# Westlake-AI/SemiReward

Hardware: AMD Instinct MI355X
Metric: unlabeled images/sec/node (FlexMatch+SR, ViT-S CIFAR-100) (higher is better)
Workload: dtype bf16

## Files before the change

include/srhip.h:

```cpp
#ifndef SRHIP_H
#define SRHIP_H

#ifdef __cplusplus
extern "C" {
#endif

enum {
  SRHIP_EPI_BF16 = 0,
  SRHIP_EPI_GELU_BF16 = 1,
  SRHIP_EPI_RESID_F32 = 2,
  SRHIP_EPI_DGELU_BF16 = 3,
  SRHIP_EPI_F32 = 4
};
int srhip_gemm_nt(int epilogue, const void* A, int lda, const void* B, int ldb, void* C, int ldc, int M, int N, int K,
                  const float* bias, const float* row_scale, int rows_per_sample, const void* aux_in, void* aux_out,
                  int ldaux, float alpha, float beta, void* stream);
#define SRHIP_GEMM_PLAN_TILE128 0
#define SRHIP_GEMM_PLAN_SMALL64 1
#define SRHIP_GEMM_PLAN_BIG256 2
#define SRHIP_GEMM_PLAN_BIG128 3
#define SRHIP_GEMM_PLAN_BIG2WG 4
#define SRHIP_GEMM_PLAN_PP256 5
int srhip_gemm_nt_plan(int epilogue, int M, int N, int K, float beta);
int srhip_gemm_nt_planned(int epilogue, const void* A, int lda, const void* B, int ldb, void* C, int ldc, int M, int N, int K,
                          const float* bias, const float* row_scale, int rows_per_sample, const void* aux_in, void* aux_out,
                          int ldaux, float alpha, float beta, int plan_M, void* stream);
int srhip_gemm_small_max_grid(int n);


int srhip_gemm_nt_resid_dropout(const void* A, int lda, const void* B, int ldb, float* C, int ldc, int M, int N, int K,
                                const float* bias, const float* resid, int ldresid, unsigned drop_key, unsigned drop_thresh,
                                float drop_scale, void* stream);
int srhip_gemm_nt_resid_ln_dropout(const void* A, int lda, const void* B, int ldb, float* C, int ldc, int M, int N, int K,
                                   const float* bias, const float* ln_mean, const float* ln_rstd, const float* ln_gamma,
                                   const float* ln_beta, unsigned drop_key, unsigned drop_thresh, float drop_scale, void* stream);

typedef struct srhip_group_desc {
  const void* A; const void* B; float* C;
  int M, N, K, lda, ldb, ldc, tile_start, pad0, pad1, pad2;
} srhip_group_desc;
int srhip_gemm_nt_grouped_f32(const srhip_group_desc* desc_dev, int n_problems, int total_tiles, float alpha, float beta,
                              void* stream);
int srhip_gemm_nt_grouped_n64_f32(const srhip_group_desc* desc_dev, int n_problems, int total_tiles, float alpha, float beta,
                                  void* stream);

#define SRHIP_TN_ATOMIC 1
#define SRHIP_TN_OVERWRITE 2
typedef struct srhip_group_tn_desc {
  const void* A; const void* B; float* C; float* dbias;
  int M, N, K, lda, ldb, ldc, tile_start, flags;
} srhip_group_tn_desc;
int srhip_gemm_tn_grouped_f32(const srhip_group_tn_desc* desc_dev, int n_problems, int total_tiles, float alpha, float beta,
                              void* stream);
typedef struct srhip_slab_desc {
  float* dst; const float* src; long long stride;
  int count, n_slabs, block_start, pad0;
} srhip_slab_desc;
int srhip_slab_reduce_f32(const srhip_slab_desc* desc_dev, int n, int total_blocks, void* stream);
int srhip_gemm_tn_grouped_pp_f32(const srhip_group_tn_desc* desc_dev, int n_problems, int total_tiles, float alpha, float beta,
                                 void* stream);

int srhip_attn_fwd(const void* qkv, void* out, float* lse, int B, int N, int H, float scale, void* stream);
int srhip_attn_bwd(const void* qkv, const void* out, const void* d_out, const float* lse, void* dqkv, float* delta_ws,
                   int B, int N, int H, float scale, void* stream);

int srhip_attn_plan(int B, int N, int H, int* nkt, int* fwd_pair, int* bwd_l2, int* bwd_split);

int srhip_attn_masked_fwd(const void* qkv, void* out, float* lse, const int* key_len, int B, int N, int H, float scale,
                          unsigned drop_key, unsigned drop_thresh, float drop_scale, void* stream);
int srhip_attn_masked_bwd(const void* qkv, const void* out, const void* d_out, const float* lse, void* dqkv, float* delta_ws,
                          const int* key_len, int B, int N, int H, float scale, unsigned drop_key, unsigned drop_thresh,
                          float drop_scale, void* stream);

int srhip_layernorm_fwd(const float* x, const float* gamma, const float* beta, float eps, void* out, float* mean,
                        float* rstd, int M, int D, void* stream);
int srhip_layernorm_bwd(const void* dy, const float* x, const float* mean, const float* rstd, const float* gamma,
                        float* dx, float* dgamma, float* dbeta, int M, int D, void* stream);
int srhip_layernorm_bwd_cast(const void* dy, const float* x, const float* mean, const float* rstd, const float* gamma, float* dx, float* dgamma,
                             float* dbeta, void* out_bf16, const float* row_scale, int rows_per_sample, int M, int D, void* stream);
int srhip_layernorm_bwd_part(const void* dy, const float* x, const float* mean, const float* rstd, const float* gamma, float* dx, float* part,
                             int n_rep, void* out_bf16, const float* row_scale, int rows_per_sample, int M, int D, void* stream);
typedef struct srhip_ln_reduce_desc { float* dgamma; float* dbeta; } srhip_ln_reduce_desc;
int srhip_ln_grad_reduce(const srhip_ln_reduce_desc* desc_dev, float* part, int n_ln, int n_rep, int D, void* stream);
typedef struct srhip_dw_tail {
  const srhip_ln_reduce_desc* ln_desc; float* ln_part;
  const float* dlogits; const float* feat; float* dWh; float* dbh;
  const float* dx; const float* img; const int* img_index; float* dpos; float* dcls; float* pe_ws;
  int n_ln, n_rep, C, B, D, in_chans, HW, ps;
} srhip_dw_tail;
int srhip_gemm_tn_grouped_tail_f32(const srhip_group_tn_desc* desc_dev, int n_problems, int total_tiles, float alpha, float beta,
                                   const srhip_dw_tail* tail, void* stream);
int srhip_patch_embed_bwd_fold(const float* ws, float* dWp, float* dbp, int B, int C, int HW, int ps, int D, void* stream);

int srhip_mlp_fused(const float* x, float* x_out, const float* ln_gamma, const float* ln_beta, float eps, const void* W1,
                    const float* b1, const void* W2, const float* b2, const float* row_scale, int rows_per_sample, int save_rows,
                    void* save_ln2, void* save_pre, void* save_h, float* save_mean, float* save_rstd, int M, int D, int Hd,
                    void* stream);
int srhip_gelu_eval(const float* x, float* y_erf, float* y_poly, int n, void* stream);
int srhip_mlp_fused_proj(const float* x, float* x_out, const void* ao, const void* Wp, const float* bp, const float* row_scale1,
                         int ao_scaled, const float* ln_gamma, const float* ln_beta, float eps, const void* W1, const float* b1, const void* W2,
                         const float* b2, const float* row_scale2, int rows_per_sample, void* ln_next, const float* next_gamma,
                         const float* next_beta, int M, int D, int Hd, void* stream);
int srhip_mlp_fused_proj_strided(const float* x, float* x_out, const void* ao, const void* Wp, const float* bp, const float* row_scale1,
                                 int ao_scaled, const float* ln_gamma, const float* ln_beta, float eps, const void* W1, const float* b1,
                                 const void* W2, const float* b2, const float* row_scale2, int rows_per_sample, void* ln_next,
                                 const float* next_gamma, const float* next_beta, int M, int D, int Hd, int row_pitch, void* stream);

int srhip_attn_block_supported(int N, int D, int H);
int srhip_attn_block_fused(const void* xn_bf16, const void* Wqkv, const float* bqkv, const void* qkv_extra, void* out, const float* out_scale,
                           int B, int N, int D, int H, float scale, void* stream);

int srhip_patch_embed_fwd(const float* img, const int* img_index, const float* Wp, const float* bp, const float* cls,
                          const float* pos, float* x, int B, int C, int HW, int ps, int D, void* stream);
int srhip_patch_embed_bwd(const float* dx, const float* img, const int* img_index, float* dWp, float* dbp, float* dcls,
                          float* dpos, int B, int C, int HW, int ps, int D, void* stream);
long srhip_patch_embed_bwd_ws_floats(int B, int C, int HW, int ps, int D);
int srhip_patch_embed_bwd_ws(const float* dx, const float* img, const int* img_index, float* dWp, float* dbp, float* dcls,
                             float* dpos, float* ws, int B, int C, int HW, int ps, int D, void* stream);

int srhip_patch_im2col(const float* img, const int* img_index, void* out, int B, int C, int HW, int ps, void* stream);
int srhip_patch_assemble(const float* tok, const float* bp, const float* cls, const float* pos, float* x, int B, int Np, int D,
                         void* stream);
int srhip_patch_grad_operands(const float* dx, void* dx_tok_bf16, float* dpos, float* dcls, int B, int Np, int D, void* stream);

enum {
  SRHIP_X3_EPI_F32 = 0,
  SRHIP_X3_EPI_GELU_F32 = 1,
  SRHIP_X3_EPI_RESID_F32 = 2
};
int srhip_gemm_nt_x3(int epilogue, const float* A, int lda, const float* W, int ldw, float* C, int ldc, int M, int N, int K,
                     const float* bias, const float* row_scale, int rows_per_sample, void* stream);
int srhip_attn_fwd_x3(const float* qkv, float* out, int B, int N, int H, float scale, void* stream);
int srhip_layernorm_fwd_f32(const float* x, const float* gamma, const float* beta, float eps, float* out, float* mean, float* rstd, int M,
                            int D, void* stream);
int srhip_patch_im2col_f32(const float* img, const int* img_index, float* out, int B, int C, int HW, int ps, void* stream);

enum { SRHIP_X3B_NT = 0, SRHIP_X3B_NN = 1 };
enum {
  SRHIP_X3B_EPI_F32 = 0,
  SRHIP_X3B_EPI_ACC = 1,
  SRHIP_X3B_EPI_DGELU = 2,
  SRHIP_X3B_EPI_GELU_PRE = 3
};
int srhip_attn_fwd_x3_lse(const float* qkv, float* out, float* lse, int B, int N, int H, float scale, void* stream);
int srhip_gemm_x3(int layout, int epilogue, const float* A, int lda, const float* B, int ldb, float* C, int ldc, int M, int N, int K,
                  const float* bias, const float* aux, float* aux_out, int ldaux, void* stream);
int srhip_gemm_tn_x3_grouped(const srhip_group_tn_desc* desc_dev, int n_problems, int total_tiles, void* stream);
int srhip_attn_bwd_x3(const float* qkv, const float* out, const float* d_out, const float* lse, float* dqkv, float* delta_ws, int B, int N,
                      int H, float scale, void* stream);
int srhip_layernorm_bwd_part_f32(const float* dy, const float* x, const float* mean, const float* rstd, const float* gamma, float* dx,
                                 float* part, int n_rep, float* out, const float* row_scale, int rows_per_sample, int M, int D, void* stream);
int srhip_patch_grad_operands_f32(const float* dx, float* dx_tok, float* dpos, float* dcls, int B, int Np, int D, void* stream);
int srhip_scale_rows_f32(const float* x, const float* scale, int rows_per_sample, float* out, long M, int D, void* stream);

int srhip_cls_head_fwd(const float* x, const float* gamma, const float* beta, float eps, const float* Wh, const float* bh,
                       float* feat, float* logits, float* xhat, float* rstd, int B, int N, int D, int C, void* stream);
int srhip_cls_head_fwd_scatter(const float* x, const float* gamma, const float* beta, float eps, const float* Wh, const float* bh,
                               float* feat, float* logits, float* xhat, float* rstd, float* feat_all, float* logits_all,
                               const long long* out_rows, int B, int N, int D, int C, void* stream);
int srhip_cls_head_bwd(const float* dlogits, const float* Wh, const float* gamma, const float* feat, const float* xhat,
                       const float* rstd, float* dx, float* dWh, float* dbh, float* dgamma, float* dbeta, int B, int N,
                       int D, int C, void* stream);

int srhip_cast_scale_rows(const float* x, const float* scale, int rows_per_sample, void* out, long M, int D, void* stream);
int srhip_transpose_to_bf16(const void* in, int in_is_f32, int ld_in, void* out, int ld_out, int M, int Mp, int C,
                            int apply_gelu, float* colsum, void* stream);
typedef struct srhip_transpose_desc {
  const void* in; void* out;
  int in_is_f32, ld_in, ld_out, M, Mp, C, apply_gelu, tile_start;
  long pad;
} srhip_transpose_desc;
int srhip_transpose_batched(const srhip_transpose_desc* desc_dev, int n, int total_tiles, void* stream);
int srhip_cast_f32_bf16(const float* x, void* out, long n, void* stream);
int srhip_droppath_fill(float* out, const float* probs, int depth, int B, unsigned long long seed, void* stream);
int srhip_droppath_fill_cols(float* out, const float* probs, const long long* cols, int depth, int B, int n_cols, unsigned long long seed,
                             void* stream);

int srhip_vit_fork(float* x, void* ln, const int* parent, int n_new, int dst0, int rows_per_node, int D, void* stream);
int srhip_vit_fanout(const float* node_logits, const float* node_feat, int n_nodes, const int* col_node, const long long* col_rows,
                     int n_cols, float* logits_all, float* feat_all, long long rows_all, int C, int D, void* stream);

int srhip_row_max(const float* in, int in_is_probs, float* probs_out, float* max_probs, long long* max_idx, int B, int C,
                  void* stream);
int srhip_row_max_strided(const float* in, int in_is_probs, float* probs_out, float* max_probs, long long* max_idx, int B, int C,
                          int rows_per_group, long long group_stride, void* stream);
int srhip_flexmatch_mask(const float* max_probs, const long long* max_idx, const long long* idx_ulb, float p_cutoff,
                         long long* selected_label, int* hist, float* classwise_acc, float* mask, int B, int C,
                         int ulb_dest_len, int thresh_warmup, void* stream);
int srhip_flexmatch_mask_passes(const float* max_probs, const long long* max_idx, const long long* idx_ulb, float p_cutoff,
                                long long* selected_label, int* hist, float* classwise_acc, float* mask, int n_pass, int B, int C,
                                int ulb_dest_len, int thresh_warmup, void* stream);
int srhip_index_error(int* bits_out, int reset, void* stream);
int srhip_flexmatch_rebuild_hist(const long long* selected_label, int* hist, int ulb_dest_len, int C, void* stream);
int srhip_fixed_mask(const float* max_probs, float p_cutoff, float* mask, int B, void* stream);
int srhip_freematch_stats(const float* probs, const long long* max_idx, float* colsum, float* hist, int B, int C, void* stream);
int srhip_freematch_update(const float* maxp_all, int n_all, const float* colsum, const float* hist, const float* max_probs,
                           const long long* max_idx, float* time_p, float* p_model, float* label_hist, float* mask, int B, int C,
                           float momentum, float one_minus_momentum, int use_quantile, int clip_thresh, void* stream);
int srhip_distalign(const float* probs, const float* colsum_ulb, int n_ulb, const float* colsum_lb, int n_lb, float* p_model,
                    float* p_target, int* inited, double momentum, float* aligned, float* max_probs, long long* max_idx, int B, int C,
                    void* stream);
int srhip_softmatch_mask(const float* maxp_all, int n_all, const float* max_probs, float* mu_var, double momentum, int n_sigma, float* mask,
                         int B, void* stream);
int srhip_freematch_entropy(const float* logits, const float* mask, const float* p_model, const float* label_hist, float grad_scale,
                            float* loss_out, float* dlogits, float* ws, int B, int C, int accumulate, void* stream);
int srhip_reward_mask2(const float* reward, float* mask2, float* mean_out, const float* mean_in, int groups, int B,
                       void* stream);
int srhip_masked_ce(const float* logits, const long long* targets, const float* mask, const float* mask2, float grad_scale,
                    float* loss_out, float* dlogits, int B, int C, void* stream);
#define SRHIP_REDUCE_NONE 0
#define SRHIP_REDUCE_MEAN 1
#define SRHIP_REDUCE_SUM 2
int srhip_ce_hard(const float* logits, long long ld, const long long* targets, const float* mask, const float* mask2, float grad_scale,
                  int reduction, float* loss_rows, float* loss, float* dlogits, long long ldd, int B, int C, void* stream);
int srhip_ce_soft(const float* logits, long long ld, const float* targets, long long ldt, const float* mask, const float* mask2,
                  float grad_scale, int reduction, float* loss_rows, float* loss, float* dlogits, long long ldd, int B, int C, void* stream);
int srhip_consistency_mse(const float* logits, long long ld, const float* targets, long long ldt, const float* mask, const float* mask2,
                          float grad_scale, int reduction, float* loss_rows, float* loss, float* dlogits, long long ldd, int B, int C,
                          void* stream);
int srhip_consistency_l1(const float* logits, long long ld, const float* targets, long long ldt, const float* mask, const float* mask2,
                         float grad_scale, int reduction, float* loss_rows, float* loss, float* dlogits, long long ldd, int B, int C,
                         void* stream);

int srhip_eval_accumulate(const float* logits, long long ld, const long long* y, int* confusion, void* state, long long* pred_out,
                          long long row_offset, int B, int C, void* stream);

int srhip_pl_monitor(const long long* pseudo, const float* mask0, const float* mask_kept, const float* mask2, const float* reward,
                     const long long* idx_ulb, const long long* ulb_targets, long long n_ulb, int P, int nu, int C, long long* istate,
                     double* fstate, void* stream);

#define SRHIP_SCORE_FIXED 0
#define SRHIP_SCORE_FLEX 1
#define SRHIP_SCORE_FREE 2
#define SRHIP_SCORE_SOFT 3
int srhip_score_rows(const float* logits, long long ld, int B, int C, int mode, float p_cutoff, const float* classwise_acc,
                     const float* time_p, const float* p_model, const float* mu_var, int n_sigma, const float* da_p_model,
                     const float* da_p_target, const int* da_inited, long long* label, float* conf, float* margin, float* entropy,
                     float* weight, void* stream);
int srhip_score_commit(const long long* label, const float* conf, const float* margin, const float* entropy, const float* weight,
                       const float* reward, const float* reward_keep, const long long* idx, long long row_offset, int B, long long n,
                       long long* t_label, float* t_conf, float* t_margin, float* t_entropy, float* t_weight, float* t_reward,
                       unsigned char* t_reward_keep, unsigned char* t_selected, int* t_count, void* stream);
int srhip_reward_mask2_ragged(const float* reward, float* mask2, float* mean_out, int total, int B, void* stream);

long srhip_rewarder_param_count(int F, int L);
long srhip_rewarder_ws_floats(int G, int B);
long srhip_generator_param_count(int F);
long srhip_rewarder_t_floats(int F);
long srhip_generator_t_floats(int F);
int srhip_rewarder_prepare(const float* params, float* params_t, int F, int L, void* stream);
int srhip_generator_prepare(const float* params, float* params_t, int F, void* stream);
int srhip_rewarder_fwd(const float* params, const float* params_t, const float* feats, const long long* labels, float* reward,
                       float* ws, int G, int B, int F, int L, int save_for_bwd, void* stream);
int srhip_rewarder_fwd_strided(const float* params, const float* params_t, const float* feats, long long feat_group_stride,
                               const long long* labels, float* reward, float* ws, float* max_reward_inout, int G, int B, int F, int L,
                               int save_for_bwd, void* stream);
int srhip_rewarder_bwd(const float* params, const float* feats, const long long* labels, const float* target, float* ws,
                       float* grads, float* losses, int B, int F, int L, void* stream);
int srhip_generator_fwd(const float* params, const float* params_t, const float* x, float* out, long long* label, int B, int F,
// ... 154 lines not shown
```

semireward_amd/_lib.py:

```python
import ctypes
import os
from ctypes import c_double, c_float, c_int, c_long, c_longlong, c_uint, c_ulonglong, c_void_p

import torch

HERE = os.path.dirname(os.path.abspath(__file__))
LIB_PATH = os.path.join(HERE, "libsrhip.so")

EPI_BF16, EPI_GELU_BF16, EPI_RESID_F32, EPI_DGELU_BF16, EPI_F32 = range(5)
X3_EPI_F32, X3_EPI_GELU_F32, X3_EPI_RESID_F32 = range(3)
X3B_NT, X3B_NN = range(2)
X3B_EPI_F32, X3B_EPI_ACC, X3B_EPI_DGELU, X3B_EPI_GELU_PRE = range(4)
REDUCE_NONE, REDUCE_MEAN, REDUCE_SUM = range(3)
SCORE_FIXED, SCORE_FLEX, SCORE_FREE, SCORE_SOFT = range(4)

P, I, F, L, Dbl, U = c_void_p, c_int, c_float, c_long, c_double, c_uint
SIGNATURES = {
    "srhip_gemm_nt": (I, [I, P, I, P, I, P, I, I, I, I, P, P, I, P, P, I, F, F, P]),
    "srhip_gemm_nt_plan": (I, [I, I, I, I, F]),
    "srhip_gemm_nt_planned": (I, [I, P, I, P, I, P, I, I, I, I, P, P, I, P, P, I, F, F, I, P]),
    "srhip_vit_fork": (I, [P, P, P, I, I, I, I, P]),
    "srhip_vit_fanout": (I, [P, P, I, P, P, I, P, P, c_longlong, I, I, P]),
    "srhip_gemm_small_max_grid": (I, [I]),
    "srhip_gemm_nt_grouped_f32": (I, [P, I, I, F, F, P]),
    "srhip_gemm_nt_grouped_n64_f32": (I, [P, I, I, F, F, P]),
    "srhip_gemm_tn_grouped_f32": (I, [P, I, I, F, F, P]),
    "srhip_gemm_tn_grouped_pp_f32": (I, [P, I, I, F, F, P]),
    "srhip_gemm_tn_grouped_tail_f32": (I, [P, I, I, F, F, P, P]),
    "srhip_patch_embed_bwd_fold": (I, [P, P, P, I, I, I, I, I, P]),
    "srhip_slab_reduce_f32": (I, [P, I, I, P]),
    "srhip_attn_fwd": (I, [P, P, P, I, I, I, F, P]),
    "srhip_attn_bwd": (I, [P, P, P, P, P, P, I, I, I, F, P]),
    "srhip_attn_plan": (I, [I, I, I, P, P, P, P]),
    "srhip_layernorm_fwd": (I, [P, P, P, F, P, P, P, I, I, P]),
    "srhip_layernorm_bwd": (I, [P, P, P, P, P, P, P, P, I, I, P]),
    "srhip_layernorm_bwd_cast": (I, [P, P, P, P, P, P, P, P, P, P, I, I, I, P]),
    "srhip_layernorm_bwd_part": (I, [P, P, P, P, P, P, P, I, P, P, I, I, I, P]),
    "srhip_ln_grad_reduce": (I, [P, P, I, I, I, P]),
    "srhip_mlp_fused": (I, [P, P, P, P, F, P, P, P, P, P, I, I, P, P, P, P, P, I, I, I, P]),
    "srhip_attn_block_supported": (I, [I, I, I]),
    "srhip_attn_block_fused": (I, [P, P, P, P, P, P, I, I, I, I, F, P]),
    "srhip_gelu_eval": (I, [P, P, P, I, P]),
    "srhip_mlp_fused_proj": (I, [P, P, P, P, P, P, I, P, P, F, P, P, P, P, P, I, P, P, P, I, I, I, P]),
    "srhip_mlp_fused_proj_strided": (I, [P, P, P, P, P, P, I, P, P, F, P, P, P, P, P, I, P, P, P, I, I, I, I, P]),
    "srhip_adam_bias_corrections": (I, [F, F, I, P]),
    "srhip_adamw_flat_dyn": (I, [P, P, P, P, P, P, P, I, P, P, P, F, F, F, Dbl, F, P, I, P]),
    "srhip_adam_flat_dyn": (I, [P, P, P, P, L, F, F, F, F, P, P]),
    "srhip_droppath_fill_cols_dyn": (I, [P, P, P, I, I, I, P, c_ulonglong, P]),
    "srhip_patch_embed_fwd": (I, [P, P, P, P, P, P, P, I, I, I, I, I, P]),
    "srhip_patch_embed_bwd": (I, [P, P, P, P, P, P, P, I, I, I, I, I, P]),
    "srhip_patch_embed_bwd_ws_floats": (L, [I, I, I, I, I]),
    "srhip_patch_embed_bwd_ws": (I, [P, P, P, P, P, P, P, P, I, I, I, I, I, P]),
    "srhip_patch_im2col": (I, [P, P, P, I, I, I, I, P]),
    "srhip_patch_assemble": (I, [P, P, P, P, P, I, I, I, P]),
    "srhip_patch_grad_operands": (I, [P, P, P, P, I, I, I, P]),
    "srhip_gemm_nt_x3": (I, [I, P, I, P, I, P, I, I, I, I, P, P, I, P]),
    "srhip_attn_fwd_x3": (I, [P, P, I, I, I, F, P]),
    "srhip_layernorm_fwd_f32": (I, [P, P, P, F, P, P, P, I, I, P]),
    "srhip_patch_im2col_f32": (I, [P, P, P, I, I, I, I, P]),
    "srhip_attn_fwd_x3_lse": (I, [P, P, P, I, I, I, F, P]),
    "srhip_gemm_x3": (I, [I, I, P, I, P, I, P, I, I, I, I, P, P, P, I, P]),
    "srhip_gemm_tn_x3_grouped": (I, [P, I, I, P]),
    "srhip_attn_bwd_x3": (I, [P, P, P, P, P, P, I, I, I, F, P]),
    "srhip_layernorm_bwd_part_f32": (I, [P, P, P, P, P, P, P, I, P, P, I, I, I, P]),
    "srhip_patch_grad_operands_f32": (I, [P, P, P, P, I, I, I, P]),
    "srhip_scale_rows_f32": (I, [P, P, I, P, L, I, P]),
    "srhip_cls_head_fwd": (I, [P, P, P, F, P, P, P, P, P, P, I, I, I, I, P]),
    "srhip_cls_head_fwd_scatter": (I, [P, P, P, F, P, P, P, P, P, P, P, P, P, I, I, I, I, P]),
    "srhip_cls_head_bwd": (I, [P, P, P, P, P, P, P, P, P, P, P, I, I, I, I, P]),
    "srhip_cast_scale_rows": (I, [P, P, I, P, L, I, P]),
    "srhip_transpose_to_bf16": (I, [P, I, I, P, I, I, I, I, I, P, P]),
    "srhip_transpose_batched": (I, [P, I, I, P]),
    "srhip_cast_f32_bf16": (I, [P, P, L, P]),
    "srhip_droppath_fill": (I, [P, P, I, I, c_ulonglong, P]),
    "srhip_droppath_fill_cols": (I, [P, P, P, I, I, I, c_ulonglong, P]),
    "srhip_row_max": (I, [P, I, P, P, P, I, I, P]),
    "srhip_row_max_strided": (I, [P, I, P, P, P, I, I, I, c_longlong, P]),
    "srhip_flexmatch_mask": (I, [P, P, P, F, P, P, P, P, I, I, I, I, P]),
    "srhip_flexmatch_mask_passes": (I, [P, P, P, F, P, P, P, P, I, I, I, I, I, P]),
    "srhip_flexmatch_rebuild_hist": (I, [P, P, I, I, P]),
    "srhip_fixed_mask": (I, [P, F, P, I, P]),
    "srhip_freematch_stats": (I, [P, P, P, P, I, I, P]),
    "srhip_freematch_update": (I, [P, I, P, P, P, P, P, P, P, P, I, I, F, F, I, I, P]),
    "srhip_freematch_entropy": (I, [P, P, P, P, F, P, P, P, I, I, I, P]),
    "srhip_distalign": (I, [P, P, I, P, I, P, P, P, Dbl, P, P, P, I, I, P]),
    "srhip_softmatch_mask": (I, [P, I, P, P, Dbl, I, P, I, P]),
    "srhip_reward_mask2": (I, [P, P, P, P, I, I, P]),
    "srhip_masked_ce": (I, [P, P, P, P, F, P, P, I, I, P]),
    "srhip_ce_hard": (I, [P, c_longlong, P, P, P, F, I, P, P, P, c_longlong, I, I, P]),
    "srhip_ce_soft": (I, [P, c_longlong, P, c_longlong, P, P, F, I, P, P, P, c_longlong, I, I, P]),
    "srhip_consistency_mse": (I, [P, c_longlong, P, c_longlong, P, P, F, I, P, P, P, c_longlong, I, I, P]),
    "srhip_consistency_l1": (I, [P, c_longlong, P, c_longlong, P, P, F, I, P, P, P, c_longlong, I, I, P]),
    "srhip_eval_accumulate": (I, [P, c_longlong, P, P, P, P, c_longlong, I, I, P]),
    "srhip_pl_monitor": (I, [P, P, P, P, P, P, P, c_longlong, I, I, I, P, P, P]),
    "srhip_score_rows": (I, [P, c_longlong, I, I, I, F, P, P, P, P, I, P, P, P, P, P, P, P, P, P]),
    "srhip_score_commit": (I, [P, P, P, P, P, P, P, P, c_longlong, I, c_longlong, P, P, P, P, P, P, P, P, P, P]),
    "srhip_reward_mask2_ragged": (I, [P, P, P, I, I, P]),
    "srhip_rewarder_param_count": (L, [I, I]),
    "srhip_rewarder_ws_floats": (L, [I, I]),
    "srhip_generator_param_count": (L, [I]),
    "srhip_rewarder_t_floats": (L, [I]),
    "srhip_generator_t_floats": (L, [I]),
    "srhip_rewarder_prepare": (I, [P, P, I, I, P]),
    "srhip_generator_prepare": (I, [P, P, I, P]),
    "srhip_rewarder_fwd": (I, [P, P, P, P, P, P, I, I, I, I, I, P]),
    "srhip_rewarder_fwd_strided": (I, [P, P, P, c_longlong, P, P, P, P, I, I, I, I, I, P]),
    "srhip_rewarder_bwd": (I, [P, P, P, P, P, P, P, I, I, I, P]),
    "srhip_generator_fwd": (I, [P, P, P, P, P, I, I, P]),
    "srhip_sr_target": (I, [P, P, P, I, I, P]),
    "srhip_label_error": (I, [P, I, P]),
    "srhip_index_error": (I, [P, I, P]),
    "srhip_prof_enable": (I, [I]),
    "srhip_prof_count": (I, []),
    "srhip_prof_elapsed_ms": (I, [I, I, P]),
    "srhip_adam_flat": (I, [P, P, P, P, L, F, F, F, F, I, P]),
    "srhip_adamw_flat": (I, [P, P, P, P, P, P, P, I, P, P, F, F, F, F, I, Dbl, F, P, I, P]),
    "srhip_clip_grad_ws_floats": (I, []),
    "srhip_clip_grad_coef": (I, [P, L, F, F, P, P, P]),
    "srhip_nchw_to_nhwc_bf16": (I, [P, P, I, I, I, I, P]),
    "srhip_im2col": (I, [P, P, I, I, I, I, I, I, I, P]),
    "srhip_im2col_bn": (I, [P, P, P, P, P, F, I, P, I, I, I, I, I, I, I, P]),
    "srhip_col2im": (I, [P, P, I, I, I, I, I, I, I, I, P]),
    "srhip_conv_weight_prep": (I, [P, P, P, I, I, I, I, P]),
    "srhip_add_unpad": (I, [P, P, I, I, I, I, P]),
    "srhip_conv_weight_prep_grouped": (I, [P, I, c_longlong, P]),
    "srhip_add_unpad_grouped": (I, [P, I, c_longlong, P]),
    "srhip_conv_weight_flip_grouped": (I, [P, I, c_longlong, P]),
    "srhip_bn_ws_doubles": (ctypes.c_longlong, []),
    "srhip_wrn_conv_supported": (I, [I, I, I]),
    "srhip_wrn_conv_last_plan": (I, []),
    "srhip_bn_acc_doubles": (ctypes.c_longlong, [I]),
    "srhip_wrn_conv_bn": (I, [P, I, P, P, P, P, P, F, F, P, P, P, P, F, I, P, P, P, I, I, I, I, I, I, I, I, P, I, P]),
    "srhip_wrn_head": (I, [P, I, P, P, P, P, P, F, F, P, P, P, P, F, I, P, P, P, P, I, I, I, I, I, P]),
    "srhip_wrn_conv_bn_passes": (I, [P, I, P, P, P, P, P, F, F, P, P, P, P, F, I, P, P, P, I, I, I, I, I, I, I, I, P, I, I, P]),
    "srhip_wrn_head_passes": (I, [P, I, P, P, P, P, P, F, F, P, P, P, P, F, I, P, P, P, P, I, I, I, I, I, I, P]),
    "srhip_bn_running_chain": (I, [P, I, I, F, P]),
    "srhip_bn_stats": (I, [P, F, F, I, P, P, P, P, P, I, I, P]),
    "srhip_bn_act": (I, [P, P, P, P, P, F, F, I, P, P, I, I, P]),
    "srhip_bn_accumulate": (I, [P, P, I, I, P]),
    "srhip_bn_fold": (I, [P, Dbl, F, F, I, P, P, P, P, P, I, P]),
    "srhip_bn_bwd_reduce": (I, [P, P, P, P, P, P, F, P, I, I, P]),
    "srhip_bn_bwd_apply": (I, [P, P, P, P, P, P, F, P, P, P, P, P, P, Dbl, P, I, I, P]),
    "srhip_bn_fwd": (I, [P, P, P, F, F, F, I, I, P, P, P, P, P, P, P, I, I, P]),
    "srhip_bn_bwd": (I, [P, P, P, P, P, P, F, P, P, P, P, P, I, I, P]),
    "srhip_avgpool_fwd": (I, [P, P, I, I, I, P]),
    "srhip_avgpool_bwd": (I, [P, P, I, I, I, P]),
    "srhip_fc_fwd": (I, [P, P, P, P, I, I, I, P]),
    "srhip_fc_bwd": (I, [P, P, P, P, P, P, I, I, I, P]),
    "srhip_sgd_flat": (I, [P, P, P, P, P, I, L, F, F, F, P, Dbl, I, I, P]),
    "srhip_gemm_nt_resid_dropout": (I, [P, I, P, I, P, I, I, I, I, P, P, I, U, U, F, P]),
    "srhip_gemm_nt_resid_ln_dropout": (I, [P, I, P, I, P, I, I, I, I, P, P, P, P, P, U, U, F, P]),
    "srhip_attn_masked_fwd": (I, [P, P, P, P, I, I, I, F, U, U, F, P]),
    "srhip_attn_masked_bwd": (I, [P, P, P, P, P, P, P, I, I, I, F, U, U, F, P]),
    "srhip_embed_ln_fwd": (I, [P, I, P, P, P, P, P, P, F, P, P, P, P, I, I, I, U, U, F, P]),
    "srhip_embed_ln_bwd": (I, [P, P, I, P, P, P, P, P, P, P, P, P, P, P, P, I, I, I, I, U, U, F, P]),
    "srhip_postln_fwd": (I, [P, P, P, F, P, P, P, P, I, I, P]),
    "srhip_postln_bwd": (I, [P, P, P, P, P, P, P, P, P, I, I, U, U, F, P]),
# ... 55 lines not shown
```

semireward_amd/csrc/attn_block.hip:

```cpp
#include <stdlib.h>

#include <type_traits>
#include <utility>

#include "../../include/srhip.h"
#include "common.h"

namespace {

constexpr int HD = 64;
constexpr int DM = 384;
constexpr int NH = DM / HD;
constexpr int KS = DM / 32;
constexpr int SK = 64;
constexpr int ST_EL = 64 * SK;
constexpr int NS = 8;
constexpr int GS = 2;
constexpr int NG = NS / GS;
constexpr int SPM = DM / SK;
constexpr int SPH = 3 * SPM;
constexpr int NSTG = NH * SPH;
constexpr float LOG2E = 1.4426950408889634f;

typedef __attribute__((address_space(3))) void lds_void;
template <int N_>
__device__ __forceinline__ void wait_vm() { asm volatile("s_waitcnt vmcnt(%0)" ::"n"(N_) : "memory"); }
__device__ __forceinline__ void lds_barrier() {
  asm volatile("s_waitcnt lgkmcnt(0)" ::: "memory");
  __builtin_amdgcn_s_barrier();
  asm volatile("" ::: "memory");
}

__device__ __forceinline__ int fresh_lane() {
  int l;
  asm volatile("v_mbcnt_lo_u32_b32 %0, -1, 0\n\tv_mbcnt_hi_u32_b32 %0, -1, %0" : "=v"(l));
  return l;
}

__device__ __forceinline__ float max3_raw(float a, float b, float c) {
  return __builtin_amdgcn_fmed3f(__builtin_amdgcn_fmed3f(a, b, INFINITY), c, INFINITY);
}
__device__ __forceinline__ float rows_max(float x) {
  const unsigned u = __float_as_uint(x);
  const auto a = __builtin_amdgcn_permlane16_swap(u, u, false, false);
  const unsigned v = __float_as_uint(__builtin_amdgcn_fmed3f(__uint_as_float(a[0]), __uint_as_float(a[1]), INFINITY));
  const auto b = __builtin_amdgcn_permlane32_swap(v, v, false, false);
  return __builtin_amdgcn_fmed3f(__uint_as_float(b[0]), __uint_as_float(b[1]), INFINITY);
}
__device__ __forceinline__ float rows_sum(float x) {
  const unsigned u = __float_as_uint(x);
  const auto a = __builtin_amdgcn_permlane16_swap(u, u, false, false);
  const unsigned v = __float_as_uint(__uint_as_float(a[0]) + __uint_as_float(a[1]));
  const auto b = __builtin_amdgcn_permlane32_swap(v, v, false, false);
  return __uint_as_float(b[0]) + __uint_as_float(b[1]);
}

__device__ __forceinline__ f32x4_t mfma16(u32x4_t a, u32x4_t b, f32x4_t c) {
  return __builtin_amdgcn_mfma_f32_16x16x32_bf16(__builtin_bit_cast(bf16x8_t, a), __builtin_bit_cast(bf16x8_t, b), c, 0, 0, 0);
}
__device__ __forceinline__ u32x4_t ldf(const bf16_t* p) { return *reinterpret_cast<const u32x4_t*>(p); }
__device__ __forceinline__ u32x4_t pack8v(f32x4_t lo, f32x4_t hi) {
  return u32x4_t{pack_bf2(lo[0], lo[1]), pack_bf2(lo[2], lo[3]), pack_bf2(hi[0], hi[1]), pack_bf2(hi[2], hi[3])};
}
constexpr int vt_pitch(int NP) { return ((NP / 2) % 64 == 16 || (NP / 2) % 64 == 48) ? NP : NP + 32; }
__device__ __forceinline__ int swz4(int row) { return (0x78 >> (((row >> 2) & 3) * 2)) & 3; }
constexpr int nkt_of(int N) { return 2 * ((N + 31) / 32); }

template <class F, int... Is>
__device__ __forceinline__ void static_for_impl(F&& f, std::integer_sequence<int, Is...>) { (f(std::integral_constant<int, Is>{}), ...); }
template <int N, class F>
__device__ __forceinline__ void static_for(F&& f) { static_for_impl(f, std::make_integer_sequence<int, N>{}); }

struct AbArgs {
  const bf16_t* xnb;
  const bf16_t* qx;
  const float* bqkv;
  const bf16_t* W;
  bf16_t* out;
  const float* osc;
  float scale;
  int B;
};

template <int N, int DBG>
__global__ __launch_bounds__(512, 2) void attn_block_kernel(AbArgs a) {
  constexpr int NKT = nkt_of(N), NP = NKT * 16, TP = vt_pitch(NP);
  constexpr int NQT = (N + 15) / 16;
  constexpr bool EXTRA = NQT == 17;
  static_assert(NQT <= 16 || (EXTRA && N == 257), "two token tiles per wave (+ one extra token)");
  constexpr int NKT_LO = (N - 1) / 16;
  extern __shared__ __attribute__((aligned(16))) bf16_t sm[];
  bf16_t* ring = sm;
  bf16_t* Ks = ring + NS * ST_EL;
  bf16_t* Vt = Ks + NP * HD;
  bf16_t* sx = Vt + HD * TP;
  float* sbias = reinterpret_cast<float*>(sx + 3 * DM);
  const int tid = threadIdx.x, lane = tid & 63;
  const int wave = __builtin_amdgcn_readfirstlane(tid >> 6);
  const int l15 = lane & 15, g = lane >> 4;
  const int img = blockIdx.x;
  const float osc = a.osc ? a.osc[img] : 1.0f;
  const int hpw = NH / gridDim.y, hbeg = blockIdx.y * hpw, hend = hbeg + hpw;
  const size_t row0 = (size_t)img * N;

  const int rho = 8 * wave + (lane >> 3);
  const int srcc = (lane & 7) ^ ((rho >> 1) & 7);
  const int fperm = (rho & 32) + 8 * ((rho & 15) >> 2) + 4 * ((rho >> 4) & 1) + (rho & 3);
  const int vo_kq = (fperm * DM + srcc * 8) * 2, vo_v = (rho * DM + srcc * 8) * 2;
  const __amdgpu_buffer_rsrc_t rw = __builtin_amdgcn_make_buffer_rsrc(const_cast<bf16_t*>(a.W), 0, 3 * DM * DM * 2, 0x00020000);
  constexpr int OOB = 0x7ffffff0;
  auto issue = [&](auto rc, int h) __attribute__((always_inline)) {
    constexpr int r0 = decltype(rc)::value, r = r0 % SPH, m = r / SPM, kc = r % SPM;
    const int hh = h + r0 / SPH;
    const bool valid = hh < hend;
    constexpr int brow = m == 0 ? DM : m == 1 ? 2 * DM : 0;
    lds_void* dst = (lds_void*)(ring + (r0 % NS >= 0 ? ((hh * SPH + r) & (NS - 1)) : 0) * ST_EL + wave * 8 * SK);
    if constexpr ((DBG & 4) != 0) return;
    __builtin_amdgcn_raw_ptr_buffer_load_lds(rw, dst, 16, valid ? (m == 1 ? vo_v : vo_kq) : OOB,
                                             valid ? ((brow + hh * HD) * DM + kc * SK) * 2 : 0, 0, 0);
  };
  issue(std::integral_constant<int, 0>{}, hbeg); issue(std::integral_constant<int, 1>{}, hbeg);
  issue(std::integral_constant<int, 2>{}, hbeg); issue(std::integral_constant<int, 3>{}, hbeg);
  static_assert((NG - 2) * GS == 4, "prologue issues the first two groups");

  for (int i = tid; i < 3 * DM; i += 512) sbias[i] = a.bqkv[i];
  if (EXTRA && tid < 3 * DM / 8) reinterpret_cast<u32x4_t*>(sx)[tid] = ldf(a.qx + (size_t)img * 3 * DM + 8 * tid);
  for (int i = tid; i < (NP - N) * HD / 8; i += 512) reinterpret_cast<u32x4_t*>(Ks + N * HD)[i] = u32x4_t{0u, 0u, 0u, 0u};
  for (int i = tid; i < HD * TP / 8; i += 512) reinterpret_cast<u32x4_t*>(Vt)[i] = u32x4_t{0u, 0u, 0u, 0u};
  __syncthreads();

  u32x4_t xn[2][KS];
#pragma unroll
  for (int tt = 0; tt < 2; ++tt) {
    const bool have = tt == 0 || NQT - (EXTRA ? 1 : 0) == 16 || wave + 8 < NQT - (EXTRA ? 1 : 0);
    const int tok = min(16 * (wave + 8 * tt) + l15, N - 1);
    const bf16_t* xr = a.xnb + (row0 + tok) * DM + 8 * g;
#pragma unroll
    for (int k = 0; k < KS; ++k) xn[tt][k] = have ? ldf(xr + 32 * k) : u32x4_t{0u, 0u, 0u, 0u};
  }

  const int kc_ = g ^ ((l15 >> 1) & 7);
  const int fo0 = l15 * SK + (kc_ << 3), fo1 = l15 * SK + ((kc_ ^ 4) << 3);
  const int kof0 = l15 * HD + (kc_ << 3), kof1 = l15 * HD + ((kc_ ^ 4) << 3);
  const int vof = l15 * TP + ((g ^ swz4(l15)) << 3);
  const float sc2 = a.scale * LOG2E;

  auto sync_group = [&](auto rc, int h) __attribute__((always_inline)) {
    constexpr int r = decltype(rc)::value;
    if constexpr ((DBG & 4) == 0) wait_vm<GS*(NG - 3)>();
    __builtin_amdgcn_s_barrier();
    if constexpr ((DBG & 32) == 0) {
      issue(std::integral_constant<int, r + (NG - 2) * GS>{}, h);
      issue(std::integral_constant<int, r + (NG - 2) * GS + 1>{}, h);
    }
    static_assert(GS == 2, "two stages per group");
  };
  constexpr bool ALL2 = NQT - (EXTRA ? 1 : 0) == 16;
  const bool tile1 = ALL2 || wave + 8 < NQT - (EXTRA ? 1 : 0);

  u32x4_t qf[2][2];
  auto project = [&](auto mc, int h) __attribute__((always_inline)) {
    constexpr int M = decltype(mc)::value;
    f32x4_t acc[2][4];
    const float* bb = sbias + (M == 0 ? DM : M == 1 ? 2 * DM : 0) + h * HD;
#pragma unroll
    for (int t = 0; t < 4; ++t) {
      f32x4_t b4;
      if constexpr (M == 1) { const float b = bb[16 * t + l15]; b4 = f32x4_t{b, b, b, b}; }
      else b4 = *reinterpret_cast<const f32x4_t*>(bb + 32 * (t >> 1) + 8 * g + 4 * (t & 1));
      acc[0][t] = b4; acc[1][t] = b4;
    }
    u32x4_t fa[2][2];
    auto rd = [&](auto uc) __attribute__((always_inline)) {
      constexpr int u = decltype(uc)::value, j = u >> 1, hf = u & 1, stg = j >> 1, sh = j & 1;
      const bf16_t* tile = ring + ((h * SPH + M * SPM + stg) & (NS - 1)) * ST_EL;
      fa[u & 1][0] = ldf(tile + (2 * hf) * 16 * SK + (sh ? fo1 : fo0));
      fa[u & 1][1] = ldf(tile + (2 * hf + 1) * 16 * SK + (sh ? fo1 : fo0));
    };
    auto mm = [&](auto uc) __attribute__((always_inline)) {
      constexpr int u = decltype(uc)::value, j = u >> 1, hf = u & 1;
      u32x4_t(&fr)[2] = fa[u & 1];
      if constexpr ((DBG & 2) != 0) {
        asm volatile("" ::"v"(fr[0]), "v"(fr[1]));
      } else if constexpr (M != 1) {
#pragma unroll
        for (int t = 0; t < 2; ++t) {
          acc[0][2 * hf + t] = mfma16(fr[t], xn[0][j], acc[0][2 * hf + t]);
// ... 210 lines not shown
```

semireward_amd/csrc/mlp_fused.hip:

```cpp
#include <stdlib.h>

#include <utility>

#include "../../include/srhip.h"
#include "common.h"

namespace {

constexpr int BK = 32;
constexpr int RT = 128;
constexpr int TILE_EL = RT * BK;
constexpr int NS = 16;
constexpr int FBM = 128;
constexpr int CH = 64;

__device__ __forceinline__ int swz(int row) { return (0x78 >> (((row >> 2) & 3) * 2)) & 3; }

typedef __attribute__((address_space(3))) void lds_void;
typedef const __attribute__((address_space(1))) void gbl_void;
template <int N_>
__device__ __forceinline__ void wait_vm() { asm volatile("s_waitcnt vmcnt(%0)" ::"n"(N_) : "memory"); }

template <class F, int... Is>
__device__ __forceinline__ void static_for_impl(F&& f, std::integer_sequence<int, Is...>) { (f(std::integral_constant<int, Is>{}), ...); }
template <int N, class F>
__device__ __forceinline__ void static_for(F&& f) { static_for_impl(f, std::make_integer_sequence<int, N>{}); }

struct MlpArgs {
  const float* x;
  float* xo;
  bf16_t *s_ln2, *s_pre, *s_h;
  float *s_mean, *s_rstd;
  int save_rows;
  const float *gamma, *beta, *b1, *b2, *row_scale;
  const bf16_t *W1, *W2;
  const bf16_t *ao, *Wp;
  const float *bp, *row_scale1;
  int ao_scaled;
  bf16_t* ln_next;
  const float *gamma_n, *beta_n;
  float eps;
  int M, Hd, rows_per_sample;
  int pitch;
};

#ifdef SRHIP_TUNING
__device__ long long srhip_mlp_dbg[8 * 1024];
#define MDBG_T(i) do { if (threadIdx.x == 0 && blockIdx.x < 1024) srhip_mlp_dbg[8 * blockIdx.x + (i)] = wall_clock64(); } while (0)
#else
#define MDBG_T(i) do { } while (0)
#endif
template <int D_, int DBG, int GS, bool PROJ = false, int SPREAD = 0, bool PITCH = false>
__global__ __launch_bounds__(512, 2) void mlp_fused_kernel(MlpArgs a) {
  static_assert(PROJ || !PITCH, "the row pitch belongs to the PROJ variant");
  constexpr int KS1 = D_ / BK;
  constexpr int KQ = 4;
  constexpr int G1S = 2 * (KS1 / KQ);
  constexpr int TH = D_ / RT;
  constexpr int NT2 = D_ / 16;
  constexpr int G2S = (CH / BK) * TH;
  constexpr int SPC = G1S + G2S;
  constexpr int NG = NS / GS;
  constexpr int PD = (NG - 2) * GS;
  static_assert(KS1 % KQ == 0 && D_ % RT == 0 && SPC % GS == 0 && NS % GS == 0 && NG >= 3, "layout");
  extern __shared__ __attribute__((aligned(16))) bf16_t sm[];
  float* sb1 = reinterpret_cast<float*>(sm + NS * TILE_EL);
  float* sb2 = sb1 + a.Hd;
  float* sgam = sb2 + D_;
  float* sbet = sgam + D_;
  float* sbp = sbet + D_;
  float* sgn = sbp + D_;
  float* sbn = sgn + D_;
  const int tid = threadIdx.x, lane = tid & 63;
  const int wave = __builtin_amdgcn_readfirstlane(tid >> 6);
  const int l15 = lane & 15, lg = lane >> 4;
  const int nch = a.Hd / CH;
  for (int i = tid; i < a.Hd; i += 512) sb1[i] = a.b1[i];
  for (int i = tid; i < D_; i += 512) { sb2[i] = a.b2[i]; sgam[i] = a.gamma[i]; sbet[i] = a.beta[i]; }
  if constexpr (PROJ) {
    for (int i = tid; i < D_; i += 512) sbp[i] = a.bp[i];
    if (a.ln_next) for (int i = tid; i < D_; i += 512) { sgn[i] = a.gamma_n[i]; sbn[i] = a.beta_n[i]; }
  }
  __syncthreads();

  const int pr = 16 * wave + (lane >> 2);
  const int psl = ((lane & 3) ^ swz(pr)) * 8;
  const int lo1 = ((pr & 31) * D_ + (pr >> 5) * BK + psl) * 2;
  const int lo2 = (pr * a.Hd + psl) * 2;
  const int pdst = 16 * wave * BK;
  const int wbytes = a.Hd * D_ * 2;
  const __amdgpu_buffer_rsrc_t r1 = __builtin_amdgcn_make_buffer_rsrc(const_cast<bf16_t*>(a.W1), 0, wbytes, 0x00020000);
  const __amdgpu_buffer_rsrc_t r2 = __builtin_amdgcn_make_buffer_rsrc(const_cast<bf16_t*>(a.W2), 0, wbytes, 0x00020000);
  constexpr int OOB = 0x7ffffff0;
  constexpr int VOFF = PROJ ? TH : 0;
  const int nchv = nch + VOFF;
  const __amdgpu_buffer_rsrc_t rp = __builtin_amdgcn_make_buffer_rsrc(const_cast<bf16_t*>(PROJ ? a.Wp : a.W2), 0, D_ * D_ * 2, 0x00020000);
  const int lop = (pr * D_ + psl) * 2;
  auto issue = [&](int cv, int j, int slot) {
    if (DBG & 2) return;
    lds_void* dst = (lds_void*)(sm + slot * TILE_EL + pdst);
    const bool valid = cv < nchv;
    if (PROJ && cv < VOFF) {
      __builtin_amdgcn_raw_ptr_buffer_load_lds(rp, dst, 16, lop, (cv * RT * D_ + j * BK) * 2, 0, 0);
      return;
    }
    const int c = cv - VOFF;
    if (j < G1S) {
      const int u = j / (KS1 / KQ), kt = j % (KS1 / KQ);
      __builtin_amdgcn_raw_ptr_buffer_load_lds(r1, dst, 16, valid ? lo1 : OOB, ((c * CH + 32 * u) * D_ + kt * KQ * BK) * 2, 0, 0);
    } else {
      const int jj = j - G1S, u = jj / TH, th = jj % TH;
      __builtin_amdgcn_raw_ptr_buffer_load_lds(r2, dst, 16, valid ? lo2 : OOB, (th * RT * a.Hd + c * CH + u * BK) * 2, 0, 0);
    }
  };

  const int fo2 = l15 * BK + ((lg ^ swz(l15)) << 3);
  const int h1 = 8 * (l15 >> 2) + (l15 & 3);
  const int fo1p = h1 * BK + ((lg ^ swz(h1)) << 3);
  const int fo1q = (h1 + 4) * BK + ((lg ^ swz(h1 + 4)) << 3);

  const size_t rpitch = PITCH ? (size_t)a.pitch : (size_t)D_;
  const int ntiles = (a.M + FBM - 1) / FBM;
  for (int tile = blockIdx.x; tile < ntiles; tile += gridDim.x) {
    const int m = tile * FBM + wave * 16 + l15;
    const int mc = min(m, a.M - 1);
    MDBG_T(0);
    u32x4_t xn[KS1];
    if constexpr (!PROJ) {
      const float* xr = a.x + (size_t)mc * D_ + 8 * lg;
      f32x4_t v[2 * KS1];
      float s = 0.f;
#pragma unroll
      for (int k = 0; k < KS1; ++k) {
        v[2 * k] = *reinterpret_cast<const f32x4_t*>(xr + 32 * k);
        v[2 * k + 1] = *reinterpret_cast<const f32x4_t*>(xr + 32 * k + 4);
      }
#pragma unroll
      for (int k = 0; k < 2 * KS1; ++k) s += (v[k][0] + v[k][1]) + (v[k][2] + v[k][3]);
      s += __shfl_xor(s, 16, 64);
      s += __shfl_xor(s, 32, 64);
      const float mu = s * (1.0f / D_);
      float q = 0.f;
#pragma unroll
      for (int k = 0; k < 2 * KS1; ++k) {
#pragma unroll
        for (int e = 0; e < 4; ++e) { const float d = v[k][e] - mu; q += d * d; }
      }
      q += __shfl_xor(q, 16, 64);
      q += __shfl_xor(q, 32, 64);
      const float rs = rsqrtf(q * (1.0f / D_) + a.eps);
      if (a.save_rows > 0 && m < a.save_rows && lg == 0) { a.s_mean[m] = mu; a.s_rstd[m] = rs; }
#pragma unroll
      for (int k = 0; k < KS1; ++k) {
        const f32x4_t g0 = *reinterpret_cast<const f32x4_t*>(sgam + 32 * k + 8 * lg);
        const f32x4_t g1 = *reinterpret_cast<const f32x4_t*>(sgam + 32 * k + 8 * lg + 4);
        const f32x4_t b0 = *reinterpret_cast<const f32x4_t*>(sbet + 32 * k + 8 * lg);
        const f32x4_t b1 = *reinterpret_cast<const f32x4_t*>(sbet + 32 * k + 8 * lg + 4);
        const f32x4_t p = v[2 * k], r = v[2 * k + 1];
        xn[k] = u32x4_t{pack_bf2((p[0] - mu) * rs * g0[0] + b0[0], (p[1] - mu) * rs * g0[1] + b0[1]),
                        pack_bf2((p[2] - mu) * rs * g0[2] + b0[2], (p[3] - mu) * rs * g0[3] + b0[3]),
                        pack_bf2((r[0] - mu) * rs * g1[0] + b1[0], (r[1] - mu) * rs * g1[1] + b1[1]),
                        pack_bf2((r[2] - mu) * rs * g1[2] + b1[2], (r[3] - mu) * rs * g1[3] + b1[3])};
        if (k & 1) __builtin_amdgcn_sched_barrier(0);
      }
    }
    const bool save_tile = !PROJ && a.save_rows > 0 && tile * FBM + wave * 16 < a.save_rows;
    if (save_tile && m < a.save_rows) {
      bf16_t* lr = a.s_ln2 + (size_t)m * D_ + 8 * lg;
#pragma unroll
      for (int k = 0; k < KS1; ++k) *reinterpret_cast<u32x4_t*>(lr + 32 * k) = xn[k];
    }
    u32x4_t aof[PROJ ? KS1 : 1];
    if constexpr (PROJ) {
      const bf16_t* ar = a.ao + (size_t)mc * rpitch + 8 * lg;
#pragma unroll
      for (int k = 0; k < KS1; ++k) aof[k] = *reinterpret_cast<const u32x4_t*>(ar + 32 * k);
    }
    float rs1v = 1.0f, rs2v = 1.0f;
    f32x4_t acc2[NT2];
    if constexpr (PROJ) {
      if (a.row_scale1) rs1v = a.row_scale1[mc / a.rows_per_sample];
      if (a.row_scale) rs2v = a.row_scale[mc / a.rows_per_sample];
      const float* xr = a.x + (size_t)mc * rpitch + 4 * lg;
#pragma unroll
      for (int t = 0; t < NT2; ++t) acc2[t] = *reinterpret_cast<const f32x4_t*>(xr + 16 * t);
      if (rs1v != 1.0f && !a.ao_scaled) {
#pragma unroll
        for (int k = 0; k < KS1; ++k)
#pragma unroll
          for (int e = 0; e < 4; ++e)
            aof[k][e] = pack_bf2(rs1v * __builtin_bit_cast(float, aof[k][e] << 16), rs1v * __builtin_bit_cast(float, aof[k][e] & 0xffff0000u));
      }
    }
    __syncthreads();
    MDBG_T(1);
#pragma unroll
    for (int p = 0; p < PD; ++p) issue(p / SPC, p % SPC, p);

    __builtin_amdgcn_sched_barrier(0);
    if constexpr (!PROJ) {
#pragma unroll
      for (int t = 0; t < NT2; ++t) acc2[t] = f32x4_t{0.f, 0.f, 0.f, 0.f};
    } else {
#pragma unroll
      for (int t = 0; t < NT2; ++t) {
        const f32x4_t bb = *reinterpret_cast<const f32x4_t*>(sbp + 16 * t + 4 * lg);
        acc2[t][0] += rs1v * bb[0]; acc2[t][1] += rs1v * bb[1]; acc2[t][2] += rs1v * bb[2]; acc2[t][3] += rs1v * bb[3];
      }
    }
    f32x4_t acc1[4];
    u32x4_t hf[2];
    u32x4_t fa0[4], fa1[4];

    auto sync_group = [&](auto jc, int c) __attribute__((always_inline)) {
      constexpr int j = decltype(jc)::value;
      static_assert(j % GS == 0, "group start");
      if constexpr ((DBG & 2) == 0) wait_vm<GS*(NG - 3)>();
      __builtin_amdgcn_s_barrier();
      if constexpr (!SPREAD) {
#pragma unroll
        for (int i = 0; i < GS; ++i) {
          const int jn = (j + PD + i) % SPC, cn = c + (j + PD + i) / SPC;
          issue(cn, jn, (c * SPC + j + PD + i) & (NS - 1));
        }
      }
    };
    auto issue_ahead = [&](auto jc, int c, bool late) __attribute__((always_inline)) {
      constexpr int j = decltype(jc)::value;
      if constexpr (SPREAD == 1) { if (!late) issue(c + (j + PD) / SPC, (j + PD) % SPC, (c * SPC + j + PD) & (NS - 1)); }
    };
    auto read_half = [&](auto jc, auto hc, int c) __attribute__((always_inline)) {
      constexpr int j = decltype(jc)::value, h = decltype(hc)::value;
      u32x4_t(&fa)[4] = h ? fa1 : fa0;
      const bf16_t* st = sm + ((c * SPC + j) & (NS - 1)) * TILE_EL;
      if constexpr ((DBG & 4) != 0) {
#pragma unroll
        for (int t = 0; t < 4; ++t) fa[t] = u32x4_t{(unsigned)(c + t), 1u, 2u, (unsigned)j};
      } else if constexpr (j < G1S) {
#pragma unroll
        for (int s_ = 0; s_ < 2; ++s_) {
          fa[2 * s_] = *reinterpret_cast<const u32x4_t*>(st + fo1p + (2 * h + s_) * 32 * BK);
          fa[2 * s_ + 1] = *reinterpret_cast<const u32x4_t*>(st + fo1q + (2 * h + s_) * 32 * BK);
        }
      } else {
#pragma unroll
        for (int t = 0; t < 4; ++t) fa[t] = *reinterpret_cast<const u32x4_t*>(st + fo2 + (4 * h + t) * 16 * BK);
      }
    };
    float gcarry = 0.f, pcarry = 0.f;
    auto acc1_start = [&](auto uc, auto xc, int c) __attribute__((always_inline)) {
      constexpr int u = decltype(uc)::value, X = decltype(xc)::value;
      acc1[2 * u + X] = *reinterpret_cast<const f32x4_t*>(sb1 + min(c - VOFF, nch - 1) * CH + 32 * u + 8 * lg + 4 * X);
    };
    auto gelu_elem = [&](auto uc, auto ec, int c) __attribute__((always_inline)) {
      constexpr int u = decltype(uc)::value, e = decltype(ec)::value, X = e >> 2, r = e & 3;
      const float v = acc1[2 * u + X][r];
      if constexpr (PROJ && (DBG & 1) == 0) {
        if constexpr ((e & 1) == 1) {
          const f32x2_t g2 = gelu_poly2(f32x2_t{acc1[2 * u + X][r - 1], v}) * f32x2_t{rs2v, rs2v};
          hf[u][e >> 1] = pack_bf2(g2[0], g2[1]);
        }
      } else {
      float gv;
      if constexpr ((DBG & 1) != 0) gv = v; else gv = gelu_erf(v);
      if constexpr (PROJ) gv *= rs2v;
      if constexpr ((e & 1) == 0) { gcarry = gv; pcarry = v; } else hf[u][e >> 1] = pack_bf2(gcarry, gv);
      }
      if constexpr ((e & 1) == 1) {
        if (save_tile && m < a.save_rows) {
          const size_t o = (size_t)m * a.Hd + (c - VOFF) * CH + 32 * u + 8 * lg + (e - 1);
          *reinterpret_cast<uint32_t*>(a.s_pre + o) = pack_bf2(pcarry, v);
          *reinterpret_cast<uint32_t*>(a.s_h + o) = hf[u][e >> 1];
        }
      }
      if constexpr (r == 3) acc1_start(uc, std::integral_constant<int, X>{}, c + 1);
    };
    auto gelu_slot = [&](auto jc, auto hc, auto pc, int c) __attribute__((always_inline)) {
      constexpr int j = decltype(jc)::value, h = decltype(hc)::value, part = decltype(pc)::value;
      if constexpr (j >= 3 && j <= 8 && (DBG & 8) == 0) {
        constexpr int u = (j - 3) / 3, q = 2 * ((j - 3) % 3) + h;
        constexpr int first[7] = {0, 2, 3, 4, 6, 7, 8};
        constexpr int e0 = first[q], n = first[q + 1] - first[q];
        if constexpr (part < n) gelu_elem(std::integral_constant<int, u>{}, std::integral_constant<int, e0 + part>{}, c);
      }
    };
    auto mfma_one = [&](auto jc, auto hc, auto tc) __attribute__((always_inline)) {
      constexpr int j = decltype(jc)::value, h = decltype(hc)::value, t = decltype(tc)::value;
      u32x4_t(&fa)[4] = h ? fa1 : fa0;
      if constexpr ((DBG & 8) != 0) {
        asm volatile("" ::"v"(fa[t]));
        if constexpr (j == G1S - 1) { hf[0] = fa[0]; hf[1] = fa[1]; }
      } else if constexpr (j < G1S) {
        constexpr int u = j / (KS1 / KQ), kt = j % (KS1 / KQ);
        acc1[2 * u + (t & 1)] = __builtin_amdgcn_mfma_f32_16x16x32_bf16(
            __builtin_bit_cast(bf16x8_t, fa[t]), __builtin_bit_cast(bf16x8_t, xn[kt * KQ + 2 * h + (t >> 1)]), acc1[2 * u + (t & 1)],
            0, 0, 0);
      } else {
        constexpr int u = (j - G1S) / TH, th = (j - G1S) % TH;
        acc2[th * 8 + 4 * h + t] = __builtin_amdgcn_mfma_f32_16x16x32_bf16(
            __builtin_bit_cast(bf16x8_t, fa[t]), __builtin_bit_cast(bf16x8_t, hf[u]), acc2[th * 8 + 4 * h + t], 0, 0, 0);
      }
    };
    auto mfma_half = [&](auto jc, auto hc, int c) __attribute__((always_inline)) {
      using T0 = std::integral_constant<int, 0>;
      using T1 = std::integral_constant<int, 1>;
      using T2 = std::integral_constant<int, 2>;
      using T3 = std::integral_constant<int, 3>;
      mfma_one(jc, hc, T0{});
      mfma_one(jc, hc, T1{});
      __builtin_amdgcn_sched_barrier(0);
      gelu_slot(jc, hc, T0{}, c);
      __builtin_amdgcn_sched_barrier(0);
      mfma_one(jc, hc, T2{});
      mfma_one(jc, hc, T3{});
      __builtin_amdgcn_sched_barrier(0);
      gelu_slot(jc, hc, T1{}, c);
      __builtin_amdgcn_sched_barrier(0);
    };
    using H0 = std::integral_constant<int, 0>;
    using H1 = std::integral_constant<int, 1>;
    if constexpr (PROJ) {
      auto read_half_p = [&](auto jc, auto hc, int cv) __attribute__((always_inline)) {
        constexpr int j = decltype(jc)::value, h = decltype(hc)::value;
        u32x4_t(&fa)[4] = h ? fa1 : fa0;
        const bf16_t* st = sm + ((cv * SPC + j) & (NS - 1)) * TILE_EL;
#pragma unroll
        for (int t = 0; t < 4; ++t) fa[t] = *reinterpret_cast<const u32x4_t*>(st + fo2 + (4 * h + t) * 16 * BK);
      };
      sync_group(H0{}, 0);
      read_half_p(H0{}, H0{}, 0);
      static_for<VOFF>([&](auto vc) __attribute__((always_inline)) {
        constexpr int v = decltype(vc)::value;
        static_for<SPC>([&](auto jc) __attribute__((always_inline)) {
          constexpr int j = decltype(jc)::value;
          constexpr int jn = (j + 1) % SPC, vn = v + (j + 1) / SPC;
          read_half_p(jc, H1{}, v);
#pragma unroll
          for (int t = 0; t < 4; ++t)
            acc2[v * 8 + t] = __builtin_amdgcn_mfma_f32_16x16x32_bf16(__builtin_bit_cast(bf16x8_t, fa0[t]), __builtin_bit_cast(bf16x8_t, aof[j]),
                                                                       acc2[v * 8 + t], 0, 0, 0);
          __builtin_amdgcn_sched_barrier(0);
          issue_ahead(jc, v, false);
          if constexpr (jn % GS == 0) sync_group(std::integral_constant<int, jn>{}, vn);
          if constexpr (vn == VOFF) read_half(std::integral_constant<int, 0>{}, H0{}, vn);
          else read_half_p(std::integral_constant<int, jn>{}, H0{}, vn);
#pragma unroll
          for (int t = 0; t < 4; ++t)
            acc2[v * 8 + 4 + t] = __builtin_amdgcn_mfma_f32_16x16x32_bf16(__builtin_bit_cast(bf16x8_t, fa1[t]), __builtin_bit_cast(bf16x8_t, aof[j]),
                                                                           acc2[v * 8 + 4 + t], 0, 0, 0);
          __builtin_amdgcn_sched_barrier(0);
          issue_ahead(jc, v, true);
        });
      });
      MDBG_T(4);
      {
        float sum = 0.f;
#pragma unroll
        for (int t = 0; t < NT2; ++t) sum += (acc2[t][0] + acc2[t][1]) + (acc2[t][2] + acc2[t][3]);
        const float mu = rows_sum4(sum) * (1.0f / D_);
        float q = 0.f;
#pragma unroll
        for (int t = 0; t < NT2; ++t)
#pragma unroll
          for (int e = 0; e < 4; ++e) { const float d = acc2[t][e] - mu; q += d * d; }
        const float rs = rsqrtf(rows_sum4(q) * (1.0f / D_) + a.eps);
        int ko = 4 * lg;
        asm volatile("" : "+v"(ko) : "v"(rs));
#pragma unroll
        for (int sI = 0; sI < KS1; ++sI) {
          if (sI > 0) asm volatile("" : "+v"(ko) : "v"(xn[sI - 1][3]));
          unsigned pk[2][2];
#pragma unroll
          for (int e = 0; e < 2; ++e) {
            const int t = 2 * sI + e;
            const f32x4_t g4 = *reinterpret_cast<const f32x4_t*>(sgam + 16 * t + ko);
            const f32x4_t b4 = *reinterpret_cast<const f32x4_t*>(sbet + 16 * t + ko);
            pk[e][0] = pack_bf2((acc2[t][0] - mu) * rs * g4[0] + b4[0], (acc2[t][1] - mu) * rs * g4[1] + b4[1]);
            pk[e][1] = pack_bf2((acc2[t][2] - mu) * rs * g4[2] + b4[2], (acc2[t][3] - mu) * rs * g4[3] + b4[3]);
          }
          unsigned out4[4];
#pragma unroll
          for (int d = 0; d < 2; ++d) {
            const auto w32 = __builtin_amdgcn_permlane32_swap(pk[0][d], pk[1][d], false, false);
            const auto w16 = __builtin_amdgcn_permlane16_swap(w32[0], w32[1], false, false);
            out4[d] = w16[0];
            out4[2 + d] = w16[1];
          }
          xn[sI] = u32x4_t{out4[0], out4[1], out4[2], out4[3]};
          if (sI & 1) __builtin_amdgcn_sched_barrier(0);
        }
      }
      MDBG_T(5);
#pragma unroll
      for (int t = 0; t < NT2; ++t) {
        const f32x4_t bb = *reinterpret_cast<const f32x4_t*>(sb2 + 16 * t + 4 * lg);
        acc2[t][0] += rs2v * bb[0]; acc2[t][1] += rs2v * bb[1]; acc2[t][2] += rs2v * bb[2]; acc2[t][3] += rs2v * bb[3];
      }
    }
    {
      using I0 = std::integral_constant<int, 0>;
      using I1 = std::integral_constant<int, 1>;
      acc1_start(I0{}, I0{}, VOFF); acc1_start(I0{}, I1{}, VOFF); acc1_start(I1{}, I0{}, VOFF); acc1_start(I1{}, I1{}, VOFF);
    }
    if constexpr (!PROJ) {
      sync_group(H0{}, 0);
      read_half(H0{}, H0{}, 0);
    }
    for (int c = VOFF; c < nchv; ++c)
      static_for<SPC>([&](auto jc) __attribute__((always_inline)) {
        constexpr int j = decltype(jc)::value;
        constexpr int jn = (j + 1) % SPC;
        const int cn = c + (j + 1) / SPC;
        read_half(jc, H1{}, c);
        mfma_half(jc, H0{}, c);
        issue_ahead(jc, c, false);
        if constexpr (jn % GS == 0) sync_group(std::integral_constant<int, jn>{}, cn);
        read_half(std::integral_constant<int, jn>{}, H0{}, cn);
        mfma_half(jc, H1{}, c);
        issue_ahead(jc, c, true);
      });
    MDBG_T(2);
    if (PROJ && a.ln_next) {
      float* xw = a.xo + (size_t)mc * rpitch + 4 * lg;
      float sum = 0.f;
#pragma unroll
      for (int t = 0; t < NT2; ++t) {
        const f32x4_t xv = acc2[t];
        if (m < a.M) *reinterpret_cast<f32x4_t*>(xw + 16 * t) = xv;
        sum += (xv[0] + xv[1]) + (xv[2] + xv[3]);
      }
      const float mu = rows_sum4(sum) * (1.0f / D_);
      float q = 0.f;
#pragma unroll
      for (int t = 0; t < NT2; ++t)
#pragma unroll
        for (int e = 0; e < 4; ++e) { const float d = acc2[t][e] - mu; q += d * d; }
      const float rs = rsqrtf(rows_sum4(q) * (1.0f / D_) + a.eps);
      bf16_t* lw = a.ln_next + (size_t)mc * D_ + 8 * lg;
      int ko = 4 * lg;
      asm volatile("" : "+v"(ko) : "v"(rs));
      unsigned chain = 0;
#pragma unroll
      for (int sI = 0; sI < KS1; ++sI) {
        if (sI > 0) asm volatile("" : "+v"(ko) : "v"(chain));
        unsigned pk[2][2];
#pragma unroll
        for (int e = 0; e < 2; ++e) {
          const int t = 2 * sI + e;
          const f32x4_t g4 = *reinterpret_cast<const f32x4_t*>(sgn + 16 * t + ko);
          const f32x4_t b4 = *reinterpret_cast<const f32x4_t*>(sbn + 16 * t + ko);
          pk[e][0] = pack_bf2((acc2[t][0] - mu) * rs * g4[0] + b4[0], (acc2[t][1] - mu) * rs * g4[1] + b4[1]);
          pk[e][1] = pack_bf2((acc2[t][2] - mu) * rs * g4[2] + b4[2], (acc2[t][3] - mu) * rs * g4[3] + b4[3]);
        }
        unsigned out4[4];
#pragma unroll
        for (int d = 0; d < 2; ++d) {
          const auto w32 = __builtin_amdgcn_permlane32_swap(pk[0][d], pk[1][d], false, false);
          const auto w16 = __builtin_amdgcn_permlane16_swap(w32[0], w32[1], false, false);
          out4[d] = w16[0];
          out4[2 + d] = w16[1];
        }
        chain = out4[3];
        if (m < a.M) *reinterpret_cast<u32x4_t*>(lw + 32 * sI) = u32x4_t{out4[0], out4[1], out4[2], out4[3]};
      }
    } else if (PROJ) {
      float* xw = a.xo + (size_t)mc * rpitch + 4 * lg;
      if (m < a.M) {
#pragma unroll
        for (int t = 0; t < NT2; ++t) *reinterpret_cast<f32x4_t*>(xw + 16 * t) = acc2[t];
      }
    } else if (m < a.M) {
      const float rsc = a.row_scale ? a.row_scale[m / a.rows_per_sample] : 1.0f;
      const float* xr = a.x + (size_t)m * D_ + 4 * lg;
      float* xw = a.xo + (size_t)m * D_ + 4 * lg;
#pragma unroll
      for (int t = 0; t < NT2; ++t) {
        const f32x4_t bb = *reinterpret_cast<const f32x4_t*>(sb2 + 16 * t + 4 * lg);
        f32x4_t xv = *reinterpret_cast<const f32x4_t*>(xr + 16 * t);
        xv[0] += rsc * (acc2[t][0] + bb[0]); xv[1] += rsc * (acc2[t][1] + bb[1]);
        xv[2] += rsc * (acc2[t][2] + bb[2]); xv[3] += rsc * (acc2[t][3] + bb[3]);
        *reinterpret_cast<f32x4_t*>(xw + 16 * t) = xv;
      }
    }
#ifdef SRHIP_TUNING
    __builtin_amdgcn_s_waitcnt(0);
    __syncthreads();
    MDBG_T(3);
#endif
  }
}


__global__ void gelu_eval_kernel(const float* __restrict__ x, float* __restrict__ y_erf, float* __restrict__ y_poly, int n) {
  const int i = 2 * (blockIdx.x * blockDim.x + threadIdx.x);
  if (i >= n) return;
  const float a = x[i], b = i + 1 < n ? x[i + 1] : 0.f;
  const f32x2_t g = gelu_poly2(f32x2_t{a, b});
  y_erf[i] = gelu_erf(a); y_poly[i] = g[0];
  if (i + 1 < n) { y_erf[i + 1] = gelu_erf(b); y_poly[i + 1] = g[1]; }
}

}

#ifdef SRHIP_TUNING
extern "C" int srhip_mlp_debug(long long* out_host, int n) {
  return hipMemcpyFromSymbol(out_host, HIP_SYMBOL(srhip_mlp_dbg), (size_t)n * sizeof(long long)) == hipSuccess ? SR_OK : SR_EINVAL;
}
#endif
extern "C" int srhip_gelu_eval(const float* x, float* y_erf, float* y_poly, int n, void* stream) {
  if (!x || !y_erf || !y_poly || n <= 0) return SR_EINVAL;
  SR_LAUNCH(gelu_eval_kernel, dim3(cdiv((n + 1) / 2, 256)), dim3(256), 0, (hipStream_t)stream, x, y_erf, y_poly, n);
  SR_CHECK_LAUNCH();
  return SR_OK;
}
extern "C" int srhip_mlp_fused(const float* x, float* x_out, const float* ln_gamma, const float* ln_beta, float eps, const void* W1,
                               const float* b1, const void* W2, const float* b2, const float* row_scale, int rows_per_sample,
                               int save_rows, void* save_ln2, void* save_pre, void* save_h, float* save_mean, float* save_rstd,
                               int M, int D, int Hd, void* stream) {
  if (!x || !x_out || !ln_gamma || !ln_beta || !W1 || !b1 || !W2 || !b2 || M <= 0) return SR_EINVAL;
  if (D != 384 || Hd < 128 || (Hd % RT) || Hd > 4096) return SR_EINVAL;
  if (row_scale && rows_per_sample <= 0) return SR_EINVAL;
  if (save_rows < 0 || save_rows > M || (save_rows > 0 && (!save_ln2 || !save_pre || !save_h || !save_mean || !save_rstd))) return SR_EINVAL;
  if (((uintptr_t)x | (uintptr_t)x_out | (uintptr_t)W1 | (uintptr_t)W2 | (uintptr_t)ln_gamma | (uintptr_t)ln_beta | (uintptr_t)save_ln2 |
       (uintptr_t)save_pre | (uintptr_t)save_h) & 15)
    return SR_EINVAL;
  MlpArgs a;
  a.x = x; a.xo = x_out; a.gamma = ln_gamma; a.beta = ln_beta; a.b1 = b1; a.b2 = b2; a.row_scale = row_scale;
  a.s_ln2 = (bf16_t*)save_ln2; a.s_pre = (bf16_t*)save_pre; a.s_h = (bf16_t*)save_h; a.s_mean = save_mean; a.s_rstd = save_rstd;
  a.save_rows = save_rows;
  a.W1 = (const bf16_t*)W1; a.W2 = (const bf16_t*)W2; a.eps = eps; a.M = M; a.Hd = Hd;
  a.rows_per_sample = rows_per_sample > 0 ? rows_per_sample : 1;
  a.ao = nullptr; a.Wp = nullptr; a.bp = nullptr; a.row_scale1 = nullptr; a.ao_scaled = 0; a.ln_next = nullptr; a.gamma_n = a.beta_n = nullptr;
  a.pitch = D;
  const size_t smem = (size_t)NS * TILE_EL * sizeof(bf16_t) + (size_t)(Hd + 6 * D) * sizeof(float);
  void (*kern)(MlpArgs) = mlp_fused_kernel<384, 0, 4>;
#ifdef SRHIP_TUNING
  switch (SR_TUNE_ENV("SRHIP_MLP_DEBUG") ? atoi(SR_TUNE_ENV("SRHIP_MLP_DEBUG")) : 0) {
    case 1: kern = mlp_fused_kernel<384, 1, 4>; break;
    case 2: kern = mlp_fused_kernel<384, 2, 4>; break;
    case 3: kern = mlp_fused_kernel<384, 3, 4>; break;
    case 7: kern = mlp_fused_kernel<384, 7, 4>; break;
    case 11: kern = mlp_fused_kernel<384, 11, 4>; break;
    case 15: kern = mlp_fused_kernel<384, 15, 4>; break;
    case 100: kern = mlp_fused_kernel<384, 0, 2>; break;
    case 101: kern = mlp_fused_kernel<384, 0, 1>; break;
    default: break;
  }
#endif
  (void)hipFuncSetAttribute((const void*)kern, hipFuncAttributeMaxDynamicSharedMemorySize, (int)smem);
  const int ntiles = cdiv(M, FBM);
  SR_LAUNCH(kern, dim3(min(ntiles, 256)), dim3(512), smem, (hipStream_t)stream, a);
  SR_CHECK_LAUNCH();
  return SR_OK;
}

static int mlp_fused_proj_launch(const float* x, float* x_out, const void* ao, const void* Wp, const float* bp, const float* row_scale1,
                                 int ao_scaled, const float* ln_gamma, const float* ln_beta, float eps, const void* W1, const float* b1, const void* W2,
                                 const float* b2, const float* row_scale2, int rows_per_sample, void* ln_next, const float* next_gamma,
                                 const float* next_beta, int M, int D, int Hd, int row_pitch, void* stream) {
  if (!x || !x_out || !ao || !Wp || !bp || !ln_gamma || !ln_beta || !W1 || !b1 || !W2 || !b2 || M <= 0) return SR_EINVAL;
  if (ln_next && (!next_gamma || !next_beta || ((uintptr_t)ln_next & 15))) return SR_EINVAL;
  if (D != 384 || Hd < 128 || (Hd % RT) || Hd > 4096) return SR_EINVAL;
  if ((row_scale1 || row_scale2) && rows_per_sample <= 0) return SR_EINVAL;
  if (((uintptr_t)x | (uintptr_t)x_out | (uintptr_t)ao | (uintptr_t)Wp | (uintptr_t)W1 | (uintptr_t)W2 | (uintptr_t)ln_gamma | (uintptr_t)ln_beta) & 15)
    return SR_EINVAL;
  MlpArgs a;
  a.x = x; a.xo = x_out; a.gamma = ln_gamma; a.beta = ln_beta; a.b1 = b1; a.b2 = b2; a.row_scale = row_scale2;
  a.s_ln2 = a.s_pre = a.s_h = nullptr; a.s_mean = a.s_rstd = nullptr; a.save_rows = 0;
  a.W1 = (const bf16_t*)W1; a.W2 = (const bf16_t*)W2; a.eps = eps; a.M = M; a.Hd = Hd;
  a.rows_per_sample = rows_per_sample > 0 ? rows_per_sample : 1;
  a.ao = (const bf16_t*)ao; a.Wp = (const bf16_t*)Wp; a.bp = bp; a.row_scale1 = row_scale1; a.ao_scaled = ao_scaled;
  a.ln_next = (bf16_t*)ln_next; a.gamma_n = next_gamma; a.beta_n = next_beta; a.pitch = row_pitch ? row_pitch : D;
  const size_t smem = (size_t)NS * TILE_EL * sizeof(bf16_t) + (size_t)(Hd + 6 * D) * sizeof(float);
  static const int spread = SR_TUNE_ENV("SRHIP_MLP_SPREAD") ? atoi(SR_TUNE_ENV("SRHIP_MLP_SPREAD")) : 1;
  void (*kern)(MlpArgs) = spread ? mlp_fused_kernel<384, 0, 4, true, 1> : mlp_fused_kernel<384, 0, 4, true, 0>;
  if (row_pitch) kern = mlp_fused_kernel<384, 0, 4, true, 1, true>;
  (void)hipFuncSetAttribute((const void*)kern, hipFuncAttributeMaxDynamicSharedMemorySize, (int)smem);
  const int ntiles = cdiv(M, FBM);
  SR_LAUNCH(kern, dim3(min(ntiles, 256)), dim3(512), smem, (hipStream_t)stream, a);
  SR_CHECK_LAUNCH();
  return SR_OK;
}

extern "C" int srhip_mlp_fused_proj(const float* x, float* x_out, const void* ao, const void* Wp, const float* bp, const float* row_scale1,
                                    int ao_scaled, const float* ln_gamma, const float* ln_beta, float eps, const void* W1, const float* b1, const void* W2,
                                    const float* b2, const float* row_scale2, int rows_per_sample, void* ln_next, const float* next_gamma,
                                    const float* next_beta, int M, int D, int Hd, void* stream) {
  return mlp_fused_proj_launch(x, x_out, ao, Wp, bp, row_scale1, ao_scaled, ln_gamma, ln_beta, eps, W1, b1, W2, b2, row_scale2, rows_per_sample, ln_next,
                               next_gamma, next_beta, M, D, Hd, 0, stream);
}

extern "C" int srhip_mlp_fused_proj_strided(const float* x, float* x_out, const void* ao, const void* Wp, const float* bp, const float* row_scale1,
                                            int ao_scaled, const float* ln_gamma, const float* ln_beta, float eps, const void* W1, const float* b1,
                                            const void* W2, const float* b2, const float* row_scale2, int rows_per_sample, void* ln_next,
                                            const float* next_gamma, const float* next_beta, int M, int D, int Hd, int row_pitch, void* stream) {
  if (row_pitch < D || (row_pitch % 8) != 0) return SR_EINVAL;
  if (ln_next && row_pitch != D) return SR_EINVAL;
  return mlp_fused_proj_launch(x, x_out, ao, Wp, bp, row_scale1, ao_scaled, ln_gamma, ln_beta, eps, W1, b1, W2, b2, row_scale2, rows_per_sample, ln_next,
                               next_gamma, next_beta, M, D, Hd, row_pitch, stream);
}
```

semireward_amd/csrc/vit_ops.hip:

```cpp
#include "common.h"
#include "srhip.h"
#include "tail_ops.h"

namespace {

template <int NV, typename TOUT = bf16_t>
__global__ __launch_bounds__(256) void ln_fwd_kernel(const float* __restrict__ x, const float* __restrict__ gamma,
                                                    const float* __restrict__ beta, float eps, TOUT* __restrict__ out,
                                                    float* __restrict__ mean, float* __restrict__ rstd, int M) {
  constexpr int D = NV * 128, RW = 2;
  const int row0 = (blockIdx.x * 4 + (threadIdx.x >> 6)) * RW, lane = threadIdx.x & 63;
  if (row0 >= M) return;
  float2 v[RW][NV], g[NV], b[NV];
#pragma unroll
  for (int r = 0; r < RW; ++r) {
    const float2* xr = reinterpret_cast<const float2*>(x + (size_t)min(row0 + r, M - 1) * D);
#pragma unroll
    for (int i = 0; i < NV; ++i) v[r][i] = xr[i * 64 + lane];
  }
#pragma unroll
  for (int i = 0; i < NV; ++i) {
    g[i] = reinterpret_cast<const float2*>(gamma)[i * 64 + lane];
    b[i] = reinterpret_cast<const float2*>(beta)[i * 64 + lane];
  }
// ... 339 lines not shown
  uint4 o = {pack_bf2(a.x * s, a.y * s), pack_bf2(a.z * s, a.w * s), pack_bf2(b.x * s, b.y * s), pack_bf2(b.z * s, b.w * s)};
  reinterpret_cast<uint4*>(out)[i] = o;
}

template <typename TIN, bool GELU>
__device__ __forceinline__ void transpose_tile(const TIN* __restrict__ in, int ld_in, bf16_t* __restrict__ out, int ld_out,
                                               int M, int Mp, float* __restrict__ colsum, int m0, int c0, float (*tile)[65]) {
  for (int e = threadIdx.x; e < 64 * 64; e += 256) {
    const int r = e >> 6, c = e & 63, m = m0 + r;
    float v = 0.f;
    if (m < M) {
      if constexpr (sizeof(TIN) == 2) v = bf2f(in[(size_t)m * ld_in + c0 + c]);
      else v = (float)in[(size_t)m * ld_in + c0 + c];
      if (GELU) v = gelu_erf(v);
    }
    tile[r][c] = v;
  }
  __syncthreads();
  for (int e = threadIdx.x; e < 64 * 32; e += 256) {
    const int c = e >> 5, rp = (e & 31) * 2, m = m0 + rp;
    if (m < Mp) *reinterpret_cast<uint32_t*>(out + (size_t)(c0 + c) * ld_out + m) = pack_bf2(tile[rp][c], tile[rp + 1][c]);
  }
  if (colsum && threadIdx.x < 64) {
    float s = 0.f;
    for (int r = 0; r < 64; ++r) s += tile[r][threadIdx.x];
    atomicAdd(colsum + c0 + threadIdx.x, s);
  }
}

template <typename TIN, bool GELU>
__global__ __launch_bounds__(256) void transpose_kernel(const TIN* __restrict__ in, int ld_in, bf16_t* __restrict__ out, int ld_out,
                                                       int M, int Mp, float* __restrict__ colsum) {
  __shared__ float tile[64][65];
  transpose_tile<TIN, GELU>(in, ld_in, out, ld_out, M, Mp, colsum, blockIdx.x * 64, blockIdx.y * 64, tile);
}

__global__ __launch_bounds__(256) void transpose_batched_kernel(const srhip_transpose_desc* __restrict__ desc, int n) {
  __shared__ float tile[64][65];
  const int t = blockIdx.x;
  int p = 0;
  {
    int lo = 0, hi = n - 1;
    while (lo < hi) { const int mid = (lo + hi + 1) >> 1; if (t >= desc[mid].tile_start) lo = mid; else hi = mid - 1; }
    p = lo;
  }
  const srhip_transpose_desc d = desc[p];
  const int local = t - d.tile_start, tm = (d.Mp + 63) / 64;
  const int m0 = (local % tm) * 64, c0 = (local / tm) * 64;
  if (d.in_is_f32) transpose_tile<float, false>((const float*)d.in, d.ld_in, (bf16_t*)d.out, d.ld_out, d.M, d.Mp, nullptr, m0, c0, tile);
  else if (d.apply_gelu) transpose_tile<bf16_t, true>((const bf16_t*)d.in, d.ld_in, (bf16_t*)d.out, d.ld_out, d.M, d.Mp, nullptr, m0, c0, tile);
  else transpose_tile<bf16_t, false>((const bf16_t*)d.in, d.ld_in, (bf16_t*)d.out, d.ld_out, d.M, d.Mp, nullptr, m0, c0, tile);
}

__global__ void cast_f32_bf16_kernel(const float* __restrict__ x, bf16_t* __restrict__ out, size_t n) {
  const size_t i = ((size_t)blockIdx.x * blockDim.x + threadIdx.x) * 4;
  if (i + 3 < n) {
    const float4 a = *reinterpret_cast<const float4*>(x + i);
    uint2 o = {pack_bf2(a.x, a.y), pack_bf2(a.z, a.w)};
    *reinterpret_cast<uint2*>(out + i) = o;
  } else {
    for (size_t j = i; j < n; ++j) out[j] = f2bf(x[j]);
  }
}

__global__ void droppath_fill_kernel(float* __restrict__ out, const float* __restrict__ probs, int depth, int B,
                                     unsigned long long seed, const long long* __restrict__ cols, int n,
                                     const unsigned long long* __restrict__ seed_dev) {
  if (seed_dev) seed += seed_dev[0];
  const int o = blockIdx.x * blockDim.x + threadIdx.x;
  if (o >= depth * 2 * n) return;
  long long col = o % n;
  if (cols) { col = cols[col]; if (col < 0 || col >= B) col = 0; }
  const int i = (o / n) * B + (int)col;
  const float p = probs[i / (2 * B)];
  unsigned long long z = seed + 0x9E3779B97F4A7C15ull * (unsigned long long)(i + 1);
  z = (z ^ (z >> 30)) * 0xBF58476D1CE4E5B9ull;
  z = (z ^ (z >> 27)) * 0x94D049BB133111EBull;
  z ^= z >> 31;
  const float u = (float)(z >> 40) * (1.0f / 16777216.0f);
  const float keep = 1.0f - p;
  out[o] = (p <= 0.f) ? 1.0f : (u < keep ? 1.0f / keep : 0.0f);
}

}

template <typename TOUT = bf16_t>
__global__ __launch_bounds__(256) void patch_im2col_kernel(const float* __restrict__ img, const int* __restrict__ img_index,
                                                          TOUT* __restrict__ out, int C, int HW, int ps) {
  const int gw = HW / ps, Np = gw * gw, K = C * ps * ps;
  const int p = blockIdx.x, b = blockIdx.y, py = p / gw, px = p % gw;
  const int bi = img_index ? img_index[b] : b;
  const float* im = img + (size_t)bi * C * HW * HW;
  TOUT* o = out + ((size_t)b * Np + p) * K;
  for (int e = 2 * threadIdx.x; e < K; e += 512) {
    const int c = e / (ps * ps), i = (e / ps) % ps, j = e % ps;
    const float2 v = *reinterpret_cast<const float2*>(im + ((size_t)c * HW + py * ps + i) * HW + px * ps + j);
    if constexpr (sizeof(TOUT) == 4) *reinterpret_cast<float2*>(o + e) = v;
    else *reinterpret_cast<uint32_t*>(o + e) = pack_bf2(v.x, v.y);
  }
}

__global__ void patch_assemble_kernel(const float* __restrict__ tok, const float* __restrict__ bp, const float* __restrict__ cls,
                                      const float* __restrict__ pos, float* __restrict__ x, int Np, int D) {
  const int t = blockIdx.x, b = blockIdx.y, N = Np + 1;
  float* xr = x + ((size_t)b * N + t) * D;
  for (int d = threadIdx.x; d < D; d += blockDim.x) {
    const float v = (t == 0) ? cls[d] : tok[((size_t)b * Np + t - 1) * D + d] + bp[d];
    xr[d] = v + pos[(size_t)t * D + d];
  }
}

template <typename TOUT = bf16_t>
__global__ void patch_gather_grad_kernel(const float* __restrict__ dx, TOUT* __restrict__ out, int Np, int D) {
  const int p = blockIdx.x, b = blockIdx.y;
  const float* src = dx + ((size_t)b * (Np + 1) + 1 + p) * D;
  TOUT* o = out + ((size_t)b * Np + p) * D;
  for (int d = 2 * threadIdx.x; d < D; d += 2 * blockDim.x) {
    if constexpr (sizeof(TOUT) == 4) *reinterpret_cast<float2*>(o + d) = make_float2(src[d], src[d + 1]);
    else *reinterpret_cast<uint32_t*>(o + d) = pack_bf2(src[d], src[d + 1]);
  }
}

extern "C" int srhip_layernorm_fwd(const float* x, const float* gamma, const float* beta, float eps, void* out,
                                   float* mean, float* rstd, int M, int D, void* stream) {
  if (M <= 0 || (D != 128 && D != 384 && D != 512 && D != 768) || ((mean == nullptr) != (rstd == nullptr))) return SR_EINVAL;
  hipStream_t s = (hipStream_t)stream;
  dim3 grid(cdiv(M, 8)), block(256);
  if (D == 128) SR_LAUNCH(ln_fwd_kernel<1>, grid, block, 0, s, x, gamma, beta, eps, (bf16_t*)out, mean, rstd, M);
  else if (D == 512) SR_LAUNCH(ln_fwd_kernel<4>, grid, block, 0, s, x, gamma, beta, eps, (bf16_t*)out, mean, rstd, M);
  else if (D == 384) SR_LAUNCH(ln_fwd_kernel<3>, grid, block, 0, s, x, gamma, beta, eps, (bf16_t*)out, mean, rstd, M);
  else SR_LAUNCH(ln_fwd_kernel<6>, grid, block, 0, s, x, gamma, beta, eps, (bf16_t*)out, mean, rstd, M);
  SR_CHECK_LAUNCH();
  return SR_OK;
}

extern "C" int srhip_layernorm_fwd_f32(const float* x, const float* gamma, const float* beta, float eps, float* out,
                                       float* mean, float* rstd, int M, int D, void* stream) {
  if (!x || !out || M <= 0 || (D != 128 && D != 384 && D != 512 && D != 768) || ((mean == nullptr) != (rstd == nullptr))) return SR_EINVAL;
  hipStream_t s = (hipStream_t)stream;
  dim3 grid(cdiv(M, 8)), block(256);
  if (D == 128) SR_LAUNCH((ln_fwd_kernel<1, float>), grid, block, 0, s, x, gamma, beta, eps, out, mean, rstd, M);
  else if (D == 512) SR_LAUNCH((ln_fwd_kernel<4, float>), grid, block, 0, s, x, gamma, beta, eps, out, mean, rstd, M);
  else if (D == 384) SR_LAUNCH((ln_fwd_kernel<3, float>), grid, block, 0, s, x, gamma, beta, eps, out, mean, rstd, M);
  else SR_LAUNCH((ln_fwd_kernel<6, float>), grid, block, 0, s, x, gamma, beta, eps, out, mean, rstd, M);
  SR_CHECK_LAUNCH();
  return SR_OK;
}

static int layernorm_bwd_impl(const void* dy, const float* x, const float* mean, const float* rstd, const float* gamma, float* dx, float* dgamma,
                              float* dbeta, void* out_bf16, const float* row_scale, int rows_per_sample, int M, int D, void* stream,
                              float* part = nullptr, int n_rep = 0) {
  if (M <= 0 || (D != 128 && D != 384 && D != 512 && D != 768) || (row_scale && rows_per_sample <= 0)) return SR_EINVAL;
  hipStream_t s = (hipStream_t)stream;
  static const int rpw_env = SR_TUNE_ENV("SRHIP_LNB_RPW") ? atoi(SR_TUNE_ENV("SRHIP_LNB_RPW")) : 0;
  const bool small = rpw_env ? rpw_env == 2 : M < 16384;
  dim3 grid(cdiv(M, small ? 8 : 32)), block(256);
  const int rps = rows_per_sample > 0 ? rows_per_sample : 1;
#define LNB(NV)                                                                                                                                   \
  do {                                                                                                                                            \
    if (small) SR_LAUNCH((ln_bwd_kernel<NV, 2>), grid, block, 0, s, (const bf16_t*)dy, x, mean, rstd, gamma, dx, dgamma, dbeta, M,        \
                                  (bf16_t*)out_bf16, row_scale, rps, part, n_rep);                                                                             \
    else SR_LAUNCH((ln_bwd_kernel<NV, 8>), grid, block, 0, s, (const bf16_t*)dy, x, mean, rstd, gamma, dx, dgamma, dbeta, M,              \
                            (bf16_t*)out_bf16, row_scale, rps, part, n_rep);                                                                                   \
  } while (0)
  if (D == 128) LNB(1); else if (D == 512) LNB(4); else if (D == 384) LNB(3); else LNB(6);
#undef LNB
// ... 97 lines not shown
  if ((feat_all || logits_all) && !out_rows) return SR_EINVAL;
  SR_LAUNCH(cls_head_fwd_kernel, dim3(B, C >= 32 ? 4 : 1), dim3(256), (D + 4) * sizeof(float), (hipStream_t)stream, x, gamma, beta, eps,
                     Wh, bh, feat, logits, xhat, rstd, feat_all, logits_all, out_rows, N, D, C);
  SR_CHECK_LAUNCH();
  return SR_OK;
}

extern "C" int srhip_cls_head_bwd(const float* dlogits, const float* Wh, const float* gamma, const float* feat,
                                  const float* xhat, const float* rstd, float* dx, float* dWh, float* dbh, float* dgamma,
                                  float* dbeta, int B, int N, int D, int C, void* stream) {
  if (B <= 0 || D > 1024 || C <= 0 || (!dx && !dWh) || !dlogits) return SR_EINVAL;
  if (dx && (!Wh || !gamma || !xhat || !rstd || !dgamma || !dbeta)) return SR_EINVAL;
  if (dWh && (!dbh || !feat)) return SR_EINVAL;
  hipStream_t s = (hipStream_t)stream;
  if (dx) {
    SR_LAUNCH(cls_head_bwd_x_kernel, dim3(B), dim3(256), (C + 4) * sizeof(float), s, dlogits, Wh, gamma, xhat, rstd, dx,
                       dgamma, dbeta, N, D, C);
    SR_CHECK_LAUNCH();
  }
  if (dWh) {
    SR_LAUNCH(cls_head_bwd_w_kernel, dim3(C), dim3(256), 0, s, dlogits, feat, dWh, dbh, B, D, C);
    SR_CHECK_LAUNCH();
  }
  return SR_OK;
}

extern "C" int srhip_cast_scale_rows(const float* x, const float* scale, int rows_per_sample, void* out, long M, int D,
                                     void* stream) {
  if (M <= 0 || D % 8 || (scale && rows_per_sample <= 0)) return SR_EINVAL;
  const size_t n8 = (size_t)M * D / 8;
  SR_LAUNCH(cast_scale_rows_kernel, dim3(cdiv(n8, 256)), dim3(256), 0, (hipStream_t)stream, x, scale,
                     rows_per_sample > 0 ? rows_per_sample : 1, (bf16_t*)out, n8, D);
  SR_CHECK_LAUNCH();
  return SR_OK;
}

extern "C" int srhip_transpose_to_bf16(const void* in, int in_is_f32, int ld_in, void* out, int ld_out, int M, int Mp, int C,
                                       int apply_gelu, float* colsum, void* stream) {
  if (M <= 0 || Mp < M || (Mp % 2) || (C % 64) || ld_out < Mp || (ld_out % 2)) return SR_EINVAL;
  dim3 grid(cdiv(Mp, 64), C / 64), block(256);
  hipStream_t s = (hipStream_t)stream;
  if (in_is_f32) {
    if (apply_gelu) return SR_EINVAL;
    SR_LAUNCH((transpose_kernel<float, false>), grid, block, 0, s, (const float*)in, ld_in, (bf16_t*)out, ld_out, M, Mp, colsum);
  } else if (apply_gelu) {
    SR_LAUNCH((transpose_kernel<bf16_t, true>), grid, block, 0, s, (const bf16_t*)in, ld_in, (bf16_t*)out, ld_out, M, Mp, colsum);
  } else {
    SR_LAUNCH((transpose_kernel<bf16_t, false>), grid, block, 0, s, (const bf16_t*)in, ld_in, (bf16_t*)out, ld_out, M, Mp, colsum);
  }
  SR_CHECK_LAUNCH();
  return SR_OK;
}

extern "C" int srhip_cast_f32_bf16(const float* x, void* out, long n, void* stream) {
  if (n <= 0) return SR_EINVAL;
  SR_LAUNCH(cast_f32_bf16_kernel, dim3(cdiv(cdiv(n, 4), 256)), dim3(256), 0, (hipStream_t)stream, x, (bf16_t*)out, (size_t)n);
  SR_CHECK_LAUNCH();
  return SR_OK;
}

extern "C" int srhip_droppath_fill(float* out, const float* probs, int depth, int B, unsigned long long seed, void* stream) {
  if (depth <= 0 || B <= 0) return SR_EINVAL;
  SR_LAUNCH(droppath_fill_kernel, dim3(cdiv((long)depth * 2 * B, 256)), dim3(256), 0, (hipStream_t)stream, out, probs, depth, B, seed,
                     (const long long*)nullptr, B, (const unsigned long long*)nullptr);
  SR_CHECK_LAUNCH();
  return SR_OK;
}
extern "C" int srhip_droppath_fill_cols(float* out, const float* probs, const long long* cols, int depth, int B, int n_cols,
                                        unsigned long long seed, void* stream) {
  if (depth <= 0 || B <= 0 || n_cols <= 0 || !cols) return SR_EINVAL;
  SR_LAUNCH(droppath_fill_kernel, dim3(cdiv((long)depth * 2 * n_cols, 256)), dim3(256), 0, (hipStream_t)stream, out, probs, depth, B, seed,
                     cols, n_cols, (const unsigned long long*)nullptr);
  SR_CHECK_LAUNCH();
  return SR_OK;
}
extern "C" int srhip_droppath_fill_cols_dyn(float* out, const float* probs, const long long* cols, int depth, int B, int n_cols,
                                            const unsigned long long* seed_dev, unsigned long long seed_offset, void* stream) {
  if (depth <= 0 || B <= 0 || n_cols <= 0 || !seed_dev) return SR_EINVAL;
  SR_LAUNCH(droppath_fill_kernel, dim3(cdiv((long)depth * 2 * n_cols, 256)), dim3(256), 0, (hipStream_t)stream, out, probs, depth, B, seed_offset,
                     cols, cols ? n_cols : B, seed_dev);
  SR_CHECK_LAUNCH();
  return SR_OK;
}

extern "C" int srhip_transpose_batched(const srhip_transpose_desc* desc_dev, int n, int total_tiles, void* stream) {
  if (!desc_dev || n <= 0 || total_tiles <= 0) return SR_EINVAL;
  SR_LAUNCH(transpose_batched_kernel, dim3(total_tiles), dim3(256), 0, (hipStream_t)stream, desc_dev, n);
  SR_CHECK_LAUNCH();
  return SR_OK;
}

extern "C" int srhip_patch_im2col(const float* img, const int* img_index, void* out, int B, int C, int HW, int ps, void* stream) {
  if (!img || !out || B <= 0 || C <= 0 || ps <= 0 || (ps & 1) || HW % ps) return SR_EINVAL;
  const int gw = HW / ps;
  SR_LAUNCH(patch_im2col_kernel<bf16_t>, dim3(gw * gw, B), dim3(256), 0, (hipStream_t)stream, img, img_index, (bf16_t*)out, C, HW, ps);
  SR_CHECK_LAUNCH();
  return SR_OK;
}

extern "C" int srhip_patch_im2col_f32(const float* img, const int* img_index, float* out, int B, int C, int HW, int ps, void* stream) {
  if (!img || !out || B <= 0 || C <= 0 || ps <= 0 || (ps & 1) || HW % ps) return SR_EINVAL;
  const int gw = HW / ps;
  SR_LAUNCH(patch_im2col_kernel<float>, dim3(gw * gw, B), dim3(256), 0, (hipStream_t)stream, img, img_index, out, C, HW, ps);
  SR_CHECK_LAUNCH();
  return SR_OK;
}

extern "C" int srhip_patch_assemble(const float* tok, const float* bp, const float* cls, const float* pos, float* x, int B, int Np,
                                    int D, void* stream) {
  if (!tok || !bp || !cls || !pos || !x || B <= 0 || Np <= 0 || D <= 0) return SR_EINVAL;
  SR_LAUNCH(patch_assemble_kernel, dim3(Np + 1, B), dim3(D < 256 ? 64 : 256), 0, (hipStream_t)stream, tok, bp, cls, pos, x, Np, D);
  SR_CHECK_LAUNCH();
  return SR_OK;
}

extern "C" int srhip_patch_grad_operands(const float* dx, void* dx_tok_bf16, float* dpos, float* dcls, int B, int Np, int D,
                                         void* stream) {
  if (!dx || !dx_tok_bf16 || !dpos || !dcls || B <= 0 || Np <= 0 || D <= 0 || (D & 1) || D > 1024) return SR_EINVAL;
  hipStream_t s = (hipStream_t)stream;
  SR_LAUNCH(patch_embed_bwd_pos_kernel, dim3(Np + 1), dim3(D), 0, s, dx, dpos, dcls, B, Np + 1, D);
  SR_CHECK_LAUNCH();
  SR_LAUNCH(patch_gather_grad_kernel<bf16_t>, dim3(Np, B), dim3(D < 512 ? 64 : 256), 0, s, dx, (bf16_t*)dx_tok_bf16, Np, D);
  SR_CHECK_LAUNCH();
  return SR_OK;
}

extern "C" int srhip_patch_grad_operands_f32(const float* dx, float* dx_tok, float* dpos, float* dcls, int B, int Np, int D, void* stream) {
  if (!dx || !dx_tok || !dpos || !dcls || B <= 0 || Np <= 0 || D <= 0 || (D & 1) || D > 1024) return SR_EINVAL;
  hipStream_t s = (hipStream_t)stream;
  SR_LAUNCH(patch_embed_bwd_pos_kernel, dim3(Np + 1), dim3(D), 0, s, dx, dpos, dcls, B, Np + 1, D);
  SR_CHECK_LAUNCH();
  SR_LAUNCH(patch_gather_grad_kernel<float>, dim3(Np, B), dim3(D < 512 ? 64 : 256), 0, s, dx, dx_tok, Np, D);
  SR_CHECK_LAUNCH();
  return SR_OK;
}

extern "C" int srhip_layernorm_bwd_part_f32(const float* dy, const float* x, const float* mean, const float* rstd, const float* gamma, float* dx,
                                            float* part, int n_rep, float* out, const float* row_scale, int rows_per_sample, int M, int D,
                                            void* stream) {
  if (!dy || !part || n_rep <= 0 || M <= 0 || (D != 128 && D != 384 && D != 512 && D != 768) || (row_scale && rows_per_sample <= 0))
    return SR_EINVAL;
  hipStream_t s = (hipStream_t)stream;
  const bool small = M < 16384;
  dim3 grid(cdiv(M, small ? 8 : 32)), block(256);
  const int rps = rows_per_sample > 0 ? rows_per_sample : 1;
#define LNB(NV)                                                                                                                          \
  do {                                                                                                                                   \
    if (small) SR_LAUNCH((ln_bwd_kernel<NV, 2, float>), grid, block, 0, s, dy, x, mean, rstd, gamma, dx, (float*)nullptr, (float*)nullptr, M, \
                         out, row_scale, rps, part, n_rep);                                                                              \
    else SR_LAUNCH((ln_bwd_kernel<NV, 8, float>), grid, block, 0, s, dy, x, mean, rstd, gamma, dx, (float*)nullptr, (float*)nullptr, M,     \
                   out, row_scale, rps, part, n_rep);                                                                                    \
  } while (0)
  if (D == 128) LNB(1); else if (D == 512) LNB(4); else if (D == 384) LNB(3); else LNB(6);
#undef LNB
  SR_CHECK_LAUNCH();
  return SR_OK;
}
```

semireward_amd/nets/vit.py:

```python
import math
import types

import numpy as np
import torch

from .. import ops
from .pretrained import load_checkpoint
from .surface import ModuleSurface


class VitConfig:
    def __init__(self, img_size=224, patch_size=16, in_chans=3, num_classes=1000, embed_dim=768, depth=12,
                 num_heads=12, mlp_ratio=4.0, drop_path_rate=0.0, eps=1e-6):
        self.img_size, self.patch_size, self.in_chans, self.num_classes = img_size, patch_size, in_chans, num_classes
        self.embed_dim, self.depth, self.num_heads, self.mlp_ratio = embed_dim, depth, num_heads, mlp_ratio
        self.drop_path_rate, self.eps = drop_path_rate, eps
        assert embed_dim % num_heads == 0 and embed_dim // num_heads == 64, "libsrhip attention is built for head_dim 64"
        assert embed_dim in (128, 384, 768)

    @property
    def num_tokens(self):
        return (self.img_size // self.patch_size) ** 2 + 1

    @property
    def hidden(self):
        return int(self.embed_dim * self.mlp_ratio)


def param_names_shapes(cfg):
    D, Hd, p, C = cfg.embed_dim, cfg.hidden, cfg.patch_size, cfg.num_classes
    out = [("cls_token", (1, 1, D)), ("pos_embed", (1, cfg.num_tokens, D)),
           ("patch_embed.proj.weight", (D, cfg.in_chans, p, p)), ("patch_embed.proj.bias", (D,))]
    for i in range(cfg.depth):
        b = "blocks.%d." % i
        out += [(b + "norm1.weight", (D,)), (b + "norm1.bias", (D,)),
                (b + "attn.qkv.weight", (3 * D, D)), (b + "attn.qkv.bias", (3 * D,)),
                (b + "attn.proj.weight", (D, D)), (b + "attn.proj.bias", (D,)),
                (b + "norm2.weight", (D,)), (b + "norm2.bias", (D,)),
                (b + "mlp.fc1.weight", (Hd, D)), (b + "mlp.fc1.bias", (Hd,)),
                (b + "mlp.fc2.weight", (D, Hd)), (b + "mlp.fc2.bias", (D,))]
    out += [("norm.weight", (D,)), ("norm.bias", (D,)), ("head.weight", (C, D)), ("head.bias", (C,))]
    return out


DW_GROUPS = 3
LN_REP = 16
_FUSED_MLP = True
_FUSED_ATTN = True
_FUSED_PROJ = True
_FUSED_NEXT_LN = True
_LAST_BLOCK_CLASS_ROWS = True
_FUSED_MLP_MIN_ROWS = 16384


def _fused_mlp(cfg, rows):
    Hd = cfg.hidden
    return cfg.embed_dim == 384 and Hd % 128 == 0 and Hd <= 4096 and rows >= _FUSED_MLP_MIN_ROWS and _FUSED_MLP


def launch_kernels(cfg, n_images, kernels_as_images=None, precision="bf16"):
    if precision == "bf16x3":
        return ("bf16x3",)
    D, N, H, Hd = cfg.embed_dim, cfg.num_tokens, cfg.num_heads, cfg.hidden
    M = n_images * N
    fused = _fused_mlp(cfg, max(M, (kernels_as_images or 0) * N))
    fused_attn = _FUSED_ATTN and ops.attn_block_supported(N, D, H)
    gemms = []
    if cfg.in_chans * cfg.patch_size ** 2 > 64:
        gemms.append((ops.EPI_F32, n_images * (N - 1), D, cfg.in_chans * cfg.patch_size ** 2))
    if not fused_attn:
        gemms.append((ops.EPI_BF16, M, 3 * D, D))
    if not (fused and _FUSED_PROJ):
        gemms.append((ops.EPI_RESID_F32, M, D, D))
    if not fused:
        gemms += [(ops.EPI_GELU_BF16, M, Hd, D), (ops.EPI_RESID_F32, M, D, Hd)]
    return (fused, fused_attn) + tuple(ops.gemm_nt_plan(e, m, n, k) for e, m, n, k in gemms)


def droppath_keep_host(probs, depth, B, seed, cols=None):
    p = np.asarray(probs, dtype=np.float32)[:depth]
    col = np.arange(B, dtype=np.int64) if cols is None else np.asarray(cols, dtype=np.int64)
    col = np.where((col < 0) | (col >= B), 0, col)
    i = (np.arange(2 * depth, dtype=np.int64)[:, None] * B + col[None, :]).astype(np.uint64)
    with np.errstate(over="ignore"):
        z = np.uint64(int(seed) & 0xFFFFFFFFFFFFFFFF) + np.uint64(0x9E3779B97F4A7C15) * (i + np.uint64(1))
        z = (z ^ (z >> np.uint64(30))) * np.uint64(0xBF58476D1CE4E5B9)
        z = (z ^ (z >> np.uint64(27))) * np.uint64(0x94D049BB133111EB)
        z ^= z >> np.uint64(31)
    u = (z >> np.uint64(40)).astype(np.float32) * np.float32(1.0 / 16777216.0)
    pp = np.repeat(p, 2)[:, None]
    keep = (pp <= np.float32(0)) | (u < (np.float32(1.0) - pp))
    return keep.reshape(depth, 2, col.shape[0])


class FwdContext:
    __slots__ = ("B", "img", "img_index", "dp", "xs", "xmid", "ln1", "ln2", "qkv", "ao", "lse", "pre", "h", "st1", "st2",
                 "feat", "xhat", "rstd", "precision")


class VisionTransformer(ModuleSurface):
    GEMM_WEIGHTS = ("attn.qkv.weight", "attn.proj.weight", "mlp.fc1.weight", "mlp.fc2.weight")
    rows_independent = True
    scatter_outputs = True
    droppath_by_cols = True
    precise_rows = True
    precise_grad_rows = True
    pass_prefix_sharing = True
    lazy_transposed = True

    def __init__(self, cfg=None, device="cuda", **kw):
        self.cfg = cfg if cfg is not None else VitConfig(**kw)
        cfg = self.cfg
        self.device = torch.device(device)
        self._init_block(param_names_shapes(cfg), align=1, bf16=True)
        self.grad_ready_cb = None
        self.grad_rows_precision = "bf16"
        self.wT = {}
        for i in range(cfg.depth):
            for w in self.GEMM_WEIGHTS:
                n = "blocks.%d.%s" % (i, w)
                r, c = self.offsets[n][1]
                self.wT[n] = torch.zeros(c, r, dtype=torch.bfloat16, device=self.device)
        self.dp_probs_host = torch.linspace(0, cfg.drop_path_rate, cfg.depth)
        self.dp_probs = self.dp_probs_host.to(self.device)
        self.last_droppath_seed = None
        self._rng_calls = 0
        self.seed = 0

    def init_weights(self, seed=0):
        g = torch.Generator(device="cpu").manual_seed(seed)
        sd, fan = {}, {}
        for n, s_ in self.names_shapes:
            if n in ("cls_token", "pos_embed"):
                sd[n] = torch.zeros(s_)
# ... 11 lines not shown
        for n, t in self.wT.items():
            r, c = self.offsets[n][1]
            items.append((self.p(n), True, c, t, r, r, r, c, False))
        return items

    def no_weight_decay(self):
        return {"pos_embed", "cls_token"}

    def make_droppath(self, B, cols=None):
        dp = torch.empty(self.cfg.depth, 2, B if cols is None else cols.numel(), dtype=torch.float32, device=self.device)
        self._rng_calls += 1
        self.last_droppath_seed = ((self.seed << 32) + self._rng_calls) & 0xFFFFFFFFFFFFFFFF
        sc = getattr(self, "step_scalars", None)
        if sc is not None:
            self._step_draws = getattr(self, "_step_draws", 0) + 1
            ops.droppath_fill(dp, self.dp_probs, self.cfg.depth, B, self._step_draws, cols=cols, seed_dev=sc.seed_ptr)
        else:
            ops.droppath_fill(dp, self.dp_probs, self.cfg.depth, B, (self.seed << 32) + self._rng_calls, cols=cols)
        return dp

    def _ctx_buffers(self, B, precision="bf16"):
        key = ("ctx" if precision == "bf16" else "ctx3", B)
        if key in self._buf_cache:
            return self._buf_cache[key]
        cfg = self.cfg
        D, N, H, Hd = cfg.embed_dim, cfg.num_tokens, cfg.num_heads, cfg.hidden
        M = B * N
        f32 = torch.float32
        act = torch.bfloat16 if precision == "bf16" else f32
        mk = lambda shape, dt: [torch.empty(shape, dtype=dt, device=self.device) for _ in range(cfg.depth)]
        ctx = FwdContext()
        ctx.precision = precision
        ctx.xs = mk((M, D), f32) + [torch.empty(M, D, dtype=f32, device=self.device)]
        ctx.xmid, ctx.ln1, ctx.ln2 = mk((M, D), f32), mk((M, D), act), mk((M, D), act)
        ctx.qkv, ctx.ao, ctx.pre = mk((M, 3 * D), act), mk((M, D), act), mk((M, Hd), act)
        ctx.h = mk((M, Hd), act)
        ctx.lse = mk((B, H, N), f32)
        ctx.st1 = [(t[0], t[1]) for t in mk((2, M), f32)]
        ctx.st2 = [(t[0], t[1]) for t in mk((2, M), f32)]
        ctx.xhat = torch.empty(B, D, dtype=f32, device=self.device)
        ctx.rstd = torch.empty(B, dtype=f32, device=self.device)
        self._buf_cache[key] = ctx
        return ctx

    def forward_features(self, img, img_index=None, droppath=None, save=False, B=None, buftag="", out=None, precision="bf16",
                         kernels_as_images=None, tree=None):
        if tree is not None:
            assert not save and out is not None, "a pass-prefix tree is for rows without a backward that write the step's tables"
        if precision == "bf16x3":
            if save:
                assert self.grad_rows_precision == "bf16x3", "a bf16x3 forward with saved activations needs model.grad_rows_precision = 'bf16x3'"
            return self._forward_x3(img, img_index, droppath, B, buftag, out, tree, save)
        if precision != "bf16":
            raise ValueError("precision must be 'bf16' or 'bf16x3', got %r" % (precision,))
        cfg = self.cfg
        D, N, H, Hd = cfg.embed_dim, cfg.num_tokens, cfg.num_heads, cfg.hidden
        B = tree.n if tree is not None else (int(img_index.numel()) if img_index is not None else (B or img.shape[0]))
        M = B * N
        Mk = max(M, (kernels_as_images or 0) * N)
        gp = dict(plan_M=M) if tree is not None else {}
        f32, bf16 = torch.float32, torch.bfloat16
        tag = ("s" if save else "i") + buftag
        ctx = None
        if save:
            ctx = self._ctx_buffers(B)
            ctx.B, ctx.img, ctx.img_index, ctx.dp = B, img, img_index, droppath
            x = ctx.xs[0]
        else:
            x = self._buf(tag + "x", (M, D), f32)
            ln = self._buf(tag + "ln", (M, D), bf16)
            qkv = self._buf(tag + "qkv", (M, 3 * D), bf16)
            ao = self._buf(tag + "ao", (M, D), bf16)
        fused_mlp = (not save) and _fused_mlp(cfg, Mk)
        hbuf = None if (fused_mlp or save) else self._buf(tag + "h", (M, Hd), bf16)
        fused_attn = (not save) and _FUSED_ATTN and ops.attn_block_supported(N, D, H)
        qkvx = self._buf(tag + "qkvx", (B, 3 * D), bf16) if (fused_attn and N == 257) else None
        wb = self.flat_bf16
        P = self.p
        Be, idx_e = (tree.U, tree.uimg_dev) if tree is not None else (B, img_index)
        self._patch_embed(img, idx_e, x, Be, B, tag, "bf16", B * (N - 1) if tree is not None else None)
        scale = 64 ** -0.5
        dst0, dst1 = (droppath.stride(0), droppath.stride(1)) if droppath is not None else (0, 0)
        ln_ready = False
        for i in range(cfg.depth):
            b = "blocks.%d." % i
            if tree is not None:
                fk = tree.forks[i]
                if fk is not None:
                    ops.vit_fork(x, ln if ln_ready else None, fk[0], fk[1], fk[2], N, D)
                B = tree.level_n[i]
                M = B * N
                tree.launched.append(B)
            s1 = ops.RawRows(droppath, i * dst0) if droppath is not None else None
            s2 = ops.RawRows(droppath, i * dst0 + dst1) if droppath is not None else None
            if save:
                ln, qkv, ao = ctx.ln1[i], ctx.qkv[i], ctx.ao[i]
                ops.layernorm_fwd(x, P(b + "norm1.weight"), P(b + "norm1.bias"), cfg.eps, ln, ctx.st1[i][0], ctx.st1[i][1], M, D)
            elif not ln_ready:
                ops.layernorm_fwd(x, P(b + "norm1.weight"), P(b + "norm1.bias"), cfg.eps, ln, None, None, M, D)
            ao_scaled = False
            if fused_attn:
                ao_scaled = fused_mlp and _FUSED_PROJ and s1 is not None
                ops.attn_block_fused(ln, P(b + "attn.qkv.weight", wb), P(b + "attn.qkv.bias"), ao, B, N, D, H, scale, qkv_extra=qkvx,
                                     out_scale=s1 if ao_scaled else None)
            else:
                ops.gemm_nt(ops.EPI_BF16, ln, P(b + "attn.qkv.weight", wb), qkv, M, 3 * D, D, bias=P(b + "attn.qkv.bias"), **gp)
                ops.attn_fwd(qkv, ao, ctx.lse[i] if save else None, B, N, H, scale)
            if save:
                xm = ctx.xmid[i]
                ops.gemm_nt(ops.EPI_RESID_F32, ao, P(b + "attn.proj.weight", wb), xm, M, D, D, bias=P(b + "attn.proj.bias"),
                            row_scale=s1, rows_per_sample=N, aux_in=x, ldaux=D)
                ln2 = ctx.ln2[i]
                ops.layernorm_fwd(xm, P(b + "norm2.weight"), P(b + "norm2.bias"), cfg.eps, ln2, ctx.st2[i][0], ctx.st2[i][1], M, D)
                ops.gemm_nt(ops.EPI_GELU_BF16, ln2, P(b + "mlp.fc1.weight", wb), ctx.h[i], M, Hd, D, bias=P(b + "mlp.fc1.bias"),
                            aux_out=ctx.pre[i], ldaux=Hd)
                xn = ctx.xs[i + 1]
                ops.gemm_nt(ops.EPI_RESID_F32, ctx.h[i], P(b + "mlp.fc2.weight", wb), xn, M, D, Hd, bias=P(b + "mlp.fc2.bias"),
                            row_scale=s2, rows_per_sample=N, aux_in=xm, ldaux=D)
                x = xn
            elif fused_mlp and _FUSED_PROJ:
                nb = "blocks.%d." % (i + 1)
                ln_ready = _FUSED_NEXT_LN and i + 1 < cfg.depth
                class_rows = _LAST_BLOCK_CLASS_ROWS and i == cfg.depth - 1
                rps, rows, pitch = (1, B, N * D) if class_rows else (N, M, None)
                ops.mlp_fused_proj(x, ao, P(b + "attn.proj.weight", wb), P(b + "attn.proj.bias"), s1, P(b + "norm2.weight"),
                                   P(b + "norm2.bias"), cfg.eps, P(b + "mlp.fc1.weight", wb), P(b + "mlp.fc1.bias"),
                                   P(b + "mlp.fc2.weight", wb), P(b + "mlp.fc2.bias"), s2, rps, rows, D, Hd,
                                   ln_next=ln if ln_ready else None, next_gamma=P(nb + "norm1.weight") if ln_ready else None,
                                   next_beta=P(nb + "norm1.bias") if ln_ready else None, ao_scaled=ao_scaled, row_pitch=pitch)
            else:
                ops.gemm_nt(ops.EPI_RESID_F32, ao, P(b + "attn.proj.weight", wb), x, M, D, D, bias=P(b + "attn.proj.bias"),
                            row_scale=s1, rows_per_sample=N, **gp)
                if fused_mlp:
                    ops.mlp_fused(x, P(b + "norm2.weight"), P(b + "norm2.bias"), cfg.eps, P(b + "mlp.fc1.weight", wb),
                                  P(b + "mlp.fc1.bias"), P(b + "mlp.fc2.weight", wb), P(b + "mlp.fc2.bias"), s2, N, M, D, Hd)
                else:
                    ops.layernorm_fwd(x, P(b + "norm2.weight"), P(b + "norm2.bias"), cfg.eps, ln, None, None, M, D)
                    ops.gemm_nt(ops.EPI_GELU_BF16, ln, P(b + "mlp.fc1.weight", wb), hbuf, M, Hd, D, bias=P(b + "mlp.fc1.bias"), **gp)
                    ops.gemm_nt(ops.EPI_RESID_F32, hbuf, P(b + "mlp.fc2.weight", wb), x, M, D, Hd, bias=P(b + "mlp.fc2.bias"),
                                row_scale=s2, rows_per_sample=N, **gp)
        return self._head(x, B, out, ctx, tree, tag)

    def _patch_embed(self, img, idx, x, Be, B, tag, precision, plan_M=None):
        cfg = self.cfg
        D, Np, Kp = cfg.embed_dim, cfg.num_tokens - 1, cfg.in_chans * cfg.patch_size ** 2
        P = self.p
        if Kp <= 64:
            ops.patch_embed_fwd(img, idx, P("patch_embed.proj.weight"), P("patch_embed.proj.bias"), P("cls_token"),
                                P("pos_embed"), x, Be, cfg.in_chans, cfg.img_size, cfg.patch_size, D)
            return
        x3 = precision == "bf16x3"
        col = self._buf(tag + "col", (B * Np, Kp), torch.float32 if x3 else torch.bfloat16)
        tok = self._buf(tag + "tok", (B * Np, D), torch.float32)
        if x3:
            ops.patch_im2col_f32(img, idx, col, Be, cfg.in_chans, cfg.img_size, cfg.patch_size)
            ops.gemm_nt_x3(ops.X3_EPI_F32, col, P("patch_embed.proj.weight"), tok, Be * Np, D, Kp)
        else:
            ops.patch_im2col(img, idx, col, Be, cfg.in_chans, cfg.img_size, cfg.patch_size)
            ops.gemm_nt(ops.EPI_F32, col, P("patch_embed.proj.weight", self.flat_bf16), tok, Be * Np, D, Kp, plan_M=plan_M)
        ops.patch_assemble(tok, P("patch_embed.proj.bias"), P("cls_token"), P("pos_embed"), x, Be, Np, D)

    def _head(self, x, B, out, ctx, tree, tag):
        cfg = self.cfg
        D, N, C = cfg.embed_dim, cfg.num_tokens, cfg.num_classes
        P = self.p
        f32 = torch.float32
        feat = logits = xhat = rstd = None
        if tree is not None:
            feat, logits = self._buf(tag + "tfeat", (tree.n, D), f32), self._buf(tag + "tlogits", (tree.n, C), f32)
        elif ctx is not None or out is None:
            feat, logits = torch.empty(B, D, dtype=f32, device=self.device), torch.empty(B, C, dtype=f32, device=self.device)
        if ctx is not None:
            ctx.feat, xhat, rstd = feat, ctx.xhat, ctx.rstd
        if out is not None and tree is None:
            logits_all, feats_all, rows = out
            ops.cls_head_fwd_scatter(x, P("norm.weight"), P("norm.bias"), cfg.eps, P("head.weight"), P("head.bias"), feat, logits, xhat, rstd,
                                     feats_all, logits_all, rows, B, N, D, C)
        else:
            ops.cls_head_fwd(x, P("norm.weight"), P("norm.bias"), cfg.eps, P("head.weight"), P("head.bias"), feat, logits, xhat, rstd, B, N, D, C)
        if tree is not None:
            logits_all, feats_all, rows = out
            ops.vit_fanout(logits, feat, B, tree.col_node_dev, rows, tree.n, logits_all, feats_all, C, D)
            return None, None, None
        return logits, feat, ctx

    def _forward_x3(self, img, img_index, droppath, B, buftag, out, tree=None, save=False):
        cfg = self.cfg
        D, N, H, Hd = cfg.embed_dim, cfg.num_tokens, cfg.num_heads, cfg.hidden
        B = tree.n if tree is not None else (int(img_index.numel()) if img_index is not None else (B or img.shape[0]))
        M = B * N
        f32 = torch.float32
        ctx = None
        if save:
            tag = "q"
            ctx = self._ctx_buffers(B, "bf16x3")
            ctx.B, ctx.img, ctx.img_index, ctx.dp = B, img, img_index, droppath
            x = ctx.xs[0]
        else:
            tag = "p" + buftag
            x = self._buf(tag + "x", (M, D), f32)
            ln = ln2 = self._buf(tag + "ln", (M, D), f32)
            ao = self._buf(tag + "ao", (M, D), f32)
            wide = self._buf(tag + "wide", (M * max(3 * D, Hd),), f32)
            qkv, hbuf = wide[:M * 3 * D].view(M, 3 * D), wide[:M * Hd].view(M, Hd)
            st1 = st2 = (None, None)
        P = self.p
        Be, idx_e = (tree.U, tree.uimg_dev) if tree is not None else (B, img_index)
        self._patch_embed(img, idx_e, x, Be, B, tag, "bf16x3")
        scale = 64 ** -0.5
        dst0, dst1 = (droppath.stride(0), droppath.stride(1)) if droppath is not None else (0, 0)
        for i in range(cfg.depth):
            b = "blocks.%d." % i
# ... 266 lines not shown
```

semireward_amd/ops.py:

```python
import collections
import ctypes
import os

import torch

from . import _lib
from ._lib import EPI_BF16, EPI_DGELU_BF16, EPI_F32, EPI_GELU_BF16, EPI_RESID_F32
from ._lib import X3_EPI_F32, X3_EPI_GELU_F32, X3_EPI_RESID_F32
from ._lib import X3B_NT, X3B_NN, X3B_EPI_F32, X3B_EPI_ACC, X3B_EPI_DGELU, X3B_EPI_GELU_PRE
from ._lib import REDUCE_NONE, REDUCE_MEAN, REDUCE_SUM


_CHECK_ARGS = os.environ.get("SRHIP_CHECK_ARGS", "0") != "0"


def _p_checked(t):
    if t is None:
        return None
    assert t.is_cuda and t.is_contiguous(), "libsrhip needs contiguous device tensors"
    return t.data_ptr()


def _p_fast(t):
    return None if t is None else t.data_ptr()
# ... 396 lines not shown
    return bool(lib().srhip_attn_block_supported(N, D, H))


def attn_block_fused(xn, Wqkv, bqkv, out, B, N, D, H, scale, qkv_extra=None, out_scale=None):
    if N == 257:
        gemm_nt(EPI_BF16, xn[256:], Wqkv, qkv_extra, B, 3 * D, D, lda=N * D, bias=bqkv)
    if _PROFILE is not None:
        M = B * N
        _PROFILE.timed("srhip_attn_block_fused", (_p(xn), _p(Wqkv), _p(bqkv), _p(qkv_extra), _p(out), _p(out_scale), B, N, D, H, scale, _s(),), 2.0 * M * 3 * D * D + 4.0 * B * H * N * N * 64, "attn_block_kernel<%d>" % N,
                              2.0 * M * D + 2.0 * M * D + 2.0 * 3 * D * D)
        return
    _call("srhip_attn_block_fused", _p(xn), _p(Wqkv), _p(bqkv), _p(qkv_extra), _p(out), _p(out_scale), B, N, D, H, scale, _s())


AttnPlan = collections.namedtuple("AttnPlan", "nkt fwd_pair bwd_l2 bwd_split")


def attn_plan(B, N, H):
    v = [ctypes.c_int(0) for _ in range(4)]
    rc = int(_lib.lib().srhip_attn_plan(B, N, H, *[ctypes.addressof(x) for x in v]))
    if rc != 0:
        _lib.check(rc, "srhip_attn_plan")
    return AttnPlan(v[0].value, bool(v[1].value), bool(v[2].value), v[3].value)


def attn_fwd(qkv, out, lse, B, N, H, scale):
    if _PROFILE is not None:
        _PROFILE.timed("srhip_attn_fwd", (_p(qkv), _p(out), _p(lse), B, N, H, scale, _s()), 4.0 * B * H * N * N * 64, "attn_fwd_kernel",
                       2.0 * B * N * 4 * H * 64)
        return
    _call("srhip_attn_fwd", _p(qkv), _p(out), _p(lse), B, N, H, scale, _s())


def attn_bwd(qkv, out, d_out, lse, dqkv, delta_ws, B, N, H, scale):
    if _PROFILE is not None:
        _PROFILE.timed("srhip_attn_bwd", (_p(qkv), _p(out), _p(d_out), _p(lse), _p(dqkv), _p(delta_ws), B, N, H, scale, _s()),
                       10.0 * B * H * N * N * 64, "attn_bwd (dq + dkv kernels)", 2.0 * B * N * 8 * H * 64)
        return
    _call("srhip_attn_bwd", _p(qkv), _p(out), _p(d_out), _p(lse), _p(dqkv), _p(delta_ws), B, N, H, scale, _s())


def layernorm_fwd(x, gamma, beta, eps, out, mean, rstd, M, D):
    _call("srhip_layernorm_fwd", _p(x), _p(gamma), _p(beta), eps, _p(out), _p(mean), _p(rstd), M, D, _s())


def layernorm_bwd_cast(dy, x, mean, rstd, gamma, dx, dgamma, dbeta, out_bf16, row_scale, rows_per_sample, M, D):
    _call("srhip_layernorm_bwd_cast", _p(dy), _p(x), _p(mean), _p(rstd), _p(gamma), _p(dx), _p(dgamma), _p(dbeta), _p(out_bf16), _p(row_scale),
          rows_per_sample, M, D, _s())


def layernorm_bwd_part(dy, x, mean, rstd, gamma, dx, part, n_rep, out_bf16, row_scale, rows_per_sample, M, D):
    if _PROFILE is not None:
        _PROFILE.timed("srhip_layernorm_bwd_part", (_p(dy), _p(x), _p(mean), _p(rstd), _p(gamma), _p(dx), _p(part), n_rep, _p(out_bf16),
                                                    _p(row_scale), rows_per_sample, M, D, _s()), 0.0, "ln_bwd_kernel", 16.0 * M * D)
        return
    _call("srhip_layernorm_bwd_part", _p(dy), _p(x), _p(mean), _p(rstd), _p(gamma), _p(dx), _p(part), n_rep, _p(out_bf16), _p(row_scale),
          rows_per_sample, M, D, _s())


def make_ln_reduce_desc(pairs, device):
    import numpy as np
    arr = np.array([[_p(g), _p(b)] for g, b in pairs], dtype=np.uint64)
    desc = torch.from_numpy(arr.view(np.uint8).copy()).to(device)
    desc.out_ranges = [(_p(t), t.numel() * t.element_size()) for pair in pairs for t in pair]
    return desc


def ln_grad_reduce(desc, part, n_ln, n_rep, D):
    _call("srhip_ln_grad_reduce", _p(desc), _p(part), n_ln, n_rep, D, _s())


def mlp_fused(x, gamma, beta, eps, W1, b1, W2, b2, row_scale, rows_per_sample, M, D, Hd, x_out=None, save=None):
    rows, ln2, pre, h, mean, rstd = save if save is not None else (0, None, None, None, None, None)
    args = (_p(x), _p(x_out if x_out is not None else x), _p(gamma), _p(beta), eps, _p(W1), _p(b1), _p(W2), _p(b2), _p(row_scale),
            rows_per_sample, rows, _p(ln2), _p(pre), _p(h), _p(mean), _p(rstd), M, D, Hd)
    if _PROFILE is not None:
        _PROFILE.timed("srhip_mlp_fused", (*args, _s(),), 4.0 * M * D * Hd, "mlp_fused_kernel<384, 0, 4>",
                              8.0 * M * D + 4.0 * D * Hd + rows * (2.0 * D + 4.0 * Hd))
        return
    _call("srhip_mlp_fused", *args, _s())


def mlp_fused_proj(x, ao, Wp, bp, row_scale1, gamma, beta, eps, W1, b1, W2, b2, row_scale2, rows_per_sample, M, D, Hd, x_out=None,
                   ln_next=None, next_gamma=None, next_beta=None, ao_scaled=False, row_pitch=None):
    args = (_p(x), _p(x_out if x_out is not None else x), _p(ao), _p(Wp), _p(bp), _p(row_scale1), int(bool(ao_scaled)), _p(gamma), _p(beta), eps,
            _p(W1), _p(b1),
            _p(W2), _p(b2), _p(row_scale2), rows_per_sample, _p(ln_next), _p(next_gamma), _p(next_beta), M, D, Hd)
    if _PROFILE is not None:
        nbytes = 8.0 * M * D + 2.0 * M * D + (2.0 * M * D if ln_next is not None else 0.0) + 4.0 * D * Hd + 2.0 * D * D
        if row_pitch is not None:
            _PROFILE.timed("srhip_mlp_fused_proj_strided", (*args, int(row_pitch), _s(),), 4.0 * M * D * Hd + 2.0 * M * D * D,
                           "mlp_fused_kernel<384, 0, 4, true, 1> class rows", nbytes)
            return
        _PROFILE.timed("srhip_mlp_fused_proj", (*args, _s(),), 4.0 * M * D * Hd + 2.0 * M * D * D, "mlp_fused_kernel<384, 0, 4, true, 1>", nbytes)
        return
    if row_pitch is not None:
        _call("srhip_mlp_fused_proj_strided", *args, int(row_pitch), _s())
        return
    _call("srhip_mlp_fused_proj", *args, _s())


def gelu_eval(x, y_erf, y_poly):
    _call("srhip_gelu_eval", _p(x), _p(y_erf), _p(y_poly), x.numel(), _s())


def layernorm_bwd(dy, x, mean, rstd, gamma, dx, dgamma, dbeta, M, D):
    _call("srhip_layernorm_bwd", _p(dy), _p(x), _p(mean), _p(rstd), _p(gamma), _p(dx), _p(dgamma), _p(dbeta), M, D, _s())


def patch_embed_fwd(img, img_index, Wp, bp, cls, pos, x, B, C, HW, ps, D):
    _call("srhip_patch_embed_fwd", _p(img), _p(img_index), _p(Wp), _p(bp), _p(cls), _p(pos), _p(x), B, C, HW, ps, D, _s())


def patch_embed_bwd(dx, img, img_index, dWp, dbp, dcls, dpos, B, C, HW, ps, D):
    _call("srhip_patch_embed_bwd", _p(dx), _p(img), _p(img_index), _p(dWp), _p(dbp), _p(dcls), _p(dpos), B, C, HW, ps, D, _s())


def patch_embed_bwd_ws_floats(B, C, HW, ps, D):
    n = int(_lib.lib().srhip_patch_embed_bwd_ws_floats(B, C, HW, ps, D))
    if n < 0:
        raise ValueError("srhip_patch_embed_bwd_ws refuses B=%d C=%d HW=%d ps=%d D=%d" % (B, C, HW, ps, D))
    return n


def patch_embed_bwd_ws(dx, img, img_index, dWp, dbp, dcls, dpos, ws, B, C, HW, ps, D, part_done=False):
    if part_done:
        _call("srhip_patch_embed_bwd_fold", _p(ws), _p(dWp), _p(dbp), B, C, HW, ps, D, _s())
        return
    _call("srhip_patch_embed_bwd_ws", _p(dx), _p(img), _p(img_index), _p(dWp), _p(dbp), _p(dcls), _p(dpos), _p(ws), B, C, HW, ps, D, _s())


def patch_im2col(img, img_index, out, B, C, HW, ps):
    _call("srhip_patch_im2col", _p(img), _p(img_index), _p(out), B, C, HW, ps, _s())


def patch_assemble(tok, bp, cls, pos, x, B, Np, D):
    _call("srhip_patch_assemble", _p(tok), _p(bp), _p(cls), _p(pos), _p(x), B, Np, D, _s())


def patch_grad_operands(dx, dx_tok, dpos, dcls, B, Np, D):
    _call("srhip_patch_grad_operands", _p(dx), _p(dx_tok), _p(dpos), _p(dcls), B, Np, D, _s())


def gemm_nt_x3(epi, A, W, C, M, N, K, *, lda=None, ldw=None, ldc=None, bias=None, row_scale=None, rows_per_sample=0):
    args = (epi, _p(A), lda or K, _p(W), ldw or K, _p(C), ldc or N, M, N, K, _p(bias), _p(row_scale), rows_per_sample, _s())
    if _PROFILE is not None:
        _PROFILE.timed("srhip_gemm_nt_x3", args, 2.0 * M * N * K, "gemm_nt_x3_kernel<%d>" % epi,
                       4.0 * (M * K + N * K) + 4.0 * M * N * (2 if epi == X3_EPI_RESID_F32 else 1))
        return
    _call("srhip_gemm_nt_x3", *args)


def attn_fwd_x3(qkv, out, B, N, H, scale):
    if _PROFILE is not None:
        _PROFILE.timed("srhip_attn_fwd_x3", (_p(qkv), _p(out), B, N, H, scale, _s()), 4.0 * B * H * N * N * 64, "attn_fwd_x3_kernel",
                       4.0 * B * N * 4 * H * 64)
        return
    _call("srhip_attn_fwd_x3", _p(qkv), _p(out), B, N, H, scale, _s())


def layernorm_fwd_f32(x, gamma, beta, eps, out, mean, rstd, M, D):
    _call("srhip_layernorm_fwd_f32", _p(x), _p(gamma), _p(beta), eps, _p(out), _p(mean), _p(rstd), M, D, _s())


def patch_im2col_f32(img, img_index, out, B, C, HW, ps):
    _call("srhip_patch_im2col_f32", _p(img), _p(img_index), _p(out), B, C, HW, ps, _s())


def attn_fwd_x3_lse(qkv, out, lse, B, N, H, scale):
    args = (_p(qkv), _p(out), _p(lse), B, N, H, scale, _s())
    if _PROFILE is not None:
        _PROFILE.timed("srhip_attn_fwd_x3_lse", args, 4.0 * B * H * N * N * 64, "attn_fwd_x3_lse_kernel", 4.0 * B * N * 4 * H * 64)
        return
    _call("srhip_attn_fwd_x3_lse", *args)


def gemm_x3(layout, epi, A, B, C, M, N, K, *, lda=None, ldb=None, ldc=None, bias=None, aux=None, aux_out=None, ldaux=0):
# ... 7 lines not shown
    _call("srhip_gemm_x3", *args)


def gemm_tn_x3_grouped(desc, n_problems, total_tiles, flops=0.0, nbytes=0.0):
    args = (_p(desc), n_problems, total_tiles, _s())
    if _PROFILE is not None:
        _PROFILE.timed("srhip_gemm_tn_x3_grouped", args, flops, "gemm_tn_x3_grouped_kernel", nbytes)
        return
    _call("srhip_gemm_tn_x3_grouped", *args)


def make_group_tn_x3_desc(problems, device):
    desc, n, tiles, flops, _ = make_group_tn_desc(problems, device)
    nbytes = float(sum(4.0 * (M * K + N * K) + 8.0 * M * N for *_, M, N, K in problems))
    return desc, n, tiles, flops, nbytes


def attn_bwd_x3(qkv, out, d_out, lse, dqkv, delta_ws, B, N, H, scale):
    args = (_p(qkv), _p(out), _p(d_out), _p(lse), _p(dqkv), _p(delta_ws), B, N, H, scale, _s())
    if _PROFILE is not None:
        _PROFILE.timed("srhip_attn_bwd_x3", args, 14.0 * B * H * N * N * 64, "attn_bwd_x3_kernels", 4.0 * B * N * H * 64 * 8)
        return
    _call("srhip_attn_bwd_x3", *args)


def layernorm_bwd_part_f32(dy, x, mean, rstd, gamma, dx, part, n_rep, out, row_scale, rows_per_sample, M, D):
    _call("srhip_layernorm_bwd_part_f32", _p(dy), _p(x), _p(mean), _p(rstd), _p(gamma), _p(dx), _p(part), n_rep, _p(out), _p(row_scale),
          rows_per_sample, M, D, _s())


def patch_grad_operands_f32(dx, dx_tok, dpos, dcls, B, Np, D):
    _call("srhip_patch_grad_operands_f32", _p(dx), _p(dx_tok), _p(dpos), _p(dcls), B, Np, D, _s())


def scale_rows_f32(x, scale, rows_per_sample, out, M, D):
    _call("srhip_scale_rows_f32", _p(x), _p(scale), rows_per_sample, _p(out), M, D, _s())


def cls_head_fwd_scatter(x, gamma, beta, eps, Wh, bh, feat, logits, xhat, rstd, feat_all, logits_all, out_rows, B, N, D, C):
    _call("srhip_cls_head_fwd_scatter", _p(x), _p(gamma), _p(beta), eps, _p(Wh), _p(bh), _p(feat), _p(logits), _p(xhat), _p(rstd), _p(feat_all),
          _p(logits_all), _p(out_rows), B, N, D, C, _s())


def cls_head_fwd(x, gamma, beta, eps, Wh, bh, feat, logits, xhat, rstd, B, N, D, C):
    _call("srhip_cls_head_fwd", _p(x), _p(gamma), _p(beta), eps, _p(Wh), _p(bh), _p(feat), _p(logits), _p(xhat), _p(rstd),
          B, N, D, C, _s())


def cls_head_bwd(dlogits, Wh, gamma, feat, xhat, rstd, dx, dWh, dbh, dgamma, dbeta, B, N, D, C):
    _call("srhip_cls_head_bwd", _p(dlogits), _p(Wh), _p(gamma), _p(feat), _p(xhat), _p(rstd), _p(dx), _p(dWh), _p(dbh),
          _p(dgamma), _p(dbeta), B, N, D, C, _s())


def cast_scale_rows(x, scale, rows_per_sample, out, M, D):
    _call("srhip_cast_scale_rows", _p(x), _p(scale), rows_per_sample, _p(out), M, D, _s())


def transpose_to_bf16(inp, in_is_f32, ld_in, out, ld_out, M, Mp, C, apply_gelu=False, colsum=None):
    _call("srhip_transpose_to_bf16", _p(inp), int(in_is_f32), ld_in, _p(out), ld_out, M, Mp, C, int(apply_gelu), _p(colsum), _s())


TRANSPOSE_DESC_DTYPE = [("in", "<u8"), ("out", "<u8"), ("in_is_f32", "<i4"), ("ld_in", "<i4"), ("ld_out", "<i4"), ("M", "<i4"),
                        ("Mp", "<i4"), ("C", "<i4"), ("apply_gelu", "<i4"), ("tile_start", "<i4"), ("pad", "<i8")]


def make_transpose_desc(items, device):
    import numpy as np
    arr = np.zeros(len(items), dtype=TRANSPOSE_DESC_DTYPE)
    t = 0
    for i, (inp, f32, ld_in, out, ld_out, M, Mp, C, gelu) in enumerate(items):
        assert C % 64 == 0 and Mp % 2 == 0 and Mp >= M
        arr[i] = (_p(inp), _p(out), int(f32), ld_in, ld_out, M, Mp, C, int(gelu), t, 0)
        t += ((Mp + 63) // 64) * (C // 64)
    assert arr.itemsize == 56
    return torch.from_numpy(arr.view(np.uint8).copy()).to(device), len(items), t


def transpose_batched(desc, n, total_tiles):
    _call("srhip_transpose_batched", _p(desc), n, total_tiles, _s())


def cast_f32_bf16(x, out, n):
    _call("srhip_cast_f32_bf16", _p(x), _p(out), n, _s())


def droppath_fill(out, probs, depth, B, seed, cols=None, seed_dev=None):
    if seed_dev is not None:
        _call("srhip_droppath_fill_cols_dyn", _p(out), _p(probs), _p(cols), depth, B, cols.numel() if cols is not None else B, seed_dev, seed, _s())
    elif cols is None:
        _call("srhip_droppath_fill", _p(out), _p(probs), depth, B, seed, _s())
    else:
        _call("srhip_droppath_fill_cols", _p(out), _p(probs), _p(cols), depth, B, cols.numel(), seed, _s())


def vit_fork(x, ln, parent, n_new, dst0, rows_per_node, D):
    _call("srhip_vit_fork", _p(x), _p(ln), _p(parent), n_new, dst0, rows_per_node, D, _s())


def vit_fanout(node_logits, node_feat, n_nodes, col_node, col_rows, n_cols, logits_all, feat_all, C, D):
    _call("srhip_vit_fanout", _p(node_logits), _p(node_feat), n_nodes, _p(col_node), _p(col_rows), n_cols, _p(logits_all), _p(feat_all),
          min(logits_all.shape[0], feat_all.shape[0]), C, D, _s())


def row_max(inp, in_is_probs, probs_out, max_probs, max_idx, B, C):
    _call("srhip_row_max", _p(inp), int(in_is_probs), _p(probs_out), _p(max_probs), _p(max_idx), B, C, _s())


def row_max_strided(base, first_row, in_is_probs, probs_out, max_probs, max_idx, B, C, rows_per_group, group_rows):
    _call("srhip_row_max_strided", _pa(base, first_row * C), int(in_is_probs), _p(probs_out), _p(max_probs), _p(max_idx), B, C, rows_per_group,
          group_rows * C, _s())


def flexmatch_mask(max_probs, max_idx, idx_ulb, p_cutoff, selected_label, hist, classwise_acc, mask, B, C, ulb_dest_len,
                   thresh_warmup):
    _call("srhip_flexmatch_mask", _p(max_probs), _p(max_idx), _p(idx_ulb), p_cutoff, _p(selected_label), _p(hist),
          _p(classwise_acc), _p(mask), B, C, ulb_dest_len, int(thresh_warmup), _s())


def flexmatch_mask_passes(max_probs, max_idx, idx_ulb, p_cutoff, selected_label, hist, classwise_acc, mask, n_pass, B, C, ulb_dest_len,
                          thresh_warmup):
    _call("srhip_flexmatch_mask_passes", _p(max_probs), _p(max_idx), _p(idx_ulb), p_cutoff, _p(selected_label), _p(hist),
          _p(classwise_acc), _p(mask), n_pass, B, C, ulb_dest_len, int(thresh_warmup), _s())


def flexmatch_rebuild_hist(selected_label, hist, ulb_dest_len, C):
    _call("srhip_flexmatch_rebuild_hist", _p(selected_label), _p(hist), ulb_dest_len, C, _s())


def fixed_mask(max_probs, p_cutoff, mask, B):
    _call("srhip_fixed_mask", _p(max_probs), p_cutoff, _p(mask), B, _s())


def freematch_stats(probs, max_idx, colsum, hist, B, C):
    _call("srhip_freematch_stats", _p(probs), _p(max_idx), _p(colsum), _p(hist), B, C, _s())


def freematch_update(maxp_all, n_all, colsum, hist, max_probs, max_idx, time_p, p_model, label_hist, mask, B, C, m, use_quantile, clip_thresh):
    import numpy as np
    _call("srhip_freematch_update", _p(maxp_all), n_all, _p(colsum), _p(hist), _p(max_probs), _p(max_idx), _p(time_p), _p(p_model),
          _p(label_hist), _p(mask), B, C, float(np.float32(m)), float(np.float32(1 - m)), int(use_quantile), int(clip_thresh), _s())


def distalign(probs, colsum_ulb, n_ulb, colsum_lb, n_lb, p_model, p_target, inited, momentum, aligned, max_probs, max_idx, B, C):
    _call("srhip_distalign", _p(probs), _p(colsum_ulb), n_ulb, _p(colsum_lb), n_lb, _p(p_model), _p(p_target), _p(inited), float(momentum),
          _p(aligned), _p(max_probs), _p(max_idx), B, C, _s())


def softmatch_mask(maxp_all, n_all, max_probs, mu_var, momentum, n_sigma, mask, B):
    _call("srhip_softmatch_mask", _p(maxp_all), n_all, _p(max_probs), _p(mu_var), float(momentum), int(n_sigma), _p(mask), B, _s())


def freematch_entropy(logits, mask, p_model, label_hist, grad_scale, loss_out, dlogits, ws, B, C, accumulate=False):
    _call("srhip_freematch_entropy", _p(logits), _p(mask), _p(p_model), _p(label_hist), grad_scale, _p(loss_out), _p(dlogits), _p(ws),
          B, C, int(accumulate), _s())


def reward_mask2(reward, mask2, mean_out, groups, B, mean_in=None, total=None):
    if total is not None and total != groups * B:
        assert mean_in is None and groups == -(-total // B)
        _call("srhip_reward_mask2_ragged", _p(reward), _p(mask2), _p(mean_out), total, B, _s())
        return
    _call("srhip_reward_mask2", _p(reward), _p(mask2), _p(mean_out), _p(mean_in), groups, B, _s())


def masked_ce(logits, targets, mask, mask2, grad_scale, loss_out, dlogits, B, C):
    _call("srhip_masked_ce", _p(logits), _p(targets), _p(mask), _p(mask2), grad_scale, _p(loss_out), _p(dlogits), B, C, _s())
# ... 667 lines not shown
```

Measured before the change: 1690.

## Skip compute for drop-path-dropped samples in fused attention and MLP kernels

Adds a device kernel that builds a per-block plan listing the samples whose drop-path MLP branch is kept. A new planned variant of the fused proj+MLP kernel uses that plan so it can skip the MLP work for dropped samples. The attention block kernel now writes zeros and exits early for images whose output scale is zero. This removes GEMM work for stochastically dropped residual branches, at the cost of an extra plan launch per forward, more complex kernel indexing, and possible load imbalance.

```diff
diff --git a/include/srhip.h b/include/srhip.h
--- a/include/srhip.h
+++ b/include/srhip.h
@@ -105,6 +105,10 @@
                                  int ao_scaled, const float* ln_gamma, const float* ln_beta, float eps, const void* W1, const float* b1,
                                  const void* W2, const float* b2, const float* row_scale2, int rows_per_sample, void* ln_next,
                                  const float* next_gamma, const float* next_beta, int M, int D, int Hd, int row_pitch, void* stream);
+int srhip_mlp_fused_proj_planned(const float* x, float* x_out, const void* ao, const void* Wp, const float* bp, const float* row_scale1,
+                                 int ao_scaled, const float* ln_gamma, const float* ln_beta, float eps, const void* W1, const float* b1,
+                                 const void* W2, const float* b2, const float* row_scale2, int rows_per_sample, void* ln_next,
+                                 const float* next_gamma, const float* next_beta, int M, int D, int Hd, const int* plan_row, int B, void* stream);
 
 int srhip_attn_block_supported(int N, int D, int H);
 int srhip_attn_block_fused(const void* xn_bf16, const void* Wqkv, const float* bqkv, const void* qkv_extra, void* out, const float* out_scale,
@@ -175,6 +179,7 @@
 int srhip_droppath_fill(float* out, const float* probs, int depth, int B, unsigned long long seed, void* stream);
 int srhip_droppath_fill_cols(float* out, const float* probs, const long long* cols, int depth, int B, int n_cols, unsigned long long seed,
                              void* stream);
+int srhip_vit_droppath_plan(const float* dp, long long stride_block, long long stride_branch, int depth, int B, int* plan, void* stream);
 
 int srhip_vit_fork(float* x, void* ln, const int* parent, int n_new, int dst0, int rows_per_node, int D, void* stream);
 int srhip_vit_fanout(const float* node_logits, const float* node_feat, int n_nodes, const int* col_node, const long long* col_rows,
diff --git a/semireward_amd/_lib.py b/semireward_amd/_lib.py
--- a/semireward_amd/_lib.py
+++ b/semireward_amd/_lib.py
@@ -43,6 +43,7 @@
     "srhip_gelu_eval": (I, [P, P, P, I, P]),
     "srhip_mlp_fused_proj": (I, [P, P, P, P, P, P, I, P, P, F, P, P, P, P, P, I, P, P, P, I, I, I, P]),
     "srhip_mlp_fused_proj_strided": (I, [P, P, P, P, P, P, I, P, P, F, P, P, P, P, P, I, P, P, P, I, I, I, I, P]),
+    "srhip_mlp_fused_proj_planned": (I, [P, P, P, P, P, P, I, P, P, F, P, P, P, P, P, I, P, P, P, I, I, I, P, I, P]),
     "srhip_adam_bias_corrections": (I, [F, F, I, P]),
     "srhip_adamw_flat_dyn": (I, [P, P, P, P, P, P, P, I, P, P, P, F, F, F, Dbl, F, P, I, P]),
     "srhip_adam_flat_dyn": (I, [P, P, P, P, L, F, F, F, F, P, P]),
@@ -73,6 +74,7 @@
     "srhip_transpose_batched": (I, [P, I, I, P]),
     "srhip_cast_f32_bf16": (I, [P, P, L, P]),
     "srhip_droppath_fill": (I, [P, P, I, I, c_ulonglong, P]),
+    "srhip_vit_droppath_plan": (I, [P, c_longlong, c_longlong, I, I, P, P]),
     "srhip_droppath_fill_cols": (I, [P, P, P, I, I, I, c_ulonglong, P]),
     "srhip_row_max": (I, [P, I, P, P, P, I, I, P]),
     "srhip_row_max_strided": (I, [P, I, P, P, P, I, I, I, c_longlong, P]),
diff --git a/semireward_amd/csrc/attn_block.hip b/semireward_amd/csrc/attn_block.hip
--- a/semireward_amd/csrc/attn_block.hip
+++ b/semireward_amd/csrc/attn_block.hip
@@ -89,6 +89,15 @@
   constexpr bool EXTRA = NQT == 17;
   static_assert(NQT <= 16 || (EXTRA && N == 257), "two token tiles per wave (+ one extra token)");
   constexpr int NKT_LO = (N - 1) / 16;
+  if (a.osc && a.osc[blockIdx.x] == 0.0f) {
+    const int hpw0 = NH / gridDim.y, cw = hpw0 * (HD / 8);
+    bf16_t* o = a.out + (size_t)blockIdx.x * N * DM + blockIdx.y * hpw0 * HD;
+    for (int i = threadIdx.x; i < N * cw; i += 512) {
+      const int r = i / cw, c = i - r * cw;
+      *reinterpret_cast<u32x4_t*>(o + (size_t)r * DM + 8 * c) = u32x4_t{0u, 0u, 0u, 0u};
+    }
+    return;
+  }
   extern __shared__ __attribute__((aligned(16))) bf16_t sm[];
   bf16_t* ring = sm;
   bf16_t* Ks = ring + NS * ST_EL;
@@ -102,7 +111,6 @@
   const float osc = a.osc ? a.osc[img] : 1.0f;
   const int hpw = NH / gridDim.y, hbeg = blockIdx.y * hpw, hend = hbeg + hpw;
   const size_t row0 = (size_t)img * N;
-
   const int rho = 8 * wave + (lane >> 3);
   const int srcc = (lane & 7) ^ ((rho >> 1) & 7);
   const int fperm = (rho & 32) + 8 * ((rho & 15) >> 2) + 4 * ((rho >> 4) & 1) + (rho & 3);
diff --git a/semireward_amd/csrc/mlp_fused.hip b/semireward_amd/csrc/mlp_fused.hip
--- a/semireward_amd/csrc/mlp_fused.hip
+++ b/semireward_amd/csrc/mlp_fused.hip
@@ -42,6 +42,8 @@
   float eps;
   int M, Hd, rows_per_sample;
   int pitch;
+  const int* plan;
+  int nsamp;
 };
 
 #ifdef SRHIP_TUNING
@@ -52,442 +54,14 @@
 #endif
 template <int D_, int DBG, int GS, bool PROJ = false, int SPREAD = 0, bool PITCH = false>
 __global__ __launch_bounds__(512, 2) void mlp_fused_kernel(MlpArgs a) {
-  static_assert(PROJ || !PITCH, "the row pitch belongs to the PROJ variant");
-  constexpr int KS1 = D_ / BK;
-  constexpr int KQ = 4;
-  constexpr int G1S = 2 * (KS1 / KQ);
-  constexpr int TH = D_ / RT;
-  constexpr int NT2 = D_ / 16;
-  constexpr int G2S = (CH / BK) * TH;
-  constexpr int SPC = G1S + G2S;
-  constexpr int NG = NS / GS;
-  constexpr int PD = (NG - 2) * GS;
-  static_assert(KS1 % KQ == 0 && D_ % RT == 0 && SPC % GS == 0 && NS % GS == 0 && NG >= 3, "layout");
-  extern __shared__ __attribute__((aligned(16))) bf16_t sm[];
-  float* sb1 = reinterpret_cast<float*>(sm + NS * TILE_EL);
-  float* sb2 = sb1 + a.Hd;
-  float* sgam = sb2 + D_;
-  float* sbet = sgam + D_;
-  float* sbp = sbet + D_;
-  float* sgn = sbp + D_;
-  float* sbn = sgn + D_;
-  const int tid = threadIdx.x, lane = tid & 63;
-  const int wave = __builtin_amdgcn_readfirstlane(tid >> 6);
-  const int l15 = lane & 15, lg = lane >> 4;
-  const int nch = a.Hd / CH;
-  for (int i = tid; i < a.Hd; i += 512) sb1[i] = a.b1[i];
-  for (int i = tid; i < D_; i += 512) { sb2[i] = a.b2[i]; sgam[i] = a.gamma[i]; sbet[i] = a.beta[i]; }
-  if constexpr (PROJ) {
-    for (int i = tid; i < D_; i += 512) sbp[i] = a.bp[i];
-    if (a.ln_next) for (int i = tid; i < D_; i += 512) { sgn[i] = a.gamma_n[i]; sbn[i] = a.beta_n[i]; }
-  }
-  __syncthreads();
-
-  const int pr = 16 * wave + (lane >> 2);
-  const int psl = ((lane & 3) ^ swz(pr)) * 8;
-  const int lo1 = ((pr & 31) * D_ + (pr >> 5) * BK + psl) * 2;
-  const int lo2 = (pr * a.Hd + psl) * 2;
-  const int pdst = 16 * wave * BK;
-  const int wbytes = a.Hd * D_ * 2;
-  const __amdgpu_buffer_rsrc_t r1 = __builtin_amdgcn_make_buffer_rsrc(const_cast<bf16_t*>(a.W1), 0, wbytes, 0x00020000);
-  const __amdgpu_buffer_rsrc_t r2 = __builtin_amdgcn_make_buffer_rsrc(const_cast<bf16_t*>(a.W2), 0, wbytes, 0x00020000);
-  constexpr int OOB = 0x7ffffff0;
-  constexpr int VOFF = PROJ ? TH : 0;
-  const int nchv = nch + VOFF;
-  const __amdgpu_buffer_rsrc_t rp = __builtin_amdgcn_make_buffer_rsrc(const_cast<bf16_t*>(PROJ ? a.Wp : a.W2), 0, D_ * D_ * 2, 0x00020000);
-  const int lop = (pr * D_ + psl) * 2;
-  auto issue = [&](int cv, int j, int slot) {
-    if (DBG & 2) return;
-    lds_void* dst = (lds_void*)(sm + slot * TILE_EL + pdst);
-    const bool valid = cv < nchv;
-    if (PROJ && cv < VOFF) {
-      __builtin_amdgcn_raw_ptr_buffer_load_lds(rp, dst, 16, lop, (cv * RT * D_ + j * BK) * 2, 0, 0);
-      return;
-    }
-    const int c = cv - VOFF;
-    if (j < G1S) {
-      const int u = j / (KS1 / KQ), kt = j % (KS1 / KQ);
-      __builtin_amdgcn_raw_ptr_buffer_load_lds(r1, dst, 16, valid ? lo1 : OOB, ((c * CH + 32 * u) * D_ + kt * KQ * BK) * 2, 0, 0);
-    } else {
-      const int jj = j - G1S, u = jj / TH, th = jj % TH;
-      __builtin_amdgcn_raw_ptr_buffer_load_lds(r2, dst, 16, valid ? lo2 : OOB, (th * RT * a.Hd + c * CH + u * BK) * 2, 0, 0);
-    }
-  };
-
-  const int fo2 = l15 * BK + ((lg ^ swz(l15)) << 3);
-  const int h1 = 8 * (l15 >> 2) + (l15 & 3);
-  const int fo1p = h1 * BK + ((lg ^ swz(h1)) << 3);
-  const int fo1q = (h1 + 4) * BK + ((lg ^ swz(h1 + 4)) << 3);
-
-  const size_t rpitch = PITCH ? (size_t)a.pitch : (size_t)D_;
-  const int ntiles = (a.M + FBM - 1) / FBM;
-  for (int tile = blockIdx.x; tile < ntiles; tile += gridDim.x) {
-    const int m = tile * FBM + wave * 16 + l15;
-    const int mc = min(m, a.M - 1);
-    MDBG_T(0);
-    u32x4_t xn[KS1];
-    if constexpr (!PROJ) {
-      const float* xr = a.x + (size_t)mc * D_ + 8 * lg;
-      f32x4_t v[2 * KS1];
-      float s = 0.f;
-#pragma unroll
-      for (int k = 0; k < KS1; ++k) {
-        v[2 * k] = *reinterpret_cast<const f32x4_t*>(xr + 32 * k);
-        v[2 * k + 1] = *reinterpret_cast<const f32x4_t*>(xr + 32 * k + 4);
-      }
-#pragma unroll
-      for (int k = 0; k < 2 * KS1; ++k) s += (v[k][0] + v[k][1]) + (v[k][2] + v[k][3]);
-      s += __shfl_xor(s, 16, 64);
-      s += __shfl_xor(s, 32, 64);
-      const float mu = s * (1.0f / D_);
-      float q = 0.f;
-#pragma unroll
-      for (int k = 0; k < 2 * KS1; ++k) {
-#pragma unroll
-        for (int e = 0; e < 4; ++e) { const float d = v[k][e] - mu; q += d * d; }
-      }
-      q += __shfl_xor(q, 16, 64);
-      q += __shfl_xor(q, 32, 64);
-      const float rs = rsqrtf(q * (1.0f / D_) + a.eps);
-      if (a.save_rows > 0 && m < a.save_rows && lg == 0) { a.s_mean[m] = mu; a.s_rstd[m] = rs; }
-#pragma unroll
-      for (int k = 0; k < KS1; ++k) {
-        const f32x4_t g0 = *reinterpret_cast<const f32x4_t*>(sgam + 32 * k + 8 * lg);
-        const f32x4_t g1 = *reinterpret_cast<const f32x4_t*>(sgam + 32 * k + 8 * lg + 4);
-        const f32x4_t b0 = *reinterpret_cast<const f32x4_t*>(sbet + 32 * k + 8 * lg);
-        const f32x4_t b1 = *reinterpret_cast<const f32x4_t*>(sbet + 32 * k + 8 * lg + 4);
-        const f32x4_t p = v[2 * k], r = v[2 * k + 1];
-        xn[k] = u32x4_t{pack_bf2((p[0] - mu) * rs * g0[0] + b0[0], (p[1] - mu) * rs * g0[1] + b0[1]),
-                        pack_bf2((p[2] - mu) * rs * g0[2] + b0[2], (p[3] - mu) * rs * g0[3] + b0[3]),
-                        pack_bf2((r[0] - mu) * rs * g1[0] + b1[0], (r[1] - mu) * rs * g1[1] + b1[1]),
-                        pack_bf2((r[2] - mu) * rs * g1[2] + b1[2], (r[3] - mu) * rs * g1[3] + b1[3])};
-        if (k & 1) __builtin_amdgcn_sched_barrier(0);
-      }
-    }
-    const bool save_tile = !PROJ && a.save_rows > 0 && tile * FBM + wave * 16 < a.save_rows;
-    if (save_tile && m < a.save_rows) {
-      bf16_t* lr = a.s_ln2 + (size_t)m * D_ + 8 * lg;
-#pragma unroll
-      for (int k = 0; k < KS1; ++k) *reinterpret_cast<u32x4_t*>(lr + 32 * k) = xn[k];
-    }
-    u32x4_t aof[PROJ ? KS1 : 1];
-    if constexpr (PROJ) {
-      const bf16_t* ar = a.ao + (size_t)mc * rpitch + 8 * lg;
-#pragma unroll
-      for (int k = 0; k < KS1; ++k) aof[k] = *reinterpret_cast<const u32x4_t*>(ar + 32 * k);
-    }
-    float rs1v = 1.0f, rs2v = 1.0f;
-    f32x4_t acc2[NT2];
-    if constexpr (PROJ) {
-      if (a.row_scale1) rs1v = a.row_scale1[mc / a.rows_per_sample];
-      if (a.row_scale) rs2v = a.row_scale[mc / a.rows_per_sample];
-      const float* xr = a.x + (size_t)mc * rpitch + 4 * lg;
-#pragma unroll
-      for (int t = 0; t < NT2; ++t) acc2[t] = *reinterpret_cast<const f32x4_t*>(xr + 16 * t);
-      if (rs1v != 1.0f && !a.ao_scaled) {
-#pragma unroll
-        for (int k = 0; k < KS1; ++k)
-#pragma unroll
-          for (int e = 0; e < 4; ++e)
-            aof[k][e] = pack_bf2(rs1v * __builtin_bit_cast(float, aof[k][e] << 16), rs1v * __builtin_bit_cast(float, aof[k][e] & 0xffff0000u));
-      }
-    }
-    __syncthreads();
-    MDBG_T(1);
-#pragma unroll
-    for (int p = 0; p < PD; ++p) issue(p / SPC, p % SPC, p);
-
-    __builtin_amdgcn_sched_barrier(0);
-    if constexpr (!PROJ) {
-#pragma unroll
-      for (int t = 0; t < NT2; ++t) acc2[t] = f32x4_t{0.f, 0.f, 0.f, 0.f};
-    } else {
-#pragma unroll
-      for (int t = 0; t < NT2; ++t) {
-        const f32x4_t bb = *reinterpret_cast<const f32x4_t*>(sbp + 16 * t + 4 * lg);
-        acc2[t][0] += rs1v * bb[0]; acc2[t][1] += rs1v * bb[1]; acc2[t][2] += rs1v * bb[2]; acc2[t][3] += rs1v * bb[3];
-      }
-    }
-    f32x4_t acc1[4];
-    u32x4_t hf[2];
-    u32x4_t fa0[4], fa1[4];
-
-    auto sync_group = [&](auto jc, int c) __attribute__((always_inline)) {
-      constexpr int j = decltype(jc)::value;
-      static_assert(j % GS == 0, "group start");
-      if constexpr ((DBG & 2) == 0) wait_vm<GS*(NG - 3)>();
-      __builtin_amdgcn_s_barrier();
-      if constexpr (!SPREAD) {
-#pragma unroll
-        for (int i = 0; i < GS; ++i) {
-          const int jn = (j + PD + i) % SPC, cn = c + (j + PD + i) / SPC;
-          issue(cn, jn, (c * SPC + j + PD + i) & (NS - 1));
-        }
-      }
-    };
-    auto issue_ahead = [&](auto jc, int c, bool late) __attribute__((always_inline)) {
-      constexpr int j = decltype(jc)::value;
-      if constexpr (SPREAD == 1) { if (!late) issue(c + (j + PD) / SPC, (j + PD) % SPC, (c * SPC + j + PD) & (NS - 1)); }
-    };
-    auto read_half = [&](auto jc, auto hc, int c) __attribute__((always_inline)) {
-      constexpr int j = decltype(jc)::value, h = decltype(hc)::value;
-      u32x4_t(&fa)[4] = h ? fa1 : fa0;
-      const bf16_t* st = sm + ((c * SPC + j) & (NS - 1)) * TILE_EL;
-      if constexpr ((DBG & 4) != 0) {
-#pragma unroll
-        for (int t = 0; t < 4; ++t) fa[t] = u32x4_t{(unsigned)(c + t), 1u, 2u, (unsigned)j};
-      } else if constexpr (j < G1S) {
-#pragma unroll
-        for (int s_ = 0; s_ < 2; ++s_) {
-          fa[2 * s_] = *reinterpret_cast<const u32x4_t*>(st + fo1p + (2 * h + s_) * 32 * BK);
-          fa[2 * s_ + 1] = *reinterpret_cast<const u32x4_t*>(st + fo1q + (2 * h + s_) * 32 * BK);
-        }
-      } else {
-#pragma unroll
-        for (int t = 0; t < 4; ++t) fa[t] = *reinterpret_cast<const u32x4_t*>(st + fo2 + (4 * h + t) * 16 * BK);
-      }
-    };
-    float gcarry = 0.f, pcarry = 0.f;
-    auto acc1_start = [&](auto uc, auto xc, int c) __attribute__((always_inline)) {
-      constexpr int u = decltype(uc)::value, X = decltype(xc)::value;
-      acc1[2 * u + X] = *reinterpret_cast<const f32x4_t*>(sb1 + min(c - VOFF, nch - 1) * CH + 32 * u + 8 * lg + 4 * X);
-    };
-    auto gelu_elem = [&](auto uc, auto ec, int c) __attribute__((always_inline)) {
-      constexpr int u = decltype(uc)::value, e = decltype(ec)::value, X = e >> 2, r = e & 3;
-      const float v = acc1[2 * u + X][r];
-      if constexpr (PROJ && (DBG & 1) == 0) {
-        if constexpr ((e & 1) == 1) {
-          const f32x2_t g2 = gelu_poly2(f32x2_t{acc1[2 * u + X][r - 1], v}) * f32x2_t{rs2v, rs2v};
-          hf[u][e >> 1] = pack_bf2(g2[0], g2[1]);
-        }
-      } else {
-      float gv;
-      if constexpr ((DBG & 1) != 0) gv = v; else gv = gelu_erf(v);
-      if constexpr (PROJ) gv *= rs2v;
-      if constexpr ((e & 1) == 0) { gcarry = gv; pcarry = v; } else hf[u][e >> 1] = pack_bf2(gcarry, gv);
-      }
-      if constexpr ((e & 1) == 1) {
-        if (save_tile && m < a.save_rows) {
-          const size_t o = (size_t)m * a.Hd + (c - VOFF) * CH + 32 * u + 8 * lg + (e - 1);
-          *reinterpret_cast<uint32_t*>(a.s_pre + o) = pack_bf2(pcarry, v);
-          *reinterpret_cast<uint32_t*>(a.s_h + o) = hf[u][e >> 1];
-        }
-      }
-      if constexpr (r == 3) acc1_start(uc, std::integral_constant<int, X>{}, c + 1);
-    };
-    auto gelu_slot = [&](auto jc, auto hc, auto pc, int c) __attribute__((always_inline)) {
-      constexpr int j = decltype(jc)::value, h = decltype(hc)::value, part = decltype(pc)::value;
-      if constexpr (j >= 3 && j <= 8 && (DBG & 8) == 0) {
-        constexpr int u = (j - 3) / 3, q = 2 * ((j - 3) % 3) + h;
-        constexpr int first[7] = {0, 2, 3, 4, 6, 7, 8};
-        constexpr int e0 = first[q], n = first[q + 1] - first[q];
-        if constexpr (part < n) gelu_elem(std::integral_constant<int, u>{}, std::integral_constant<int, e0 + part>{}, c);
-      }
-    };
-    auto mfma_one = [&](auto jc, auto hc, auto tc) __attribute__((always_inline)) {
-      constexpr int j = decltype(jc)::value, h = decltype(hc)::value, t = decltype(tc)::value;
-      u32x4_t(&fa)[4] = h ? fa1 : fa0;
-      if constexpr ((DBG & 8) != 0) {
-        asm volatile("" ::"v"(fa[t]));
-        if constexpr (j == G1S - 1) { hf[0] = fa[0]; hf[1] = fa[1]; }
-      } else if constexpr (j < G1S) {
-        constexpr int u = j / (KS1 / KQ), kt = j % (KS1 / KQ);
-        acc1[2 * u + (t & 1)] = __builtin_amdgcn_mfma_f32_16x16x32_bf16(
-            __builtin_bit_cast(bf16x8_t, fa[t]), __builtin_bit_cast(bf16x8_t, xn[kt * KQ + 2 * h + (t >> 1)]), acc1[2 * u + (t & 1)],
-            0, 0, 0);
-      } else {
-        constexpr int u = (j - G1S) / TH, th = (j - G1S) % TH;
-        acc2[th * 8 + 4 * h + t] = __builtin_amdgcn_mfma_f32_16x16x32_bf16(
-            __builtin_bit_cast(bf16x8_t, fa[t]), __builtin_bit_cast(bf16x8_t, hf[u]), acc2[th * 8 + 4 * h + t], 0, 0, 0);
-      }
-    };
-    auto mfma_half = [&](auto jc, auto hc, int c) __attribute__((always_inline)) {
-      using T0 = std::integral_constant<int, 0>;
-      using T1 = std::integral_constant<int, 1>;
-      using T2 = std::integral_constant<int, 2>;
-      using T3 = std::integral_constant<int, 3>;
-      mfma_one(jc, hc, T0{});
-      mfma_one(jc, hc, T1{});
-      __builtin_amdgcn_sched_barrier(0);
-      gelu_slot(jc, hc, T0{}, c);
-      __builtin_amdgcn_sched_barrier(0);
-      mfma_one(jc, hc, T2{});
-      mfma_one(jc, hc, T3{});
-      __builtin_amdgcn_sched_barrier(0);
-      gelu_slot(jc, hc, T1{}, c);
-      __builtin_amdgcn_sched_barrier(0);
-    };
-    using H0 = std::integral_constant<int, 0>;
-    using H1 = std::integral_constant<int, 1>;
-    if constexpr (PROJ) {
-      auto read_half_p = [&](auto jc, auto hc, int cv) __attribute__((always_inline)) {
-        constexpr int j = decltype(jc)::value, h = decltype(hc)::value;
-        u32x4_t(&fa)[4] = h ? fa1 : fa0;
-        const bf16_t* st = sm + ((cv * SPC + j) & (NS - 1)) * TILE_EL;
-#pragma unroll
-        for (int t = 0; t < 4; ++t) fa[t] = *reinterpret_cast<const u32x4_t*>(st + fo2 + (4 * h + t) * 16 * BK);
-      };
-      sync_group(H0{}, 0);
-      read_half_p(H0{}, H0{}, 0);
-      static_for<VOFF>([&](auto vc) __attribute__((always_inline)) {
-        constexpr int v = decltype(vc)::value;
-        static_for<SPC>([&](auto jc) __attribute__((always_inline)) {
-          constexpr int j = decltype(jc)::value;
-          constexpr int jn = (j + 1) % SPC, vn = v + (j + 1) / SPC;
-          read_half_p(jc, H1{}, v);
-#pragma unroll
-          for (int t = 0; t < 4; ++t)
-            acc2[v * 8 + t] = __builtin_amdgcn_mfma_f32_16x16x32_bf16(__builtin_bit_cast(bf16x8_t, fa0[t]), __builtin_bit_cast(bf16x8_t, aof[j]),
-                                                                       acc2[v * 8 + t], 0, 0, 0);
-          __builtin_amdgcn_sched_barrier(0);
-          issue_ahead(jc, v, false);
-          if constexpr (jn % GS == 0) sync_group(std::integral_constant<int, jn>{}, vn);
-          if constexpr (vn == VOFF) read_half(std::integral_constant<int, 0>{}, H0{}, vn);
-          else read_half_p(std::integral_constant<int, jn>{}, H0{}, vn);
-#pragma unroll
-          for (int t = 0; t < 4; ++t)
-            acc2[v * 8 + 4 + t] = __builtin_amdgcn_mfma_f32_16x16x32_bf16(__builtin_bit_cast(bf16x8_t, fa1[t]), __builtin_bit_cast(bf16x8_t, aof[j]),
-                                                                           acc2[v * 8 + 4 + t], 0, 0, 0);
-          __builtin_amdgcn_sched_barrier(0);
-          issue_ahead(jc, v, true);
-        });
-      });
-      MDBG_T(4);
-      {
-        float sum = 0.f;
-#pragma unroll
-        for (int t = 0; t < NT2; ++t) sum += (acc2[t][0] + acc2[t][1]) + (acc2[t][2] + acc2[t][3]);
-        const float mu = rows_sum4(sum) * (1.0f / D_);
-        float q = 0.f;
-#pragma unroll
-        for (int t = 0; t < NT2; ++t)
-#pragma unroll
-          for (int e = 0; e < 4; ++e) { const float d = acc2[t][e] - mu; q += d * d; }
-        const float rs = rsqrtf(rows_sum4(q) * (1.0f / D_) + a.eps);
-        int ko = 4 * lg;
-        asm volatile("" : "+v"(ko) : "v"(rs));
-#pragma unroll
-        for (int sI = 0; sI < KS1; ++sI) {
-          if (sI > 0) asm volatile("" : "+v"(ko) : "v"(xn[sI - 1][3]));
-          unsigned pk[2][2];
-#pragma unroll
-          for (int e = 0; e < 2; ++e) {
-            const int t = 2 * sI + e;
-            const f32x4_t g4 = *reinterpret_cast<const f32x4_t*>(sgam + 16 * t + ko);
-            const f32x4_t b4 = *reinterpret_cast<const f32x4_t*>(sbet + 16 * t + ko);
-            pk[e][0] = pack_bf2((acc2[t][0] - mu) * rs * g4[0] + b4[0], (acc2[t][1] - mu) * rs * g4[1] + b4[1]);
-            pk[e][1] = pack_bf2((acc2[t][2] - mu) * rs * g4[2] + b4[2], (acc2[t][3] - mu) * rs * g4[3] + b4[3]);
-          }
-          unsigned out4[4];
-#pragma unroll
-          for (int d = 0; d < 2; ++d) {
-            const auto w32 = __builtin_amdgcn_permlane32_swap(pk[0][d], pk[1][d], false, false);
-            const auto w16 = __builtin_amdgcn_permlane16_swap(w32[0], w32[1], false, false);
-            out4[d] = w16[0];
-            out4[2 + d] = w16[1];
-          }
-          xn[sI] = u32x4_t{out4[0], out4[1], out4[2], out4[3]};
-          if (sI & 1) __builtin_amdgcn_sched_barrier(0);
-        }
-      }
-      MDBG_T(5);
-#pragma unroll
-      for (int t = 0; t < NT2; ++t) {
-        const f32x4_t bb = *reinterpret_cast<const f32x4_t*>(sb2 + 16 * t + 4 * lg);
-        acc2[t][0] += rs2v * bb[0]; acc2[t][1] += rs2v * bb[1]; acc2[t][2] += rs2v * bb[2]; acc2[t][3] += rs2v * bb[3];
-      }
-    }
-    {
-      using I0 = std::integral_constant<int, 0>;
-      using I1 = std::integral_constant<int, 1>;
-      acc1_start(I0{}, I0{}, VOFF); acc1_start(I0{}, I1{}, VOFF); acc1_start(I1{}, I0{}, VOFF); acc1_start(I1{}, I1{}, VOFF);
-    }
-    if constexpr (!PROJ) {
-      sync_group(H0{}, 0);
-      read_half(H0{}, H0{}, 0);
-    }
-    for (int c = VOFF; c < nchv; ++c)
-      static_for<SPC>([&](auto jc) __attribute__((always_inline)) {
-        constexpr int j = decltype(jc)::value;
-        constexpr int jn = (j + 1) % SPC;
-        const int cn = c + (j + 1) / SPC;
-        read_half(jc, H1{}, c);
-        mfma_half(jc, H0{}, c);
-        issue_ahead(jc, c, false);
-        if constexpr (jn % GS == 0) sync_group(std::integral_constant<int, jn>{}, cn);
-        read_half(std::integral_constant<int, jn>{}, H0{}, cn);
-        mfma_half(jc, H1{}, c);
-        issue_ahead(jc, c, true);
-      });
-    MDBG_T(2);
-    if (PROJ && a.ln_next) {
-      float* xw = a.xo + (size_t)mc * rpitch + 4 * lg;
-      float sum = 0.f;
-#pragma unroll
-      for (int t = 0; t < NT2; ++t) {
-        const f32x4_t xv = acc2[t];
-        if (m < a.M) *reinterpret_cast<f32x4_t*>(xw + 16 * t) = xv;
-        sum += (xv[0] + xv[1]) + (xv[2] + xv[3]);
-      }
-      const float mu = rows_sum4(sum) * (1.0f / D_);
-      float q = 0.f;
-#pragma unroll
-      for (int t = 0; t < NT2; ++t)
-#pragma unroll
-        for (int e = 0; e < 4; ++e) { const float d = acc2[t][e] - mu; q += d * d; }
-      const float rs = rsqrtf(rows_sum4(q) * (1.0f / D_) + a.eps);
-      bf16_t* lw = a.ln_next + (size_t)mc * D_ + 8 * lg;
-      int ko = 4 * lg;
-      asm volatile("" : "+v"(ko) : "v"(rs));
-      unsigned chain = 0;
-#pragma unroll
-      for (int sI = 0; sI < KS1; ++sI) {
-        if (sI > 0) asm volatile("" : "+v"(ko) : "v"(chain));
-        unsigned pk[2][2];
-#pragma unroll
-        for (int e = 0; e < 2; ++e) {
-          const int t = 2 * sI + e;
-          const f32x4_t g4 = *reinterpret_cast<const f32x4_t*>(sgn + 16 * t + ko);
-          const f32x4_t b4 = *reinterpret_cast<const f32x4_t*>(sbn + 16 * t + ko);
-          pk[e][0] = pack_bf2((acc2[t][0] - mu) * rs * g4[0] + b4[0], (acc2[t][1] - mu) * rs * g4[1] + b4[1]);
-          pk[e][1] = pack_bf2((acc2[t][2] - mu) * rs * g4[2] + b4[2], (acc2[t][3] - mu) * rs * g4[3] + b4[3]);
-        }
-        unsigned out4[4];
-#pragma unroll
-        for (int d = 0; d < 2; ++d) {
-          const auto w32 = __builtin_amdgcn_permlane32_swap(pk[0][d], pk[1][d], false, false);
-          const auto w16 = __builtin_amdgcn_permlane16_swap(w32[0], w32[1], false, false);
-          out4[d] = w16[0];
-          out4[2 + d] = w16[1];
-        }
-        chain = out4[3];
-        if (m < a.M) *reinterpret_cast<u32x4_t*>(lw + 32 * sI) = u32x4_t{out4[0], out4[1], out4[2], out4[3]};
-      }
-    } else if (PROJ) {
-      float* xw = a.xo + (size_t)mc * rpitch + 4 * lg;
-      if (m < a.M) {
-#pragma unroll
-        for (int t = 0; t < NT2; ++t) *reinterpret_cast<f32x4_t*>(xw + 16 * t) = acc2[t];
-      }
-    } else if (m < a.M) {
-      const float rsc = a.row_scale ? a.row_scale[m / a.rows_per_sample] : 1.0f;
-      const float* xr = a.x + (size_t)m * D_ + 4 * lg;
-      float* xw = a.xo + (size_t)m * D_ + 4 * lg;
-#pragma unroll
-      for (int t = 0; t < NT2; ++t) {
-        const f32x4_t bb = *reinterpret_cast<const f32x4_t*>(sb2 + 16 * t + 4 * lg);
-        f32x4_t xv = *reinterpret_cast<const f32x4_t*>(xr + 16 * t);
-        xv[0] += rsc * (acc2[t][0] + bb[0]); xv[1] += rsc * (acc2[t][1] + bb[1]);
-        xv[2] += rsc * (acc2[t][2] + bb[2]); xv[3] += rsc * (acc2[t][3] + bb[3]);
-        *reinterpret_cast<f32x4_t*>(xw + 16 * t) = xv;
-      }
-    }
-#ifdef SRHIP_TUNING
-    __builtin_amdgcn_s_waitcnt(0);
-    __syncthreads();
-    MDBG_T(3);
-#endif
-  }
+  constexpr bool PLAN = false;
+#include "mlp_fused_body.h"
+}
+template <int D_, int GS>
+__global__ __launch_bounds__(512, 2) void mlp_planned_kernel(MlpArgs a) {
+  constexpr int DBG = 0, SPREAD = 1;
+  constexpr bool PROJ = true, PITCH = false, PLAN = true;
+#include "mlp_fused_body.h"
 }
 
 
@@ -531,7 +105,7 @@
   a.W1 = (const bf16_t*)W1; a.W2 = (const bf16_t*)W2; a.eps = eps; a.M = M; a.Hd = Hd;
   a.rows_per_sample = rows_per_sample > 0 ? rows_per_sample : 1;
   a.ao = nullptr; a.Wp = nullptr; a.bp = nullptr; a.row_scale1 = nullptr; a.ao_scaled = 0; a.ln_next = nullptr; a.gamma_n = a.beta_n = nullptr;
-  a.pitch = D;
+  a.pitch = D; a.plan = nullptr; a.nsamp = 0;
   const size_t smem = (size_t)NS * TILE_EL * sizeof(bf16_t) + (size_t)(Hd + 6 * D) * sizeof(float);
   void (*kern)(MlpArgs) = mlp_fused_kernel<384, 0, 4>;
 #ifdef SRHIP_TUNING
@@ -557,7 +131,7 @@
 static int mlp_fused_proj_launch(const float* x, float* x_out, const void* ao, const void* Wp, const float* bp, const float* row_scale1,
                                  int ao_scaled, const float* ln_gamma, const float* ln_beta, float eps, const void* W1, const float* b1, const void* W2,
                                  const float* b2, const float* row_scale2, int rows_per_sample, void* ln_next, const float* next_gamma,
-                                 const float* next_beta, int M, int D, int Hd, int row_pitch, void* stream) {
+                                 const float* next_beta, int M, int D, int Hd, int row_pitch, const int* plan, int nsamp, void* stream) {
   if (!x || !x_out || !ao || !Wp || !bp || !ln_gamma || !ln_beta || !W1 || !b1 || !W2 || !b2 || M <= 0) return SR_EINVAL;
   if (ln_next && (!next_gamma || !next_beta || ((uintptr_t)ln_next & 15))) return SR_EINVAL;
   if (D != 384 || Hd < 128 || (Hd % RT) || Hd > 4096) return SR_EINVAL;
@@ -571,10 +145,12 @@
   a.rows_per_sample = rows_per_sample > 0 ? rows_per_sample : 1;
   a.ao = (const bf16_t*)ao; a.Wp = (const bf16_t*)Wp; a.bp = bp; a.row_scale1 = row_scale1; a.ao_scaled = ao_scaled;
   a.ln_next = (bf16_t*)ln_next; a.gamma_n = next_gamma; a.beta_n = next_beta; a.pitch = row_pitch ? row_pitch : D;
+  a.plan = plan; a.nsamp = nsamp;
   const size_t smem = (size_t)NS * TILE_EL * sizeof(bf16_t) + (size_t)(Hd + 6 * D) * sizeof(float);
   static const int spread = SR_TUNE_ENV("SRHIP_MLP_SPREAD") ? atoi(SR_TUNE_ENV("SRHIP_MLP_SPREAD")) : 1;
   void (*kern)(MlpArgs) = spread ? mlp_fused_kernel<384, 0, 4, true, 1> : mlp_fused_kernel<384, 0, 4, true, 0>;
   if (row_pitch) kern = mlp_fused_kernel<384, 0, 4, true, 1, true>;
+  if (plan) kern = mlp_planned_kernel<384, 4>;
   (void)hipFuncSetAttribute((const void*)kern, hipFuncAttributeMaxDynamicSharedMemorySize, (int)smem);
   const int ntiles = cdiv(M, FBM);
   SR_LAUNCH(kern, dim3(min(ntiles, 256)), dim3(512), smem, (hipStream_t)stream, a);
@@ -587,7 +163,7 @@
                                     const float* b2, const float* row_scale2, int rows_per_sample, void* ln_next, const float* next_gamma,
                                     const float* next_beta, int M, int D, int Hd, void* stream) {
   return mlp_fused_proj_launch(x, x_out, ao, Wp, bp, row_scale1, ao_scaled, ln_gamma, ln_beta, eps, W1, b1, W2, b2, row_scale2, rows_per_sample, ln_next,
-                               next_gamma, next_beta, M, D, Hd, 0, stream);
+                               next_gamma, next_beta, M, D, Hd, 0, nullptr, 0, stream);
 }
 
 extern "C" int srhip_mlp_fused_proj_strided(const float* x, float* x_out, const void* ao, const void* Wp, const float* bp, const float* row_scale1,
@@ -597,5 +173,16 @@
   if (row_pitch < D || (row_pitch % 8) != 0) return SR_EINVAL;
   if (ln_next && row_pitch != D) return SR_EINVAL;
   return mlp_fused_proj_launch(x, x_out, ao, Wp, bp, row_scale1, ao_scaled, ln_gamma, ln_beta, eps, W1, b1, W2, b2, row_scale2, rows_per_sample, ln_next,
-                               next_gamma, next_beta, M, D, Hd, row_pitch, stream);
+                               next_gamma, next_beta, M, D, Hd, row_pitch, nullptr, 0, stream);
 }
+
+extern "C" int srhip_mlp_fused_proj_planned(const float* x, float* x_out, const void* ao, const void* Wp, const float* bp, const float* row_scale1,
+                                            int ao_scaled, const float* ln_gamma, const float* ln_beta, float eps, const void* W1, const float* b1,
+                                            const void* W2, const float* b2, const float* row_scale2, int rows_per_sample, void* ln_next,
+                                            const float* next_gamma, const float* next_beta, int M, int D, int Hd, const int* plan_row, int B,
+                                            void* stream) {
+  if (!plan_row || ((uintptr_t)plan_row & 3) || B <= 0 || rows_per_sample <= 0 || !row_scale2) return SR_EINVAL;
+  if ((long long)B * rows_per_sample != (long long)M) return SR_EINVAL;
+  return mlp_fused_proj_launch(x, x_out, ao, Wp, bp, row_scale1, ao_scaled, ln_gamma, ln_beta, eps, W1, b1, W2, b2, row_scale2, rows_per_sample, ln_next,
+                               next_gamma, next_beta, M, D, Hd, 0, plan_row, B, stream);
+}
diff --git a/semireward_amd/csrc/mlp_fused_body.h b/semireward_amd/csrc/mlp_fused_body.h
--- /dev/null
+++ b/semireward_amd/csrc/mlp_fused_body.h
@@ -0,0 +1,456 @@
+  static_assert(PROJ || !PITCH, "the row pitch belongs to the PROJ variant");
+  static_assert((PROJ && !PITCH) || !PLAN, "the row map belongs to the dense PROJ variant");
+  constexpr int KS1 = D_ / BK;
+  constexpr int KQ = 4;
+  constexpr int G1S = 2 * (KS1 / KQ);
+  constexpr int TH = D_ / RT;
+  constexpr int NT2 = D_ / 16;
+  constexpr int G2S = (CH / BK) * TH;
+  constexpr int SPC = G1S + G2S;
+  constexpr int NG = NS / GS;
+  constexpr int PD = (NG - 2) * GS;
+  static_assert(KS1 % KQ == 0 && D_ % RT == 0 && SPC % GS == 0 && NS % GS == 0 && NG >= 3, "layout");
+  extern __shared__ __attribute__((aligned(16))) bf16_t sm[];
+  float* sb1 = reinterpret_cast<float*>(sm + NS * TILE_EL);
+  float* sb2 = sb1 + a.Hd;
+  float* sgam = sb2 + D_;
+  float* sbet = sgam + D_;
+  float* sbp = sbet + D_;
+  float* sgn = sbp + D_;
+  float* sbn = sgn + D_;
+  const int tid = threadIdx.x, lane = tid & 63;
+  const int wave = __builtin_amdgcn_readfirstlane(tid >> 6);
+  const int l15 = lane & 15, lg = lane >> 4;
+  const int nch = a.Hd / CH;
+  for (int i = tid; i < a.Hd; i += 512) sb1[i] = a.b1[i];
+  for (int i = tid; i < D_; i += 512) { sb2[i] = a.b2[i]; sgam[i] = a.gamma[i]; sbet[i] = a.beta[i]; }
+  if constexpr (PROJ) {
+    for (int i = tid; i < D_; i += 512) sbp[i] = a.bp[i];
+    if (a.ln_next) for (int i = tid; i < D_; i += 512) { sgn[i] = a.gamma_n[i]; sbn[i] = a.beta_n[i]; }
+  }
+  __syncthreads();
+
+  const int pr = 16 * wave + (lane >> 2);
+  const int psl = ((lane & 3) ^ swz(pr)) * 8;
+  const int lo1 = ((pr & 31) * D_ + (pr >> 5) * BK + psl) * 2;
+  const int lo2 = (pr * a.Hd + psl) * 2;
+  const int pdst = 16 * wave * BK;
+  const int wbytes = a.Hd * D_ * 2;
+  const __amdgpu_buffer_rsrc_t r1 = __builtin_amdgcn_make_buffer_rsrc(const_cast<bf16_t*>(a.W1), 0, wbytes, 0x00020000);
+  const __amdgpu_buffer_rsrc_t r2 = __builtin_amdgcn_make_buffer_rsrc(const_cast<bf16_t*>(a.W2), 0, wbytes, 0x00020000);
+  constexpr int OOB = 0x7ffffff0;
+  constexpr int VOFF = PROJ ? TH : 0;
+  int nchv = nch + VOFF;
+  const __amdgpu_buffer_rsrc_t rp = __builtin_amdgcn_make_buffer_rsrc(const_cast<bf16_t*>(PROJ ? a.Wp : a.W2), 0, D_ * D_ * 2, 0x00020000);
+  const int lop = (pr * D_ + psl) * 2;
+  auto issue = [&](int cv, int j, int slot) {
+    if (DBG & 2) return;
+    lds_void* dst = (lds_void*)(sm + slot * TILE_EL + pdst);
+    const bool valid = cv < nchv;
+    if (PROJ && cv < VOFF) {
+      __builtin_amdgcn_raw_ptr_buffer_load_lds(rp, dst, 16, lop, (cv * RT * D_ + j * BK) * 2, 0, 0);
+      return;
+    }
+    const int c = cv - VOFF;
+    if (j < G1S) {
+      const int u = j / (KS1 / KQ), kt = j % (KS1 / KQ);
+      __builtin_amdgcn_raw_ptr_buffer_load_lds(r1, dst, 16, valid ? lo1 : OOB, ((c * CH + 32 * u) * D_ + kt * KQ * BK) * 2, 0, 0);
+    } else {
+      const int jj = j - G1S, u = jj / TH, th = jj % TH;
+      __builtin_amdgcn_raw_ptr_buffer_load_lds(r2, dst, 16, valid ? lo2 : OOB, (th * RT * a.Hd + c * CH + u * BK) * 2, 0, 0);
+    }
+  };
+
+  const int fo2 = l15 * BK + ((lg ^ swz(l15)) << 3);
+  const int h1 = 8 * (l15 >> 2) + (l15 & 3);
+  const int fo1p = h1 * BK + ((lg ^ swz(h1)) << 3);
+  const int fo1q = (h1 + 4) * BK + ((lg ^ swz(h1 + 4)) << 3);
+
+  const size_t rpitch = PITCH ? (size_t)a.pitch : (size_t)D_;
+  const int ntiles = (a.M + FBM - 1) / FBM;
+  for (int tile = blockIdx.x; tile < ntiles; tile += gridDim.x) {
+    const int m = tile * FBM + wave * 16 + l15;
+    const int mc = min(m, a.M - 1);
+    int pm = mc, si = 0;
+    bool heavy = true;
+    if constexpr (PLAN) {
+      const int q = mc / a.rows_per_sample;
+      si = (int)min((unsigned)a.plan[1 + q], (unsigned)(a.nsamp - 1));
+      pm = si * a.rows_per_sample + (mc - q * a.rows_per_sample);
+      heavy = (long long)tile * FBM < (long long)a.plan[0] * a.rows_per_sample;
+      nchv = heavy ? nch + VOFF : VOFF;
+    }
+    MDBG_T(0);
+    u32x4_t xn[KS1];
+    if constexpr (!PROJ) {
+      const float* xr = a.x + (size_t)mc * D_ + 8 * lg;
+      f32x4_t v[2 * KS1];
+      float s = 0.f;
+#pragma unroll
+      for (int k = 0; k < KS1; ++k) {
+        v[2 * k] = *reinterpret_cast<const f32x4_t*>(xr + 32 * k);
+        v[2 * k + 1] = *reinterpret_cast<const f32x4_t*>(xr + 32 * k + 4);
+      }
+#pragma unroll
+      for (int k = 0; k < 2 * KS1; ++k) s += (v[k][0] + v[k][1]) + (v[k][2] + v[k][3]);
+      s += __shfl_xor(s, 16, 64);
+      s += __shfl_xor(s, 32, 64);
+      const float mu = s * (1.0f / D_);
+      float q = 0.f;
+#pragma unroll
+      for (int k = 0; k < 2 * KS1; ++k) {
+#pragma unroll
+        for (int e = 0; e < 4; ++e) { const float d = v[k][e] - mu; q += d * d; }
+      }
+      q += __shfl_xor(q, 16, 64);
+      q += __shfl_xor(q, 32, 64);
+      const float rs = rsqrtf(q * (1.0f / D_) + a.eps);
+      if (a.save_rows > 0 && m < a.save_rows && lg == 0) { a.s_mean[m] = mu; a.s_rstd[m] = rs; }
+#pragma unroll
+      for (int k = 0; k < KS1; ++k) {
+        const f32x4_t g0 = *reinterpret_cast<const f32x4_t*>(sgam + 32 * k + 8 * lg);
+        const f32x4_t g1 = *reinterpret_cast<const f32x4_t*>(sgam + 32 * k + 8 * lg + 4);
+        const f32x4_t b0 = *reinterpret_cast<const f32x4_t*>(sbet + 32 * k + 8 * lg);
+        const f32x4_t b1 = *reinterpret_cast<const f32x4_t*>(sbet + 32 * k + 8 * lg + 4);
+        const f32x4_t p = v[2 * k], r = v[2 * k + 1];
+        xn[k] = u32x4_t{pack_bf2((p[0] - mu) * rs * g0[0] + b0[0], (p[1] - mu) * rs * g0[1] + b0[1]),
+                        pack_bf2((p[2] - mu) * rs * g0[2] + b0[2], (p[3] - mu) * rs * g0[3] + b0[3]),
+                        pack_bf2((r[0] - mu) * rs * g1[0] + b1[0], (r[1] - mu) * rs * g1[1] + b1[1]),
+                        pack_bf2((r[2] - mu) * rs * g1[2] + b1[2], (r[3] - mu) * rs * g1[3] + b1[3])};
+        if (k & 1) __builtin_amdgcn_sched_barrier(0);
+      }
+    }
+    const bool save_tile = !PROJ && a.save_rows > 0 && tile * FBM + wave * 16 < a.save_rows;
+    if (save_tile && m < a.save_rows) {
+      bf16_t* lr = a.s_ln2 + (size_t)m * D_ + 8 * lg;
+#pragma unroll
+      for (int k = 0; k < KS1; ++k) *reinterpret_cast<u32x4_t*>(lr + 32 * k) = xn[k];
+    }
+    u32x4_t aof[PROJ ? KS1 : 1];
+    if constexpr (PROJ) {
+      const bf16_t* ar = a.ao + (size_t)pm * rpitch + 8 * lg;
+#pragma unroll
+      for (int k = 0; k < KS1; ++k) aof[k] = *reinterpret_cast<const u32x4_t*>(ar + 32 * k);
+    }
+    float rs1v = 1.0f, rs2v = 1.0f;
+    f32x4_t acc2[NT2];
+    if constexpr (PROJ) {
+      if (a.row_scale1) rs1v = a.row_scale1[PLAN ? si : mc / a.rows_per_sample];
+      if (a.row_scale) rs2v = a.row_scale[PLAN ? si : mc / a.rows_per_sample];
+      const float* xr = a.x + (size_t)pm * rpitch + 4 * lg;
+#pragma unroll
+      for (int t = 0; t < NT2; ++t) acc2[t] = *reinterpret_cast<const f32x4_t*>(xr + 16 * t);
+      if (rs1v != 1.0f && !a.ao_scaled) {
+#pragma unroll
+        for (int k = 0; k < KS1; ++k)
+#pragma unroll
+          for (int e = 0; e < 4; ++e)
+            aof[k][e] = pack_bf2(rs1v * __builtin_bit_cast(float, aof[k][e] << 16), rs1v * __builtin_bit_cast(float, aof[k][e] & 0xffff0000u));
+      }
+    }
+    __syncthreads();
+    MDBG_T(1);
+#pragma unroll
+    for (int p = 0; p < PD; ++p) issue(p / SPC, p % SPC, p);
+
+    __builtin_amdgcn_sched_barrier(0);
+    if constexpr (!PROJ) {
+#pragma unroll
+      for (int t = 0; t < NT2; ++t) acc2[t] = f32x4_t{0.f, 0.f, 0.f, 0.f};
+    } else {
+#pragma unroll
+      for (int t = 0; t < NT2; ++t) {
+        const f32x4_t bb = *reinterpret_cast<const f32x4_t*>(sbp + 16 * t + 4 * lg);
+        acc2[t][0] += rs1v * bb[0]; acc2[t][1] += rs1v * bb[1]; acc2[t][2] += rs1v * bb[2]; acc2[t][3] += rs1v * bb[3];
+      }
+    }
+    f32x4_t acc1[4];
+    u32x4_t hf[2];
+    u32x4_t fa0[4], fa1[4];
+
+    auto sync_group = [&](auto jc, int c) __attribute__((always_inline)) {
+      constexpr int j = decltype(jc)::value;
+      static_assert(j % GS == 0, "group start");
+      if constexpr ((DBG & 2) == 0) wait_vm<GS*(NG - 3)>();
+      __builtin_amdgcn_s_barrier();
+      if constexpr (!SPREAD) {
+#pragma unroll
+        for (int i = 0; i < GS; ++i) {
+          const int jn = (j + PD + i) % SPC, cn = c + (j + PD + i) / SPC;
+          issue(cn, jn, (c * SPC + j + PD + i) & (NS - 1));
+        }
+      }
+    };
+    auto issue_ahead = [&](auto jc, int c, bool late) __attribute__((always_inline)) {
+      constexpr int j = decltype(jc)::value;
+      if constexpr (SPREAD == 1) { if (!late) issue(c + (j + PD) / SPC, (j + PD) % SPC, (c * SPC + j + PD) & (NS - 1)); }
+    };
+    auto read_half = [&](auto jc, auto hc, int c) __attribute__((always_inline)) {
+      constexpr int j = decltype(jc)::value, h = decltype(hc)::value;
+      u32x4_t(&fa)[4] = h ? fa1 : fa0;
+      const bf16_t* st = sm + ((c * SPC + j) & (NS - 1)) * TILE_EL;
+      if constexpr ((DBG & 4) != 0) {
+#pragma unroll
+        for (int t = 0; t < 4; ++t) fa[t] = u32x4_t{(unsigned)(c + t), 1u, 2u, (unsigned)j};
+      } else if constexpr (j < G1S) {
+#pragma unroll
+        for (int s_ = 0; s_ < 2; ++s_) {
+          fa[2 * s_] = *reinterpret_cast<const u32x4_t*>(st + fo1p + (2 * h + s_) * 32 * BK);
+          fa[2 * s_ + 1] = *reinterpret_cast<const u32x4_t*>(st + fo1q + (2 * h + s_) * 32 * BK);
+        }
+      } else {
+#pragma unroll
+        for (int t = 0; t < 4; ++t) fa[t] = *reinterpret_cast<const u32x4_t*>(st + fo2 + (4 * h + t) * 16 * BK);
+      }
+    };
+    float gcarry = 0.f, pcarry = 0.f;
+    auto acc1_start = [&](auto uc, auto xc, int c) __attribute__((always_inline)) {
+      constexpr int u = decltype(uc)::value, X = decltype(xc)::value;
+      acc1[2 * u + X] = *reinterpret_cast<const f32x4_t*>(sb1 + min(c - VOFF, nch - 1) * CH + 32 * u + 8 * lg + 4 * X);
+    };
+    auto gelu_elem = [&](auto uc, auto ec, int c) __attribute__((always_inline)) {
+      constexpr int u = decltype(uc)::value, e = decltype(ec)::value, X = e >> 2, r = e & 3;
+      const float v = acc1[2 * u + X][r];
+      if constexpr (PROJ && (DBG & 1) == 0) {
+        if constexpr ((e & 1) == 1) {
+          const f32x2_t g2 = gelu_poly2(f32x2_t{acc1[2 * u + X][r - 1], v}) * f32x2_t{rs2v, rs2v};
+          hf[u][e >> 1] = pack_bf2(g2[0], g2[1]);
+        }
+      } else {
+      float gv;
+      if constexpr ((DBG & 1) != 0) gv = v; else gv = gelu_erf(v);
+      if constexpr (PROJ) gv *= rs2v;
+      if constexpr ((e & 1) == 0) { gcarry = gv; pcarry = v; } else hf[u][e >> 1] = pack_bf2(gcarry, gv);
+      }
+      if constexpr ((e & 1) == 1) {
+        if (save_tile && m < a.save_rows) {
+          const size_t o = (size_t)m * a.Hd + (c - VOFF) * CH + 32 * u + 8 * lg + (e - 1);
+          *reinterpret_cast<uint32_t*>(a.s_pre + o) = pack_bf2(pcarry, v);
+          *reinterpret_cast<uint32_t*>(a.s_h + o) = hf[u][e >> 1];
+        }
+      }
+      if constexpr (r == 3) acc1_start(uc, std::integral_constant<int, X>{}, c + 1);
+    };
+    auto gelu_slot = [&](auto jc, auto hc, auto pc, int c) __attribute__((always_inline)) {
+      constexpr int j = decltype(jc)::value, h = decltype(hc)::value, part = decltype(pc)::value;
+      if constexpr (j >= 3 && j <= 8 && (DBG & 8) == 0) {
+        constexpr int u = (j - 3) / 3, q = 2 * ((j - 3) % 3) + h;
+        constexpr int first[7] = {0, 2, 3, 4, 6, 7, 8};
+        constexpr int e0 = first[q], n = first[q + 1] - first[q];
+        if constexpr (part < n) gelu_elem(std::integral_constant<int, u>{}, std::integral_constant<int, e0 + part>{}, c);
+      }
+    };
+    auto mfma_one = [&](auto jc, auto hc, auto tc) __attribute__((always_inline)) {
+      constexpr int j = decltype(jc)::value, h = decltype(hc)::value, t = decltype(tc)::value;
+      u32x4_t(&fa)[4] = h ? fa1 : fa0;
+      if constexpr ((DBG & 8) != 0) {
+        asm volatile("" ::"v"(fa[t]));
+        if constexpr (j == G1S - 1) { hf[0] = fa[0]; hf[1] = fa[1]; }
+      } else if constexpr (j < G1S) {
+        constexpr int u = j / (KS1 / KQ), kt = j % (KS1 / KQ);
+        acc1[2 * u + (t & 1)] = __builtin_amdgcn_mfma_f32_16x16x32_bf16(
+            __builtin_bit_cast(bf16x8_t, fa[t]), __builtin_bit_cast(bf16x8_t, xn[kt * KQ + 2 * h + (t >> 1)]), acc1[2 * u + (t & 1)],
+            0, 0, 0);
+      } else {
+        constexpr int u = (j - G1S) / TH, th = (j - G1S) % TH;
+        acc2[th * 8 + 4 * h + t] = __builtin_amdgcn_mfma_f32_16x16x32_bf16(
+            __builtin_bit_cast(bf16x8_t, fa[t]), __builtin_bit_cast(bf16x8_t, hf[u]), acc2[th * 8 + 4 * h + t], 0, 0, 0);
+      }
+    };
+    auto mfma_half = [&](auto jc, auto hc, int c) __attribute__((always_inline)) {
+      using T0 = std::integral_constant<int, 0>;
+      using T1 = std::integral_constant<int, 1>;
+      using T2 = std::integral_constant<int, 2>;
+      using T3 = std::integral_constant<int, 3>;
+      mfma_one(jc, hc, T0{});
+      mfma_one(jc, hc, T1{});
+      __builtin_amdgcn_sched_barrier(0);
+      gelu_slot(jc, hc, T0{}, c);
+      __builtin_amdgcn_sched_barrier(0);
+      mfma_one(jc, hc, T2{});
+      mfma_one(jc, hc, T3{});
+      __builtin_amdgcn_sched_barrier(0);
+      gelu_slot(jc, hc, T1{}, c);
+      __builtin_amdgcn_sched_barrier(0);
+    };
+    using H0 = std::integral_constant<int, 0>;
+    using H1 = std::integral_constant<int, 1>;
+    if constexpr (PROJ) {
+      auto read_half_p = [&](auto jc, auto hc, int cv) __attribute__((always_inline)) {
+        constexpr int j = decltype(jc)::value, h = decltype(hc)::value;
+        u32x4_t(&fa)[4] = h ? fa1 : fa0;
+        const bf16_t* st = sm + ((cv * SPC + j) & (NS - 1)) * TILE_EL;
+#pragma unroll
+        for (int t = 0; t < 4; ++t) fa[t] = *reinterpret_cast<const u32x4_t*>(st + fo2 + (4 * h + t) * 16 * BK);
+      };
+      sync_group(H0{}, 0);
+      read_half_p(H0{}, H0{}, 0);
+      static_for<VOFF>([&](auto vc) __attribute__((always_inline)) {
+        constexpr int v = decltype(vc)::value;
+        static_for<SPC>([&](auto jc) __attribute__((always_inline)) {
+          constexpr int j = decltype(jc)::value;
+          constexpr int jn = (j + 1) % SPC, vn = v + (j + 1) / SPC;
+          read_half_p(jc, H1{}, v);
+#pragma unroll
+          for (int t = 0; t < 4; ++t)
+            acc2[v * 8 + t] = __builtin_amdgcn_mfma_f32_16x16x32_bf16(__builtin_bit_cast(bf16x8_t, fa0[t]), __builtin_bit_cast(bf16x8_t, aof[j]),
+                                                                       acc2[v * 8 + t], 0, 0, 0);
+          __builtin_amdgcn_sched_barrier(0);
+          issue_ahead(jc, v, false);
+          if constexpr (jn % GS == 0) sync_group(std::integral_constant<int, jn>{}, vn);
+          if constexpr (vn == VOFF) read_half(std::integral_constant<int, 0>{}, H0{}, vn);
+          else read_half_p(std::integral_constant<int, jn>{}, H0{}, vn);
+#pragma unroll
+          for (int t = 0; t < 4; ++t)
+            acc2[v * 8 + 4 + t] = __builtin_amdgcn_mfma_f32_16x16x32_bf16(__builtin_bit_cast(bf16x8_t, fa1[t]), __builtin_bit_cast(bf16x8_t, aof[j]),
+                                                                           acc2[v * 8 + 4 + t], 0, 0, 0);
+          __builtin_amdgcn_sched_barrier(0);
+          issue_ahead(jc, v, true);
+        });
+      });
+      MDBG_T(4);
+      if (PLAN && !heavy) goto epilogue;
+      {
+        float sum = 0.f;
+#pragma unroll
+        for (int t = 0; t < NT2; ++t) sum += (acc2[t][0] + acc2[t][1]) + (acc2[t][2] + acc2[t][3]);
+        const float mu = rows_sum4(sum) * (1.0f / D_);
+        float q = 0.f;
+#pragma unroll
+        for (int t = 0; t < NT2; ++t)
+#pragma unroll
+          for (int e = 0; e < 4; ++e) { const float d = acc2[t][e] - mu; q += d * d; }
+        const float rs = rsqrtf(rows_sum4(q) * (1.0f / D_) + a.eps);
+        int ko = 4 * lg;
+        asm volatile("" : "+v"(ko) : "v"(rs));
+#pragma unroll
+        for (int sI = 0; sI < KS1; ++sI) {
+          if (sI > 0) asm volatile("" : "+v"(ko) : "v"(xn[sI - 1][3]));
+          unsigned pk[2][2];
+#pragma unroll
+          for (int e = 0; e < 2; ++e) {
+            const int t = 2 * sI + e;
+            const f32x4_t g4 = *reinterpret_cast<const f32x4_t*>(sgam + 16 * t + ko);
+            const f32x4_t b4 = *reinterpret_cast<const f32x4_t*>(sbet + 16 * t + ko);
+            pk[e][0] = pack_bf2((acc2[t][0] - mu) * rs * g4[0] + b4[0], (acc2[t][1] - mu) * rs * g4[1] + b4[1]);
+            pk[e][1] = pack_bf2((acc2[t][2] - mu) * rs * g4[2] + b4[2], (acc2[t][3] - mu) * rs * g4[3] + b4[3]);
+          }
+          unsigned out4[4];
+#pragma unroll
+          for (int d = 0; d < 2; ++d) {
+            const auto w32 = __builtin_amdgcn_permlane32_swap(pk[0][d], pk[1][d], false, false);
+            const auto w16 = __builtin_amdgcn_permlane16_swap(w32[0], w32[1], false, false);
+            out4[d] = w16[0];
+            out4[2 + d] = w16[1];
+          }
+          xn[sI] = u32x4_t{out4[0], out4[1], out4[2], out4[3]};
+          if (sI & 1) __builtin_amdgcn_sched_barrier(0);
+        }
+      }
+      MDBG_T(5);
+#pragma unroll
+      for (int t = 0; t < NT2; ++t) {
+        const f32x4_t bb = *reinterpret_cast<const f32x4_t*>(sb2 + 16 * t + 4 * lg);
+        acc2[t][0] += rs2v * bb[0]; acc2[t][1] += rs2v * bb[1]; acc2[t][2] += rs2v * bb[2]; acc2[t][3] += rs2v * bb[3];
+      }
+    }
+    {
+      using I0 = std::integral_constant<int, 0>;
+      using I1 = std::integral_constant<int, 1>;
+      acc1_start(I0{}, I0{}, VOFF); acc1_start(I0{}, I1{}, VOFF); acc1_start(I1{}, I0{}, VOFF); acc1_start(I1{}, I1{}, VOFF);
+    }
+    if constexpr (!PROJ) {
+      sync_group(H0{}, 0);
+      read_half(H0{}, H0{}, 0);
+    }
+    for (int c = VOFF; c < nchv; ++c)
+      static_for<SPC>([&](auto jc) __attribute__((always_inline)) {
+        constexpr int j = decltype(jc)::value;
+        constexpr int jn = (j + 1) % SPC;
+        const int cn = c + (j + 1) / SPC;
+        read_half(jc, H1{}, c);
+        mfma_half(jc, H0{}, c);
+        issue_ahead(jc, c, false);
+        if constexpr (jn % GS == 0) sync_group(std::integral_constant<int, jn>{}, cn);
+        read_half(std::integral_constant<int, jn>{}, H0{}, cn);
+        mfma_half(jc, H1{}, c);
+        issue_ahead(jc, c, true);
+      });
+  epilogue:
+    MDBG_T(2);
+    int pme = mc;
+    if constexpr (PLAN) {
+      int ln_;
+      asm volatile("v_mbcnt_lo_u32_b32 %0, -1, 0\n\tv_mbcnt_hi_u32_b32 %0, -1, %0" : "=v"(ln_));
+      const int me = min(tile * FBM + wave * 16 + (ln_ & 15), a.M - 1), q = me / a.rows_per_sample;
+      const int se = (int)min((unsigned)a.plan[1 + q], (unsigned)(a.nsamp - 1));
+      pme = se * a.rows_per_sample + (me - q * a.rows_per_sample);
+    }
+    if (PROJ && a.ln_next) {
+      float* xw = a.xo + (size_t)pme * rpitch + 4 * lg;
+      float sum = 0.f;
+#pragma unroll
+      for (int t = 0; t < NT2; ++t) {
+        const f32x4_t xv = acc2[t];
+        if (m < a.M) *reinterpret_cast<f32x4_t*>(xw + 16 * t) = xv;
+        sum += (xv[0] + xv[1]) + (xv[2] + xv[3]);
+      }
+      const float mu = rows_sum4(sum) * (1.0f / D_);
+      float q = 0.f;
+#pragma unroll
+      for (int t = 0; t < NT2; ++t)
+#pragma unroll
+        for (int e = 0; e < 4; ++e) { const float d = acc2[t][e] - mu; q += d * d; }
+      const float rs = rsqrtf(rows_sum4(q) * (1.0f / D_) + a.eps);
+      bf16_t* lw = a.ln_next + (size_t)pme * D_ + 8 * lg;
+      int ko = 4 * lg;
+      asm volatile("" : "+v"(ko) : "v"(rs));
+      unsigned chain = 0;
+#pragma unroll
+      for (int sI = 0; sI < KS1; ++sI) {
+        if (sI > 0) asm volatile("" : "+v"(ko) : "v"(chain));
+        unsigned pk[2][2];
+#pragma unroll
+        for (int e = 0; e < 2; ++e) {
+          const int t = 2 * sI + e;
+          const f32x4_t g4 = *reinterpret_cast<const f32x4_t*>(sgn + 16 * t + ko);
+          const f32x4_t b4 = *reinterpret_cast<const f32x4_t*>(sbn + 16 * t + ko);
+          pk[e][0] = pack_bf2((acc2[t][0] - mu) * rs * g4[0] + b4[0], (acc2[t][1] - mu) * rs * g4[1] + b4[1]);
+          pk[e][1] = pack_bf2((acc2[t][2] - mu) * rs * g4[2] + b4[2], (acc2[t][3] - mu) * rs * g4[3] + b4[3]);
+        }
+        unsigned out4[4];
+#pragma unroll
+        for (int d = 0; d < 2; ++d) {
+          const auto w32 = __builtin_amdgcn_permlane32_swap(pk[0][d], pk[1][d], false, false);
+          const auto w16 = __builtin_amdgcn_permlane16_swap(w32[0], w32[1], false, false);
+          out4[d] = w16[0];
+          out4[2 + d] = w16[1];
+        }
+        chain = out4[3];
+        if (m < a.M) *reinterpret_cast<u32x4_t*>(lw + 32 * sI) = u32x4_t{out4[0], out4[1], out4[2], out4[3]};
+      }
+    } else if (PROJ) {
+      float* xw = a.xo + (size_t)pme * rpitch + 4 * lg;
+      if (m < a.M) {
+#pragma unroll
+        for (int t = 0; t < NT2; ++t) *reinterpret_cast<f32x4_t*>(xw + 16 * t) = acc2[t];
+      }
+    } else if (m < a.M) {
+      const float rsc = a.row_scale ? a.row_scale[m / a.rows_per_sample] : 1.0f;
+      const float* xr = a.x + (size_t)m * D_ + 4 * lg;
+      float* xw = a.xo + (size_t)m * D_ + 4 * lg;
+#pragma unroll
+      for (int t = 0; t < NT2; ++t) {
+        const f32x4_t bb = *reinterpret_cast<const f32x4_t*>(sb2 + 16 * t + 4 * lg);
+        f32x4_t xv = *reinterpret_cast<const f32x4_t*>(xr + 16 * t);
+        xv[0] += rsc * (acc2[t][0] + bb[0]); xv[1] += rsc * (acc2[t][1] + bb[1]);
+        xv[2] += rsc * (acc2[t][2] + bb[2]); xv[3] += rsc * (acc2[t][3] + bb[3]);
+        *reinterpret_cast<f32x4_t*>(xw + 16 * t) = xv;
+      }
+    }
+#ifdef SRHIP_TUNING
+    __builtin_amdgcn_s_waitcnt(0);
+    __syncthreads();
+    MDBG_T(3);
+#endif
+  }
diff --git a/semireward_amd/csrc/vit_ops.hip b/semireward_amd/csrc/vit_ops.hip
--- a/semireward_amd/csrc/vit_ops.hip
+++ b/semireward_amd/csrc/vit_ops.hip
@@ -445,6 +445,36 @@
   out[o] = (p <= 0.f) ? 1.0f : (u < keep ? 1.0f / keep : 0.0f);
 }
 
+__global__ __launch_bounds__(256) void droppath_plan_kernel(const float* __restrict__ dp, long long stride_block, long long stride_branch, int B,
+                                                            int* __restrict__ plan) {
+  __shared__ int wcnt[2][4];
+  const float* f = dp + (long long)blockIdx.x * stride_block + stride_branch;
+  int* row = plan + (size_t)blockIdx.x * (1 + B);
+  const int tid = threadIdx.x, lane = tid & 63, w = tid >> 6;
+  int n_keep = 0;
+  for (int b0 = 0, it = 0; b0 < B; b0 += 256, ++it) {
+    const int b = b0 + tid;
+    const unsigned long long m = __ballot(b < B && f[b] != 0.f);
+    if (lane == 0) wcnt[it & 1][w] = __popcll(m);
+    __syncthreads();
+    n_keep += wcnt[it & 1][0] + wcnt[it & 1][1] + wcnt[it & 1][2] + wcnt[it & 1][3];
+  }
+  __syncthreads();
+  if (tid == 0) row[0] = n_keep;
+  int before = 0;
+  for (int b0 = 0, it = 0; b0 < B; b0 += 256, ++it) {
+    const int b = b0 + tid;
+    const bool keep = b < B && f[b] != 0.f;
+    const unsigned long long m = __ballot(keep);
+    if (lane == 0) wcnt[it & 1][w] = __popcll(m);
+    __syncthreads();
+    int kb = before + __popcll(m & ((1ull << lane) - 1ull));
+    for (int i = 0; i < w; ++i) kb += wcnt[it & 1][i];
+    if (b < B) row[1 + (keep ? kb : n_keep + (b - kb))] = b;
+    before += wcnt[it & 1][0] + wcnt[it & 1][1] + wcnt[it & 1][2] + wcnt[it & 1][3];
+  }
+}
+
 }
 
 template <typename TOUT = bf16_t>
@@ -708,6 +738,13 @@
   SR_CHECK_LAUNCH();
   return SR_OK;
 }
+extern "C" int srhip_vit_droppath_plan(const float* dp, long long stride_block, long long stride_branch, int depth, int B, int* plan,
+                                       void* stream) {
+  if (!dp || !plan || depth <= 0 || B <= 0 || stride_block < 0 || stride_branch < 0) return SR_EINVAL;
+  SR_LAUNCH(droppath_plan_kernel, dim3(depth), dim3(256), 0, (hipStream_t)stream, dp, stride_block, stride_branch, B, plan);
+  SR_CHECK_LAUNCH();
+  return SR_OK;
+}
 
 extern "C" int srhip_transpose_batched(const srhip_transpose_desc* desc_dev, int n, int total_tiles, void* stream) {
   if (!desc_dev || n <= 0 || total_tiles <= 0) return SR_EINVAL;
diff --git a/semireward_amd/nets/vit.py b/semireward_amd/nets/vit.py
--- a/semireward_amd/nets/vit.py
+++ b/semireward_amd/nets/vit.py
@@ -1,4 +1,5 @@
 import math
+import os
 import types
 
 import numpy as np
@@ -50,6 +51,7 @@
 _FUSED_PROJ = True
 _FUSED_NEXT_LN = True
 _LAST_BLOCK_CLASS_ROWS = True
+_SKIP_DROPPED_BRANCHES = os.environ.get("SRHIP_SKIP_DROPPED", "1") != "0"
 _FUSED_MLP_MIN_ROWS = 16384
 
 
@@ -227,6 +229,10 @@
         scale = 64 ** -0.5
         dst0, dst1 = (droppath.stride(0), droppath.stride(1)) if droppath is not None else (0, 0)
         ln_ready = False
+        plan = None
+        if _SKIP_DROPPED_BRANCHES and droppath is not None and tree is None and fused_attn and fused_mlp and _FUSED_PROJ:
+            plan = self._buf(tag + "dpplan", (cfg.depth, 1 + B), torch.int32)
+            ops.vit_droppath_plan(droppath, cfg.depth, B, plan)
         for i in range(cfg.depth):
             b = "blocks.%d." % i
             if tree is not None:
@@ -272,7 +278,8 @@
                                    P(b + "norm2.bias"), cfg.eps, P(b + "mlp.fc1.weight", wb), P(b + "mlp.fc1.bias"),
                                    P(b + "mlp.fc2.weight", wb), P(b + "mlp.fc2.bias"), s2, rps, rows, D, Hd,
                                    ln_next=ln if ln_ready else None, next_gamma=P(nb + "norm1.weight") if ln_ready else None,
-                                   next_beta=P(nb + "norm1.bias") if ln_ready else None, ao_scaled=ao_scaled, row_pitch=pitch)
+                                   next_beta=P(nb + "norm1.bias") if ln_ready else None, ao_scaled=ao_scaled, row_pitch=pitch,
+                                   plan_row=ops.RawRows(plan, i * (1 + B)) if (plan is not None and not class_rows) else None)
             else:
                 ops.gemm_nt(ops.EPI_RESID_F32, ao, P(b + "attn.proj.weight", wb), x, M, D, D, bias=P(b + "attn.proj.bias"),
                             row_scale=s1, rows_per_sample=N, **gp)
diff --git a/semireward_amd/ops.py b/semireward_amd/ops.py
--- a/semireward_amd/ops.py
+++ b/semireward_amd/ops.py
@@ -502,7 +502,8 @@
 
 
 def mlp_fused_proj(x, ao, Wp, bp, row_scale1, gamma, beta, eps, W1, b1, W2, b2, row_scale2, rows_per_sample, M, D, Hd, x_out=None,
-                   ln_next=None, next_gamma=None, next_beta=None, ao_scaled=False, row_pitch=None):
+                   ln_next=None, next_gamma=None, next_beta=None, ao_scaled=False, row_pitch=None, plan_row=None):
+    assert row_pitch is None or plan_row is None
     args = (_p(x), _p(x_out if x_out is not None else x), _p(ao), _p(Wp), _p(bp), _p(row_scale1), int(bool(ao_scaled)), _p(gamma), _p(beta), eps,
             _p(W1), _p(b1),
             _p(W2), _p(b2), _p(row_scale2), rows_per_sample, _p(ln_next), _p(next_gamma), _p(next_beta), M, D, Hd)
@@ -512,7 +513,14 @@
             _PROFILE.timed("srhip_mlp_fused_proj_strided", (*args, int(row_pitch), _s(),), 4.0 * M * D * Hd + 2.0 * M * D * D,
                            "mlp_fused_kernel<384, 0, 4, true, 1> class rows", nbytes)
             return
+        if plan_row is not None:
+            _PROFILE.timed("srhip_mlp_fused_proj_planned", (*args, _p(plan_row), M // rows_per_sample, _s(),), 4.0 * M * D * Hd + 2.0 * M * D * D,
+                           "mlp_fused_kernel<384, 0, 4, true, 1>", nbytes)
+            return
         _PROFILE.timed("srhip_mlp_fused_proj", (*args, _s(),), 4.0 * M * D * Hd + 2.0 * M * D * D, "mlp_fused_kernel<384, 0, 4, true, 1>", nbytes)
+        return
+    if plan_row is not None:
+        _call("srhip_mlp_fused_proj_planned", *args, _p(plan_row), M // rows_per_sample, _s())
         return
     if row_pitch is not None:
         _call("srhip_mlp_fused_proj_strided", *args, int(row_pitch), _s())
@@ -686,6 +694,13 @@
 
 def cast_f32_bf16(x, out, n):
     _call("srhip_cast_f32_bf16", _p(x), _p(out), n, _s())
+
+
+def vit_droppath_plan(dp, depth, B, plan):
+    if _CHECK_ARGS:
+        assert dp.is_cuda and dp.dim() == 3 and dp.stride(2) == 1 and dp.shape[0] >= depth and dp.shape[1] == 2 and dp.shape[2] >= B and plan.dtype == torch.int32 and plan.is_contiguous()
+        assert plan.numel() == depth * (1 + B)
+    _call("srhip_vit_droppath_plan", dp.data_ptr(), dp.stride(0), dp.stride(1), depth, B, _p(plan), _s())
 
 
 def droppath_fill(out, probs, depth, B, seed, cols=None, seed_dev=None):
```

Result: faster. 1731 (median of 6 runs) (+2.4%).
